# SiyuanHuang95/SUG

Hardware: AMD Instinct MI355X
Metric: point-clouds/sec (train step, N=1024) (higher is better)
Workload: dtype f32

## Files before the change

include/sug_amd.h:

```cpp
#ifndef SUG_AMD_H
#define SUG_AMD_H

#include <stdint.h>

#ifdef __cplusplus
extern "C" {
#endif

#define SUG_OK 0
#define SUG_ERR_ARG (-1)
#define SUG_ERR_LAUNCH (-2)
#define SUG_STATS_BLOCKS 1024

const char* sug_last_error(void);
#define SUG_ABI_VERSION 7
int sug_abi_version(void);

int sug_knn(const float* x, int64_t ldx, int B, int N, int C, int k,
            int32_t* idx, void* stream);

int sug_knn_reverse(const int32_t* idx, int B, int N, int k,
                    int32_t* rev_off, int32_t* rev_ent, void* stream);

int sug_fps(const float* xyz, const int32_t* start, int B, int N, int npoint,
// ... 8 lines not shown
                         int32_t* idx_out, float* dist_out, void* stream);

int sug_three_nn(const float* query, const float* cand, int B, int N, int S,
                 int32_t* idx3, float* dist3, void* stream);

int sug_three_nn_direct(const float* query, const float* cand, int B, int N, int S,
                        int32_t* idx3, float* dist3, void* stream);

int sug_ball_query_multi(const float* xyz, const float* query, int B, int N, int S, int R, const float* r2,
                         const int32_t* nsample, int32_t* const* out, void* stream);

int sug_fp_interp_fwd(const float* src, int64_t lds, const int32_t* idx3, const float* d3, int B, int N, int S, int D,
                      float* out, int64_t ldo, float* w3, void* stream);
int sug_fp_interp_bwd(const float* g, int64_t ldg, const int32_t* idx3, const float* w3, int B, int N, int S, int D,
                      int32_t* rev_off, int32_t* rev_ent, float* dsrc, int64_t ldd, void* stream);

int sug_copy_rows2d(const float* src, int64_t lds, float* dst, int64_t ldd, int64_t rows, int C, void* stream);

int sug_gather_rows(const float* feat, int64_t ldf, const int32_t* idx,
                    int B, int N, int S, int C, float* out, int64_t ldo, void* stream);
int sug_scatter_add_rows(const float* g, int64_t ldg, const int32_t* idx,
                         int B, int N, int S, int C, float* dfeat, int64_t ldf, void* stream);
int64_t sug_scatter_rows_workspace(int B, int N, int S);
int sug_scatter_rows_ordered_supported(int B, int N, int S);
int sug_scatter_rows_ordered(const float* g, int64_t ldg, const int32_t* idx, int B, int N, int S, int C,
                             float* dfeat, int64_t ldf, int32_t* ws, void* stream);

int sug_group_max(const float* feat, int64_t ldf, const int32_t* idx, int B, int N, int S,
                  int ns, int C, float* out, int32_t* arg, void* stream);
int sug_group_max_shared(const float* feat, int64_t ldf, int Bsrc, const int32_t* idx, int B, int N, int S,
                         int ns, int C, float* out, int32_t* arg, void* stream);
int sug_group_max_bwd(const float* g, const int32_t* arg, int B, int N, int S, int C,
                      float* dfeat, int64_t ldf, void* stream);

int sug_edgeconv_fwd(const float* pq, int64_t ldpq, const int32_t* idx, const float* gamma,
                     int B, int N, int k, int Co, float* z, uint8_t* arg, float* s1,
                     double* stats, float* ws, void* stream);

int sug_bn_finalize(const double* stats, const float* gamma, const float* beta, int C,
                    double count, float eps, float momentum, float* running_mean,
                    float* running_var, float* coef, void* stream);

int sug_edgeconv_fwd_bn(const float* pq, int64_t ldpq, const int32_t* idx, const float* gamma,
                        const float* beta, int B, int N, int k, int Co, float eps, float momentum,
                        float* running_mean, float* running_var, float* z, uint8_t* arg, float* s1,
                        float* coef, float* ws, void* stream);
int sug_col_stats_bn(const float* y, int64_t ldy, int64_t rows, int C, const float* gamma, const float* beta,
                     float eps, float momentum, float* running_mean, float* running_var, float* coef,
                     float* ws, void* stream);

int sug_col_stats_bn_grouped(const float* y, int64_t ldy, int64_t rows, int C, int groups, const float* gamma,
                             const float* beta, float eps, float momentum, float* running_mean, float* running_var,
                             float* coef, float* ws, void* stream);

int sug_bn_replay(const float* coef, int G, int C, float momentum, float* running_mean, float* running_var,
                  void* stream);
int sug_bn_replay_multi(int n, const void* const* coef, const int32_t* G, const int32_t* C, const float* momentum,
                        void* const* running_mean, void* const* running_var, void* stream);

int sug_affine_act(const float* z, int64_t ldz, const float* coef, int64_t rows, int C,
                   float slope, float* out, int64_t ldo, void* stream);

int sug_col_stats(const float* y, int64_t ldy, int64_t rows, int C, double* stats, float* ws,
                  void* stream);

int sug_edgeconv_bwd_reduce(const float* gout, int64_t ldg, const float* z, const float* coef,
                            int64_t rows, int Co, float slope, float* a, double* red, float* ws,
                            void* stream);
int sug_edgeconv_bwd_scatter(const float* a, const uint8_t* arg, const float* s1,
                             const float* pq, int64_t ldpq, const int32_t* rev_off,
                             const int32_t* rev_ent, const float* coef, const double* red,
                             int B, int N, int k, int Co, float* dpq, int64_t lddpq, void* stream);

int64_t sug_linear_dw_workspace(int64_t R, int M, int N);
int sug_linear_dw(const float* g, int64_t ldg, const float* x, int64_t ldx, int64_t R, int M, int N,
                  float* dw, float* ws, void* stream);
int sug_linear_dw_fold(const float* part, int nchunk, int64_t MN, float* dw, void* stream);
int sug_linear_dw_bias(const float* g, int64_t ldg, const float* x, int64_t ldx, int64_t R, int M, int N,
                       float* dw, float* db, float* ws, void* stream);

int64_t sug_colsum_workspace(int64_t rows, int C);
int sug_colsum(const void* x, int64_t ld, int64_t rows, int C, int dtype, float sign, float* out, float* ws, void* stream);

int sug_gate_fwd(const float* x, const float* z, int64_t n, float* out, void* stream);
int sug_gate_bwd(const float* g, const float* x, const float* z, int64_t n, float* dx, float* dz, void* stream);
int sug_gate_bn_fwd(const float* x, const float* z, int M, int C, const float* gamma, const float* beta,
                    float* running_mean, float* running_var, int training, float eps, float momentum, float* out,
                    float* stat, void* stream);
int sug_gate_bn_bwd(const float* g, const float* x, const float* z, int M, int C, const float* gamma, const float* stat,
                    int training, float* dx, float* dz, float* dgamma, float* dbeta, void* stream);

int sug_calayer_supported(int layers, int M, int C, int Hd);
int sug_calayer_fwd(int layers, const float* x, int64_t ldx, int M, int C, int Hd, const float* const* W0,
                    const float* const* b0, const float* const* W2, const float* const* b2, float* hp, float* h, float* z,
                    void* stream);
int sug_calayer_bwd(int layers, const float* x, int64_t ldx, int M, int C, int Hd, const float* const* W0,
                    const float* const* W2, const float* h, const float* dz, const float* dxg, float* const* dW0,
                    float* const* db0, float* const* dW2, float* const* db2, float* dhp, float* dh, float* dx, int64_t lddx,
                    void* stream);

int sug_head_linear_supported(int M, int K, int No, int pro, int epi);
int sug_head_linear_fwd(int heads, const float* const* in, int64_t ldin, const float* const* W, const float* const* bias,
                        float* const* z, const float* const* gamma, const float* const* beta, const float* const* u,
                        float* const* stats, float* const* act, int M, int K, int No, int pro, float slope, float eps,
                        float p_drop, void* stream);
int sug_head_ln_bwd(int heads, const float* const* gup, int64_t ldg, const float* const* z, const float* const* stats,
                    const float* const* gamma, const float* const* beta, const float* const* u,
                    const float* const* gextra, float* const* dz, float* const* dgamma, float* const* dbeta,
                    float* const* db, int M, int No, float slope, float p_drop, void* stream);
int sug_head_linear_bwd(int heads, int sum_da, const float* const* dz, int64_t ldg, const float* const* in, int64_t ldin,
                        const float* const* stats_in, const float* const* gamma_in, const float* const* beta_in,
                        const float* const* u_in, const float* const* W, float* const* dW, float* const* db,
                        float* const* da, int64_t ldda, int M, int K, int No, int pro, float slope, float p_drop_in,
                        void* stream);

int sug_ln_act_fwd(const float* x, const float* gamma, const float* beta, int rows, int C, float eps, float slope,
                   float* y, float* stat, void* stream);
int sug_ln_act_bwd(const float* g, const float* x, const float* gamma, const float* beta, const float* stat, int rows,
                   int C, float slope, float* dx, float* dgamma, float* dbeta, float* ws, void* stream);

int sug_adam_chunk(void);
int sug_adam_step(const int64_t* table, const int32_t* block_first, const int32_t* block_first_host, int T,
                  const void* const* grads_host, double lr, double beta1, double beta2, double eps,
                  double weight_decay, double bias_corr1, double bias_corr2, void* stream);
int sug_adam_step_capturable(const int64_t* table, const int32_t* block_first, const int32_t* block_first_host,
                             int T, const void* const* grads_host, double lr, double beta1, double beta2,
                             double eps, double weight_decay, int32_t* step_dev, float* scalars_dev,
                             const double* lr_dev, void* stream);

#define SUG_ADAM_CHAIN_SLOTS 2
#define SUG_ADAM_CHAIN_BUCKETS 8
int sug_adam_chain_chunk(void);
int sug_adam_chain_step(const int64_t* table, const int32_t* block_map, const int32_t* block_first_host, int T,
                        const void* const* grads_host, int nbuckets, const double* hyper_host, int32_t* steps_dev,
                        float* scalars_dev, const double* lr_dev, void* stream);

int sug_node_offset_fwd(const float* proj, const float* loc, const int32_t* fidx,
                        const int32_t* gidx, int B, int N, int S, int ns, float* off, float* nloc,
                        void* stream);
int sug_node_offset_bwd(const float* proj, const float* loc, const int32_t* fidx,
                        const int32_t* gidx, const float* goff, int B, int N, int S, int ns,
                        float* dproj, void* stream);
int sug_node_offset_fwd_shared(const float* proj, int Bsrc, const float* loc, const int32_t* fidx,
// ... 24 lines not shown
                        const float* gmean, int64_t ld_pool, const int32_t* arg, int B, int N, int C, float slope,
                        int train, double* red, float* ws, float* dy, int64_t lddy, void* stream);

int sug_edgeconv_layer_fwd(const float* pq, int64_t ldpq, const int32_t* idx, const float* gamma,
                           const float* beta, int B, int N, int k, int Co, int groups, int training,
                           float eps, float momentum, float slope, float* running_mean,
                           float* running_var, float* z, uint8_t* arg, float* s1, float* coef,
                           float* out, int64_t ldo, double* stats, float* ws, void* stream);
int sug_edgeconv_fused_supported(int N, int k, int Cin, int Co);
int sug_edgeconv_fused_layer_fwd(const float* x, int64_t ldx, int Cin, const float* wcat, const float* qbias,
                                 const int32_t* idx, const float* gamma, const float* beta, int B, int N, int k,
                                 int Co, int groups, int training, float eps, float momentum, float slope,
                                 float* running_mean, float* running_var, float* z, uint8_t* arg, float* s1,
                                 float* pq_out, int64_t ldpq, float* coef, float* out, int64_t ldo, float* ws,
                                 void* stream);
int sug_edgeconv_layer_bwd(const float* gout, int64_t ldg, const float* z, const uint8_t* arg,
                           const float* s1, const float* pq, int64_t ldpq, const int32_t* idx,
                           const float* coef, int B, int N, int k, int Co, int groups, int training,
                           float slope, float* a, double* red, int32_t* rev_off, int32_t* rev_ent,
                           float* dpq, int64_t lddpq, float* ws, float* dgb, void* stream);
int sug_sa_first_fwd(const float* P, int64_t ldp, const float* Q, const int32_t* idx, int B, int N, int S,
                     int ns, int C, int groups, const float* gamma, const float* beta, int training,
                     float eps, float momentum, float* running_mean, float* running_var, float* coef,
                     float* Z, float* ws, void* stream);
int sug_sa_first_bwd(const float* gz, const float* P, int64_t ldp, const float* Q, const int32_t* idx, int B,
                     int N, int S, int ns, int C, int groups, int training, const float* coef, double* red,
                     int32_t* rev_off, int32_t* rev_ent, float* segsum, float* dP, float* dQ, float* ws, float* dgb,
                     void* stream);
int sug_sa_first_geo_fwd(const float* Pf, int64_t ldp, const float* xyz, const float* cent, const float* Wx, int ldw,
                         const float* bias, const int32_t* idx, int B, int N, int S, int ns, int C, int groups,
                         const float* gamma, const float* beta, int training, float eps, float momentum,
                         float* running_mean, float* running_var, float* coef, float* Z, float* ws, void* stream);
int sug_sa_first_geo_bwd(const float* gz, const float* Pf, int64_t ldp, const float* xyz, const float* cent, const float* Wx,
                         int ldw, const float* bias, const int32_t* idx, int B, int N, int S, int ns, int C, int groups,
                         int training, const float* coef, double* red, int32_t* rev_off, int32_t* rev_ent, float* segsum,
                         float* dP, float* dQ, float* ws, float* dgb, void* stream);

int sug_bn_act_rows_fwd(const float* y, int64_t ldy, int64_t rows, int C, int groups, const float* gamma,
                        const float* beta, int training, float eps, float momentum, float slope,
                        float* running_mean, float* running_var, float* coef, float* out, int64_t ldo,
                        double* stats, float* ws, void* stream);
int sug_bn_act_rows_bwd(const float* gout, int64_t ldg, const float* y, int64_t ldy, const float* coef,
                        int64_t rows, int C, int groups, int training, float slope, float* a, double* red,
                        float* dy, float* ws, float* dgb, void* stream);
int sug_bn_act_pool_layer_fwd(const float* y, int64_t ldy, int B, int N, int C, int groups,
                              const float* gamma, const float* beta, int training, float eps, float momentum,
                              float slope, float* running_mean, float* running_var, float* coef,
                              float* out_max, float* out_mean, int64_t ld_pool, int32_t* arg, double* stats, float* ws_stats,
                              float* ws_pool, void* stream);
int sug_bn_act_pool_layer_bwd(const float* y, int64_t ldy, const float* coef, const float* gmax,
                              const float* gmean, int64_t ld_pool, const int32_t* arg, int B, int N, int C, int groups,
                              float slope, int training, double* red, float* ws, float* dy, int64_t lddy,
                              float* dgb, void* stream);

int sug_pointmlp_max_fwd(const float* x, int64_t ldx, int64_t rows, int K, const float* w, const float* bias,
                         const float* gamma, int Co, int seg, float* zext, int32_t* arg, float* ws, int* nblk,
                         void* stream);
int sug_rows_gemm(const float* x, int64_t ldx, int64_t rows, int K, const float* w, const float* bias, int Co,
                  float* y, int64_t ldy, void* stream);
int sug_pointmlp_max_layer_fwd(const float* x, int64_t ldx, int64_t rows, int K, const float* w, const float* bias,
                               const float* gamma, const float* beta, int Co, int seg, int groups, int training,
                               float eps, float momentum, float slope, float* running_mean, float* running_var,
                               float* zext, int32_t* arg, float* coef, float* out, int64_t ldo, float* ws,
                               void* stream);
int sug_pointmlp_max_layer_fwd_xf(const float* y, int64_t ldy, int64_t rows, int K, const float* xcoef, float xslope,
                                  float* zout, int64_t ldz, const float* w, const float* bias, const float* gamma,
                                  const float* beta, int Co, int seg, int groups, int training, float eps, float momentum,
                                  float slope, float* running_mean, float* running_var, float* zext, int32_t* arg,
                                  float* coef, float* out, int64_t ldo, float* ws, void* stream);
int sug_pointmlp_max_bwd_coef(const float* coef, const double* red, const float* bias, const float* w, int64_t rows,
                              int K, int Co, float* kb, float* k2, float* nkb, float* nwk, void* stream);
int sug_pointmlp_max_bwd_dwfix(float* dw, const float* dws, const float* kb, const float* k2, const float* w,
                               const float* xtx, const float* sx, int K, int Co, int with_stats, void* stream);
int64_t sug_pointmlp_max_bwd_workspace(int64_t rows, int K, int Co, int seg);
int sug_pointmlp_max_bwd_sparse(const float* a, const int32_t* arg, const float* x, int64_t ldx, const float* w,
                                int64_t rows, int K, int Co, int seg, float* dx, int64_t lddx, float* dw,
                                float* ws, void* stream);

int sug_ptran_pos1_fwd(const float* xyz, const int32_t* nbr, const float* w1, const float* b1, int B, int n, int k,
                       int d, int dtype, void* out, void* stream);
int sug_ptran_pos1_bwd(const void* g, const float* xyz, const int32_t* nbr, const float* w1, const float* b1, int B,
                       int n, int k, int d, int dtype, float* dw1, float* db1, float* ws, void* stream);
int sug_ptran_qk_fwd(const float* q, const float* kf, const void* delta, const int32_t* nbr, int B, int n, int k, int d,
                     int dtype, void* out, void* stream);
int sug_ptran_qk_bwd(const void* du, void* da, const int32_t* rev_off, const int32_t* rev_ent, int B, int n, int k, int d,
                     int dtype, float* dq, float* dk, float* db, float* ws, void* stream);
int sug_ptran_attn_fwd(const void* logits, const void* delta, const float* vf, const int32_t* nbr, int B, int n, int k,
                       int d, int dtype, float scale, float* mixed, float* mx, float* sm, void* stream);
int sug_ptran_attn_bwd(const float* g, const float* mixed, const void* logits, const void* delta, const float* vf,
                       const int32_t* nbr, const float* mx, const float* sm, const int32_t* rev_off, const int32_t* rev_ent,
                       int B, int n, int k, int d, int dtype, float scale, void* dlogits, void* da, float* dv, float* db,
                       float* ws, void* stream);
int sug_ptran_fused_supported(int B, int n, int k, int d);
int sug_ptran_fused_fwd(const float* xyz, const int32_t* nbr, const float* q, const float* kf, const float* vf,
                        const float* w1, const float* b1, const void* w2, const void* b2, const void* wg1, const void* bg1,
                        const void* wg2, const void* bg2, int B, int n, int k, int d, float scale, int save, void* T0,
                        void* delta, void* U, void* T1, void* Lg, float* mixed, float* mx, float* sm, void* stream);
int64_t sug_ptran_colsum_workspace(int64_t rows);
int sug_ptran_relu_bwd_db(void* G, const void* T1, int64_t rows, int d, int dtype, float* db, float* ws, void* stream);
int sug_grad_scale16(const float* g0, int64_t n0, const float* g1, int64_t n1, const float* g2, int64_t n2, int log2_target,
                     float* out, float* ws, void* stream);

int sug_fold_groups(const double* red, int groups, int n, float* out, void* stream);

int sug_mmd_rbf(const float* z, int64_t ldz, int m, int D, const float* w,
                const float* neg_gamma, int nsigma, double* sums, float* wt, void* stream);
// ... 23 lines not shown
int sug_soft_mmd_multi_fwd(int n, const void* const* feat_s, const int64_t* lds, const void* const* feat_t,
                           const int64_t* ldt, const int32_t* D, const float* label_scale, const int64_t* label_s,
                           const int64_t* label_t, int m, int num_class, const void* const* w, const float* neg_gamma,
                           int nsigma, void* const* z, void* const* wt, double* sums, float* values, void* stream);
int sug_soft_mmd_multi_bwd(int n, const void* const* z, const int32_t* D, const void* const* wt,
                           const void* const* gscale, int m, int num_class, void* const* dz, void* stream);

#define SUG_CLASS_MMD_MAX_ROWS 1024
#define SUG_CLASS_MMD_MAX_CLASSES 64
#define SUG_CLASS_MMD_MAX_D 1048576
int sug_mmd_select(const int64_t* label_s, const int64_t* label_t, int m, int num_class, int mode, int32_t* idx_s,
                   int32_t* idx_t, int32_t* pos_s, int32_t* pos_t, int32_t* count, void* stream);
int sug_class_mmd_fwd(const float* feat_s, int64_t lds, const float* feat_t, int64_t ldt, int m, int D,
                      const int32_t* idx_s, const int32_t* idx_t, const int32_t* count, const float* neg_gamma,
                      int nsigma, float* z, float* wt, double* sums, float* value, void* stream);
int sug_class_mmd_bwd(const float* z, const float* wt, int m, int D, const int32_t* count, const int32_t* pos_s,
                      const int32_t* pos_t, const float* gscale, float* dz, float* dfeat_s, int64_t ldds,
                      float* dfeat_t, int64_t lddt, void* stream);

#define SUG_MMD_EST_MAX_ROWS 1024
#define SUG_MMD_EST_MAX_D 1048576
#define SUG_MMD_EST_MAX_SIGMAS 8
#define SUG_MMD_POLY_MAX_DEGREE 8
#define SUG_MMD_RATIO_ROW_FIELDS 9
#define SUG_MMD_RATIO_STATS 16
int sug_mmd_ratio_fwd(const float* z, int64_t ldz, int m, int D, const float* neg_gamma, int nsigma, int biased, float* K,
                      float* G, double* rows, double* stats, float* out3, float* wt_m, float* wt_v, void* stream);
int sug_mmd_ratio_bwd(const float* z, int64_t ldz, int m, int D, const float* wt_m, const float* wt_v, const float* out3,
                      const float* g3, float* dz, int64_t lddz, void* stream);
int sug_mmd_adjacent_fwd(const float* x, int64_t ldx, const float* y, int64_t ldy, int m, int D, int mode, int degree,
                         double alpha, double c, double* part, float* coef, float* value, void* stream);
int sug_mmd_adjacent_bwd(const float* x, int64_t ldx, const float* y, int64_t ldy, int m, int D, int mode, const float* coef,
                         const float* gscale, float* dx, int64_t lddx, float* dy, int64_t lddy, void* stream);

#define SUG_CL_LOSS_MAX_ROWS 1024
#define SUG_CL_LOSS_MAX_D 1048576
#define SUG_CL_LOSS_MAX_TERMS 4
#define SUG_CL_LOSS_SUM_FIELDS 3
#define SUG_CL_LOSS_ROW_FIELDS 4
int sug_cl_loss_fwd(int n, const void* const* x, const int64_t* ldx, const void* const* y, const int64_t* ldy, const int32_t* D,
                    const double* margin, const int64_t* label_s, const int64_t* label_t, int m, const void* const* w,
                    double* sums, void* const* coef, float* values, void* stream);
int sug_cl_loss_bwd(int n, const void* const* x, const int64_t* ldx, const void* const* y, const int64_t* ldy, const int32_t* D,
                    int m, const void* const* coef, const void* const* gscale, void* const* dx, const int64_t* lddx,
                    void* const* dy, const int64_t* lddy, void* stream);

int sug_edge_weight_split(const float* in, int Co, int C, int backward, float* out, void* stream);
int sug_edge_weight_split_multi(const void* const* in_host, const int32_t* Co_host, const int32_t* C_host, int n,
                                int backward, void* const* out_host, void* stream);

int64_t sug_chamfer_workspace(int B, int N, int M);
int sug_chamfer(const float* a, const float* b, int B, int N, int M, float* out, float* ws, void* stream);
int sug_chamfer_weights(const float* a, const float* b, int B, int N, int M, int method, float* out, float* ws, void* stream);
#define SUG_CHAMFER_MAX_POINTS 5000
int sug_chamfer_nn(const float* a, const float* b, int B, int N, int M, float* dist1, float* dist2, int32_t* idx1, int32_t* idx2,
                   void* stream);
int sug_chamfer_nn_bwd(const float* g1, const float* g2, const float* a, const float* b, const int32_t* idx1, const int32_t* idx2,
                       int B, int N, int M, float* ga, float* gb, void* stream);

#define SUG_CE_PAIR_MAX_ROWS 512
#define SUG_CE_PAIR_MAX_CLASSES 32
int sug_ce_pair_fwd(const float* logits1, const float* logits2, int64_t ld, const int64_t* label, int M, int C, float w,
                    int64_t ignore_index, float* loss, float* lse, void* stream);
int sug_ce_pair_bwd(const float* logits1, const float* logits2, int64_t ld, const int64_t* label, int M, int Mtot, int C,
                    float w, int64_t ignore_index, const float* g, const float* lse, float* d1, float* d2, void* stream);
#define SUG_CE_MAX_ROWS 1024
#define SUG_CE_MAX_CLASSES 64
int sug_ce_fwd(const float* logits, int64_t ld, const int64_t* label, int M, int C, int64_t ignore_index, float label_smoothing,
               float* loss, float* lse, double* totals, void* stream);
int sug_ce_bwd(const float* logits, int64_t ld, const int64_t* label, int M, int C, int64_t ignore_index, float label_smoothing,
               const float* g, const float* lse, float* dlogits, void* stream);
#define SUG_MCD_MAX_ROWS 1024
int sug_mcd_loss_fwd(const float* ys1, const float* ys2, const float* yt1, const float* yt2, int64_t ld, const int64_t* label,
                     const int64_t* label_t, int Ms, int Mt, int C, float a_s, float a_t, float r_s, float* out4, float* lse,
                     double* totals, void* stream);
int sug_mcd_loss_bwd(const float* ys1, const float* ys2, const float* yt1, const float* yt2, int64_t ld, const int64_t* label,
                     const int64_t* label_t, int Ms, int Mt, int C, float a_s, float a_t, const float* g, const float* lse,
                     float* ds1, float* ds2, float* dt1, float* dt2, void* stream);
int sug_cls_loss_fwd(const float* ys1, const float* ys2, const float* yt1, const float* yt2, int64_t ld, const int64_t* label,
                     const int64_t* label_t, int Ms, int Mt, int C, const float* alpha, float gamma, int reduce_sum,
                     int64_t ignore_index, float a_s, float a_t, float a_d, float r_s, float* out4, float* save, double* totals,
                     void* stream);
int sug_cls_loss_bwd(const float* ys1, const float* ys2, const float* yt1, const float* yt2, int64_t ld, const int64_t* label,
                     const int64_t* label_t, int Ms, int Mt, int C, const float* alpha, float gamma, int reduce_sum,
                     int64_t ignore_index, float a_s, float a_t, float a_d, float r_s, const float* g, const float* save,
                     float* ds1, float* ds2, float* dt1, float* dt2, void* stream);
int sug_loss_combine_fwd(const float* loss_cls, const float* v_geo, const float* v_sem1, const float* v_sem2, float wg, float ws,
                         float* out3, void* stream);
int sug_loss_combine_bwd(const float* g, float wg, float ws, float* out4, void* stream);

#define SUG_EVAL_MAX_ROWS 4096
#define SUG_EVAL_MAX_CLASSES 64
#define SUG_EVAL_BATCH_COUNT 0
#define SUG_EVAL_DATA_TOTAL 1
#define SUG_EVAL_CORRECT_TOTAL 2
#define SUG_EVAL_ERROR 3
#define SUG_EVAL_LOSS_TOTAL 4
#define SUG_EVAL_CLASS_ACC 8
#define SUG_EVAL_CLASS_ROWS 136
#define SUG_EVAL_CLASS_CORRECT 200
#define SUG_EVAL_BATCH_ACC 264
#define SUG_EVAL_STATE_WORDS(cap) (SUG_EVAL_BATCH_ACC + (cap))
int sug_eval_accumulate(const float* logits1, const float* logits2, int64_t ld, const int64_t* label, int B, int C,
                        const float* loss_in, int ce_mode, int64_t ignore_index, float label_smoothing, float* out,
                        int64_t* pred, int cls_eval, void* state, int cap, void* stream);

// ... 91 lines not shown
```

sug_amd/csrc/bnpool.hip:

```cpp
#include "common.h"
#include <hip/hip_fp16.h>

namespace {

__global__ __launch_bounds__(256) void bn_bwd_apply_vec4_kernel(const float* __restrict__ a,
                                                                const float* __restrict__ y, int64_t ldy,
                                                                const float* __restrict__ coef,
                                                                const double* __restrict__ red,
                                                                int64_t rows, int C, float invM,
                                                                float* __restrict__ dy, int64_t lddy) {
  const int C4 = C >> 2;
  const int64_t total = rows * C4;
  for (int64_t e = (int64_t)blockIdx.x * 256 + threadIdx.x; e < total; e += (int64_t)gridDim.x * 256) {
    const int c = (int)(e % C4) * 4;
    const int64_t r = e / C4;
    const float4 av = *reinterpret_cast<const float4*>(a + r * C + c);
    const float4 yv = *reinterpret_cast<const float4*>(y + r * ldy + c);
    const float4 sc = *reinterpret_cast<const float4*>(coef + c);
    const float4 mean = *reinterpret_cast<const float4*>(coef + 2 * C + c);
    const float4 rstd = *reinterpret_cast<const float4*>(coef + 3 * C + c);
    float4 o;
    o.x = av.x - sc.x * invM * ((float)red[c + 0] + (yv.x - mean.x) * rstd.x * (float)red[C + c + 0]);
    o.y = av.y - sc.y * invM * ((float)red[c + 1] + (yv.y - mean.y) * rstd.y * (float)red[C + c + 1]);
    o.z = av.z - sc.z * invM * ((float)red[c + 2] + (yv.z - mean.z) * rstd.z * (float)red[C + c + 2]);
// ... 10 lines not shown
                                                                       int64_t rows_g, int C, float invM, float slope,
                                                                       float* __restrict__ dy, int64_t lddy) {
  const int C4 = C >> 2;
  const int64_t total = rows * C4;
  for (int64_t e = (int64_t)blockIdx.x * 256 + threadIdx.x; e < total; e += (int64_t)gridDim.x * 256) {
    const int c = (int)(e % C4) * 4;
    const int64_t r = e / C4;
    const int64_t g = r / rows_g;
    const float* cg = coef + g * 5 * C;
    const double* rg = red + g * 2 * C;
    float4 av = *reinterpret_cast<const float4*>(a + r * lda + c);
    const float4 yv = *reinterpret_cast<const float4*>(y + r * ldy + c);
    const float4 sc = *reinterpret_cast<const float4*>(cg + c);
    const float4 mean = *reinterpret_cast<const float4*>(cg + 2 * C + c);
    const float4 rstd = *reinterpret_cast<const float4*>(cg + 3 * C + c);
    if (FROM_G) {
      const float4 sh = *reinterpret_cast<const float4*>(cg + C + c);
      av.x = sc.x * (av.x * (fmaf(sc.x, yv.x, sh.x) > 0.f ? 1.f : slope));
      av.y = sc.y * (av.y * (fmaf(sc.y, yv.y, sh.y) > 0.f ? 1.f : slope));
      av.z = sc.z * (av.z * (fmaf(sc.z, yv.z, sh.z) > 0.f ? 1.f : slope));
      av.w = sc.w * (av.w * (fmaf(sc.w, yv.w, sh.w) > 0.f ? 1.f : slope));
    }
    float4 o;
    o.x = av.x - sc.x * invM * ((float)rg[c + 0] + (yv.x - mean.x) * rstd.x * (float)rg[C + c + 0]);
    o.y = av.y - sc.y * invM * ((float)rg[c + 1] + (yv.y - mean.y) * rstd.y * (float)rg[C + c + 1]);
    o.z = av.z - sc.z * invM * ((float)rg[c + 2] + (yv.z - mean.z) * rstd.z * (float)rg[C + c + 2]);
    o.w = av.w - sc.w * invM * ((float)rg[c + 3] + (yv.w - mean.w) * rstd.w * (float)rg[C + c + 3]);
    *reinterpret_cast<float4*>(dy + r * lddy + c) = o;
  }
}

__global__ __launch_bounds__(256) void bn_bwd_apply_kernel(const float* __restrict__ a,
                                                           const float* __restrict__ y, int64_t ldy,
                                                           const float* __restrict__ coef,
                                                           const double* __restrict__ red, int64_t rows,
                                                           int C, float invM, float* __restrict__ dy,
                                                           int64_t lddy) {
  const int64_t total = rows * C;
  for (int64_t e = (int64_t)blockIdx.x * 256 + threadIdx.x; e < total; e += (int64_t)gridDim.x * 256) {
    const int c = (int)(e % C);
    const int64_t r = e / C;
    const float f = coef[c] * invM;
    const float xhat = (y[r * ldy + c] - coef[2 * C + c]) * coef[3 * C + c];
    dy[r * lddy + c] = a[r * C + c] - f * ((float)red[c] + xhat * (float)red[C + c]);
  }
}

constexpr int NS = 4;

__device__ __forceinline__ float lrelu(float u, float slope) { return u > 0.f ? u : u * slope; }

template <int VEC>
__global__ __launch_bounds__(256) void bn_act_pool_part_kernel(const float* __restrict__ y, int64_t ldy,
                                                               const float* __restrict__ coef, int N,
                                                               int C, float slope,
                                                               float* __restrict__ pmax,
                                                               float* __restrict__ psum,
                                                               int32_t* __restrict__ parg) {
  constexpr int LX = 64 / VEC, LY = 256 / LX;
  __shared__ float s_m[LY][64];
  __shared__ float s_s[LY][64];
  __shared__ int s_a[LY][64];
  const int b = blockIdx.y, ch = blockIdx.z;
  const int lx = threadIdx.x % LX, ly = threadIdx.x / LX;
  const int c = blockIdx.x * 64 + lx * VEC;
  const int n0 = (int)((int64_t)N * ch / NS), n1 = (int)((int64_t)N * (ch + 1) / NS);
  float best[VEC], sum[VEC];
  int bi[VEC];
#pragma unroll
  for (int v = 0; v < VEC; ++v) { best[v] = -INFINITY; sum[v] = 0.f; bi[v] = n0; }
  if (c < C) {
    float sc[VEC], sh[VEC];
#pragma unroll
    for (int v = 0; v < VEC; ++v) { sc[v] = coef[c + v]; sh[v] = coef[C + c + v]; }
    const float* p = y + (int64_t)b * N * ldy + c;
#pragma unroll 4
    for (int n = n0 + ly; n < n1; n += LY) {
      float val[VEC];
      if constexpr (VEC == 4) {
        const float4 t = *reinterpret_cast<const float4*>(p + (int64_t)n * ldy);
        val[0] = t.x; val[1] = t.y; val[2] = t.z; val[3] = t.w;
      } else {
        val[0] = p[(int64_t)n * ldy];
      }
#pragma unroll
      for (int v = 0; v < VEC; ++v) {
        const float u = lrelu(fmaf(sc[v], val[v], sh[v]), slope);
        sum[v] += u;
        if (u > best[v]) { best[v] = u; bi[v] = n; }
      }
    }
  }
#pragma unroll
  for (int v = 0; v < VEC; ++v) {
    s_m[ly][lx * VEC + v] = best[v];
    s_s[ly][lx * VEC + v] = sum[v];
    s_a[ly][lx * VEC + v] = bi[v];
  }
  __syncthreads();
  if (threadIdx.x < 64) {
    const int cc = blockIdx.x * 64 + threadIdx.x;
    if (cc < C) {
      float m = s_m[0][threadIdx.x], sm = s_s[0][threadIdx.x];
      int a = s_a[0][threadIdx.x];
      for (int i = 1; i < LY; ++i) {
        sm += s_s[i][threadIdx.x];
        const float mi = s_m[i][threadIdx.x];
        const int ai = s_a[i][threadIdx.x];
        if (mi > m || (mi == m && ai < a)) { m = mi; a = ai; }
      }
      const int64_t o = ((int64_t)b * NS + ch) * C + cc;
      pmax[o] = m; psum[o] = sm; parg[o] = a;
    }
  }
}

__global__ __launch_bounds__(256) void pool_combine_kernel(const float* __restrict__ pmax,
                                                           const float* __restrict__ psum,
                                                           const int32_t* __restrict__ parg, int B, int N,
                                                           int C, float* __restrict__ omax,
                                                           float* __restrict__ omean, int64_t ldp,
                                                           int32_t* __restrict__ arg) {
  const int64_t e = (int64_t)blockIdx.x * 256 + threadIdx.x;
  if (e >= (int64_t)B * C) return;
  const int b = (int)(e / C), c = (int)(e % C);
  float m = -INFINITY, sm = 0.f;
  int a = 0;
  for (int ch = 0; ch < NS; ++ch) {
    const int64_t o = ((int64_t)b * NS + ch) * C + c;
    sm += psum[o];
    if (pmax[o] > m) { m = pmax[o]; a = parg[o]; }
  }
  omax[(int64_t)b * ldp + c] = m; omean[(int64_t)b * ldp + c] = sm / (float)N; arg[e] = a;
}

template <int VEC>
__global__ __launch_bounds__(256) void pool_bwd_reduce_kernel(const float* __restrict__ y, int64_t ldy,
                                                              const float* __restrict__ coef,
                                                              const float* __restrict__ gmax,
                                                              const float* __restrict__ gmean, int64_t ldp,
                                                              const int32_t* __restrict__ arg, int N,
                                                              int C, float slope, float* __restrict__ ws) {
  constexpr int LX = 64 / VEC, LY = 256 / LX;
  __shared__ float s_g[LY][64];
  __shared__ float s_x[LY][64];
  const int b = blockIdx.y, ch = blockIdx.z;
  const int lx = threadIdx.x % LX, ly = threadIdx.x / LX;
  const int c = blockIdx.x * 64 + lx * VEC;
  const int n0 = (int)((int64_t)N * ch / NS), n1 = (int)((int64_t)N * (ch + 1) / NS);
  float sg[VEC], sx[VEC];
#pragma unroll
  for (int v = 0; v < VEC; ++v) { sg[v] = 0.f; sx[v] = 0.f; }
  if (c < C) {
    float sc[VEC], sh[VEC], mean[VEC], rstd[VEC], gm[VEC], gx[VEC];
    int am[VEC];
#pragma unroll
    for (int v = 0; v < VEC; ++v) {
      sc[v] = coef[c + v]; sh[v] = coef[C + c + v]; mean[v] = coef[2 * C + c + v]; rstd[v] = coef[3 * C + c + v];
      gm[v] = gmean[(int64_t)b * ldp + c + v] / (float)N;
      gx[v] = gmax[(int64_t)b * ldp + c + v];
      am[v] = arg[(int64_t)b * C + c + v];
    }
    const float* p = y + (int64_t)b * N * ldy + c;
#pragma unroll 4
    for (int n = n0 + ly; n < n1; n += LY) {
      float val[VEC];
      if constexpr (VEC == 4) {
        const float4 t = *reinterpret_cast<const float4*>(p + (int64_t)n * ldy);
        val[0] = t.x; val[1] = t.y; val[2] = t.z; val[3] = t.w;
      } else {
        val[0] = p[(int64_t)n * ldy];
      }
#pragma unroll
      for (int v = 0; v < VEC; ++v) {
        const float u = fmaf(sc[v], val[v], sh[v]);
        const float g = (u > 0.f ? 1.f : slope) * (gm[v] + (n == am[v] ? gx[v] : 0.f));
        sg[v] += g;
        sx[v] = fmaf(g, (val[v] - mean[v]) * rstd[v], sx[v]);
      }
    }
  }
#pragma unroll
  for (int v = 0; v < VEC; ++v) {
    s_g[ly][lx * VEC + v] = sg[v];
    s_x[ly][lx * VEC + v] = sx[v];
  }
  __syncthreads();
  if (threadIdx.x < 64) {
    const int cc = blockIdx.x * 64 + threadIdx.x;
    if (cc < C) {
      float tg = 0.f, tx = 0.f;
      for (int i = 0; i < LY; ++i) { tg += s_g[i][threadIdx.x]; tx += s_x[i][threadIdx.x]; }
      float* w = ws + ((size_t)b * NS + ch) * 2 * C;
      w[cc] = tg;
      w[C + cc] = tx;
    }
  }
}

template <int VEC>
__global__ __launch_bounds__(256) void pool_bwd_apply_kernel(const float* __restrict__ y, int64_t ldy,
                                                             const float* __restrict__ coef,
                                                             const double* __restrict__ red,
                                                             const float* __restrict__ gmax,
                                                             const float* __restrict__ gmean, int64_t ldp,
                                                             const int32_t* __restrict__ arg, int B,
                                                             int N, int C, float slope, float invM,
                                                             float* __restrict__ dy, int64_t lddy) {
  const int CV = C / VEC;
  const int64_t total = (int64_t)B * N * CV;
  for (int64_t e = (int64_t)blockIdx.x * 256 + threadIdx.x; e < total; e += (int64_t)gridDim.x * 256) {
    const int c = (int)(e % CV) * VEC;
    const int64_t r = e / CV;
    const int b = (int)(r / N), n = (int)(r - (int64_t)b * N);
    float val[VEC], out[VEC];
    if constexpr (VEC == 4) {
      const float4 t = *reinterpret_cast<const float4*>(y + r * ldy + c);
      val[0] = t.x; val[1] = t.y; val[2] = t.z; val[3] = t.w;
    } else {
      val[0] = y[r * ldy + c];
    }
#pragma unroll
    for (int v = 0; v < VEC; ++v) {
      const float sc = coef[c + v];
      const float u = fmaf(sc, val[v], coef[C + c + v]);
      const float g = (u > 0.f ? 1.f : slope) * (gmean[(int64_t)b * ldp + c + v] / (float)N +
                                                 (n == arg[(int64_t)b * C + c + v] ? gmax[(int64_t)b * ldp + c + v] : 0.f));
      const float xhat = (val[v] - coef[2 * C + c + v]) * coef[3 * C + c + v];
      out[v] = sc * (g - invM * ((float)red[c + v] + xhat * (float)red[C + c + v]));
    }
    if constexpr (VEC == 4) {
      *reinterpret_cast<float4*>(dy + r * lddy + c) = make_float4(out[0], out[1], out[2], out[3]);
    } else {
      dy[r * lddy + c] = out[0];
    }
  }
}

__global__ __launch_bounds__(256) void pool_bwd_apply_rows_kernel(const float* __restrict__ y, int64_t ldy,
                                                                  const float* __restrict__ coef,
                                                                  const double* __restrict__ red,
                                                                  const float* __restrict__ gmax,
                                                                  const float* __restrict__ gmean, int64_t ldp,
                                                                  const int32_t* __restrict__ arg, int N, int C,
                                                                  int rows_per_block, float slope, float invM,
                                                                  float* __restrict__ dy, int64_t lddy) {
  const int CV = C >> 2;
  const int b = blockIdx.y;
  const int cg = threadIdx.x % CV, rl = threadIdx.x / CV, rstep = 256 / CV;
  const int c = cg * 4;
  float sc[4], sh[4], mu[4], rs[4], r0[4], r1[4], gme[4], gmx[4];
  int am[4];
#pragma unroll
  for (int v = 0; v < 4; ++v) {
    sc[v] = coef[c + v];
    sh[v] = coef[C + c + v];
    mu[v] = coef[2 * C + c + v];
    rs[v] = coef[3 * C + c + v];
    r0[v] = (float)red[c + v];
    r1[v] = (float)red[C + c + v];
    gme[v] = gmean[(int64_t)b * ldp + c + v] / (float)N;
    gmx[v] = gmax[(int64_t)b * ldp + c + v];
    am[v] = arg[(int64_t)b * C + c + v];
  }
  const int n0 = blockIdx.x * rows_per_block;
  const int n1 = n0 + rows_per_block < N ? n0 + rows_per_block : N;
  const float* yb = y + (int64_t)b * N * ldy + c;
  float* db = dy + (int64_t)b * N * lddy + c;
#pragma unroll 4
  for (int n = n0 + rl; n < n1; n += rstep) {
    const float4 t = *reinterpret_cast<const float4*>(yb + (int64_t)n * ldy);
    const float val[4] = {t.x, t.y, t.z, t.w};
    float out[4];
#pragma unroll
    for (int v = 0; v < 4; ++v) {
      const float u = fmaf(sc[v], val[v], sh[v]);
      const float g = (u > 0.f ? 1.f : slope) * (gme[v] + (n == am[v] ? gmx[v] : 0.f));
      const float xhat = (val[v] - mu[v]) * rs[v];
      out[v] = sc[v] * (g - invM * (r0[v] + xhat * r1[v]));
    }
    *reinterpret_cast<float4*>(db + (int64_t)n * lddy) = make_float4(out[0], out[1], out[2], out[3]);
  }
}

__global__ __launch_bounds__(256) void reduce_rows_kernel(const float* __restrict__ ws, int nrow, int W,
                                                          double* __restrict__ out) {
  __shared__ double s_p[16][17];
  const int cl = threadIdx.x & 15, p = threadIdx.x >> 4;
  const int c = blockIdx.x * 16 + cl;
  double acc = 0.0;
  if (c < W)
    for (int b = p; b < nrow; b += 16) acc += (double)ws[(size_t)b * W + c];
  s_p[p][cl] = acc;
  __syncthreads();
  if (p == 0 && c < W) {
    double t = 0.0;
#pragma unroll
    for (int i = 0; i < 16; ++i) t += s_p[i][cl];
    out[c] = t;
  }
}
// ... 104 lines not shown
    }
  }
  s1 = wave_sum_f(s1) / (float)C;
  s2 = wave_sum_f(s2) / (float)C;
#pragma unroll
  for (int u = 0; u < LN_MAXV; ++u) {
    const int c = lane + 64 * u;
    if (c < C) dx[(size_t)r * C + c] = rstd * (gh[u] - s1 - xh[u] * s2);
  }
}

__global__ __launch_bounds__(256) void ln_act_bwd_param_kernel(const float* __restrict__ ga, const float* __restrict__ x,
                                                               const float* __restrict__ stat, int rows, int C,
                                                               float* __restrict__ dgamma, float* __restrict__ dbeta) {
  const int c = blockIdx.x * 256 + threadIdx.x;
  if (c >= C) return;
  float dg = 0.f, db = 0.f;
  for (int r0 = 0; r0 < rows; r0 += 8) {
    float a[8], xv[8];
#pragma unroll
    for (int u = 0; u < 8; ++u) {
      const int r = r0 + u < rows ? r0 + u : rows - 1;
      a[u] = ga[(size_t)r * C + c];
      xv[u] = x[(size_t)r * C + c];
    }
#pragma unroll
    for (int u = 0; u < 8; ++u) {
      if (r0 + u >= rows) continue;
      const int r = r0 + u;
      dg = fmaf(a[u], (xv[u] - stat[2 * r]) * stat[2 * r + 1], dg);
      db += a[u];
    }
  }
  dgamma[c] = dg;
  dbeta[c] = db;
}

static bool vec4_ok(const float* y, int64_t ld, int C) {
  return (C % 4 == 0) && (ld % 4 == 0) && ((uintptr_t)y % 16 == 0);
}

extern "C" int sug_bn_act_pool_fwd(const float* y, int64_t ldy, const float* coef, int B, int N, int C,
                                   float slope, float* out_max, float* out_mean, int64_t ld_pool, int32_t* arg,
                                   float* ws, void* stream) {
  SUG_REQUIRE(y && coef && out_max && out_mean && arg && ws, "sug_bn_act_pool_fwd: null pointer");
  SUG_REQUIRE(B > 0 && N > 0 && C > 0 && ldy >= C && ld_pool >= C && B <= 65535, "sug_bn_act_pool_fwd: bad shape");
  hipStream_t st = (hipStream_t)stream;
  const size_t part = (size_t)B * NS * C;
  float* pmax = ws;
  float* psum = ws + part;
  int32_t* parg = reinterpret_cast<int32_t*>(ws + 2 * part);
  dim3 grid(sug_divup(C, 64), B, NS);
  if (vec4_ok(y, ldy, C))
    hipLaunchKernelGGL((bn_act_pool_part_kernel<4>), grid, dim3(256), 0, st, y, ldy, coef, N, C, slope, pmax, psum, parg);
  else
    hipLaunchKernelGGL((bn_act_pool_part_kernel<1>), grid, dim3(256), 0, st, y, ldy, coef, N, C, slope, pmax, psum, parg);
  SUG_LAUNCH_CHECK("sug_bn_act_pool_fwd");
  hipLaunchKernelGGL(pool_combine_kernel, dim3(sug_divup((int64_t)B * C, 256)), dim3(256), 0, st, pmax, psum, parg,
                     B, N, C, out_max, out_mean, ld_pool, arg);
  SUG_LAUNCH_CHECK("sug_bn_act_pool_fwd(combine)");
  return SUG_OK;
}

extern "C" int sug_bn_act_pool_bwd(const float* y, int64_t ldy, const float* coef, const float* gmax,
                                   const float* gmean, int64_t ld_pool, const int32_t* arg, int B, int N, int C,
                                   float slope, int train, double* red, float* ws, float* dy,
                                   int64_t lddy, void* stream) {
  SUG_REQUIRE(y && coef && gmax && gmean && arg && red && ws && dy, "sug_bn_act_pool_bwd: null pointer");
  SUG_REQUIRE(B > 0 && N > 0 && C > 0 && ldy >= C && lddy >= C && ld_pool >= C && B * NS <= SUG_STATS_BLOCKS,
              "sug_bn_act_pool_bwd: bad shape (B must be <= %d)", SUG_STATS_BLOCKS / NS);
  hipStream_t st = (hipStream_t)stream;
  const bool vec = vec4_ok(y, ldy, C) && vec4_ok(dy, lddy, C);
  dim3 grid(sug_divup(C, 64), B, NS);
  if (vec)
    hipLaunchKernelGGL((pool_bwd_reduce_kernel<4>), grid, dim3(256), 0, st, y, ldy, coef, gmax, gmean, ld_pool, arg, N, C, slope, ws);
  else
    hipLaunchKernelGGL((pool_bwd_reduce_kernel<1>), grid, dim3(256), 0, st, y, ldy, coef, gmax, gmean, ld_pool, arg, N, C, slope, ws);
  SUG_LAUNCH_CHECK("sug_bn_act_pool_bwd(reduce)");
  hipLaunchKernelGGL(reduce_rows_kernel, dim3(sug_divup(2 * C, 16)), dim3(256), 0, st, ws, B * NS, 2 * C, red);
  SUG_LAUNCH_CHECK("sug_bn_act_pool_bwd(combine)");
  const float invM = train ? (float)(1.0 / ((double)B * N)) : 0.f;
  if (vec && (C / 4) <= 256 && 256 % (C / 4) == 0 && B <= 65535) {
    const int rpb = 64 > 256 / (C / 4) ? 64 : 256 / (C / 4);
    hipLaunchKernelGGL(pool_bwd_apply_rows_kernel, dim3(sug_divup(N, rpb), B), dim3(256), 0, st, y, ldy, coef, red, gmax,
                       gmean, ld_pool, arg, N, C, rpb, slope, invM, dy, lddy);
  } else if (vec)
    hipLaunchKernelGGL((pool_bwd_apply_kernel<4>), dim3(ew_grid((int64_t)B * N * C / 4)), dim3(256), 0, st, y, ldy,
                       coef, red, gmax, gmean, ld_pool, arg, B, N, C, slope, invM, dy, lddy);
  else
    hipLaunchKernelGGL((pool_bwd_apply_kernel<1>), dim3(ew_grid((int64_t)B * N * C)), dim3(256), 0, st, y, ldy, coef,
                       red, gmax, gmean, ld_pool, arg, B, N, C, slope, invM, dy, lddy);
  SUG_LAUNCH_CHECK("sug_bn_act_pool_bwd(apply)");
  return SUG_OK;
}


namespace {
__global__ __launch_bounds__(256) void fold_groups_kernel(const double* __restrict__ red, int groups, int n,
                                                          float* __restrict__ out) {
  const int i = blockIdx.x * 256 + threadIdx.x;
  if (i >= n) return;
  double t = 0.0;
  for (int g = 0; g < groups; ++g) t += red[(int64_t)g * n + i];
  out[i] = (float)t;
}
}

extern "C" int sug_fold_groups(const double* red, int groups, int n, float* out, void* stream) {
  SUG_REQUIRE(red && out && groups >= 1 && n > 0, "sug_fold_groups: bad argument");
  hipLaunchKernelGGL(fold_groups_kernel, dim3(sug_divup(n, 256)), dim3(256), 0, (hipStream_t)stream, red, groups, n, out);
  SUG_LAUNCH_CHECK("sug_fold_groups");
  return SUG_OK;
}

extern "C" int sug_ln_act_fwd(const float* x, const float* gamma, const float* beta, int rows, int C, float eps, float slope,
                              float* y, float* stat, void* stream) {
  SUG_REQUIRE(x && gamma && beta && y && stat, "sug_ln_act_fwd: null pointer");
  SUG_REQUIRE(rows > 0 && C > 0 && C <= 64 * LN_MAXV, "sug_ln_act_fwd: rows=%d C=%d (C <= %d)", rows, C, 64 * LN_MAXV);
  hipLaunchKernelGGL(ln_act_fwd_kernel, dim3(sug_divup(rows, 4)), dim3(256), 0, (hipStream_t)stream, x, gamma, beta, rows, C, eps,
                     slope, y, stat);
  SUG_LAUNCH_CHECK("sug_ln_act_fwd");
  return SUG_OK;
}

extern "C" int sug_ln_act_bwd(const float* g, const float* x, const float* gamma, const float* beta, const float* stat, int rows,
                              int C, float slope, float* dx, float* dgamma, float* dbeta, float* ws, void* stream) {
  SUG_REQUIRE(g && x && gamma && beta && stat && dx && dgamma && dbeta && ws, "sug_ln_act_bwd: null pointer");
  SUG_REQUIRE(rows > 0 && C > 0 && C <= 64 * LN_MAXV, "sug_ln_act_bwd: rows=%d C=%d (C <= %d)", rows, C, 64 * LN_MAXV);
  hipStream_t st = (hipStream_t)stream;
  hipLaunchKernelGGL(ln_act_bwd_dx_kernel, dim3(sug_divup(rows, 4)), dim3(256), 0, st, g, x, gamma, beta, stat, rows, C, slope, dx,
                     ws);
  SUG_LAUNCH_CHECK("sug_ln_act_bwd");
  hipLaunchKernelGGL(ln_act_bwd_param_kernel, dim3(sug_divup(C, 256)), dim3(256), 0, st, ws, x, stat, rows, C, dgamma, dbeta);
  SUG_LAUNCH_CHECK("sug_ln_act_bwd(param)");
  return SUG_OK;
}

namespace {

__global__ __launch_bounds__(256) void gate_fwd_kernel(const float* __restrict__ x, const float* __restrict__ z, int64_t n,
                                                       float* __restrict__ out) {
  const int64_t i = (int64_t)blockIdx.x * 256 + threadIdx.x;
  if (i >= n) return;
  const float s = 1.0f / (1.0f + expf(-z[i]));
  out[i] = __fadd_rn(__fmul_rn(x[i], s), x[i]);
}

__global__ __launch_bounds__(256) void gate_bwd_kernel(const float* __restrict__ g, const float* __restrict__ x,
                                                       const float* __restrict__ z, int64_t n, float* __restrict__ dx,
                                                       float* __restrict__ dz) {
  const int64_t i = (int64_t)blockIdx.x * 256 + threadIdx.x;
  if (i >= n) return;
  const float s = 1.0f / (1.0f + expf(-z[i]));
  const float gi = g[i];
  dx[i] = __fadd_rn(__fmul_rn(gi, s), gi);
  dz[i] = __fmul_rn(__fmul_rn(gi, x[i]), __fmul_rn(__fsub_rn(1.0f, s), s));
}

}

extern "C" int sug_gate_fwd(const float* x, const float* z, int64_t n, float* out, void* stream) {
  SUG_REQUIRE(x && z && out, "sug_gate_fwd: null pointer");
  SUG_REQUIRE(n > 0, "sug_gate_fwd: empty input");
  hipLaunchKernelGGL(gate_fwd_kernel, dim3((unsigned)sug_divup(n, 256)), dim3(256), 0, (hipStream_t)stream, x, z, n, out);
  SUG_LAUNCH_CHECK("sug_gate_fwd");
  return SUG_OK;
}

extern "C" int sug_gate_bwd(const float* g, const float* x, const float* z, int64_t n, float* dx, float* dz, void* stream) {
  SUG_REQUIRE(g && x && z && dx && dz, "sug_gate_bwd: null pointer");
  SUG_REQUIRE(n > 0, "sug_gate_bwd: empty input");
  hipLaunchKernelGGL(gate_bwd_kernel, dim3((unsigned)sug_divup(n, 256)), dim3(256), 0, (hipStream_t)stream, g, x, z, n, dx, dz);
  SUG_LAUNCH_CHECK("sug_gate_bwd");
  return SUG_OK;
}

namespace {

__device__ __forceinline__ float gate_val(float x, float z) {
  const float s = 1.0f / (1.0f + expf(-z));
  return __fadd_rn(__fmul_rn(x, s), x);
}

template <int MR>
__global__ __launch_bounds__(64) void gate_bn_fwd_kernel(const float* __restrict__ x, const float* __restrict__ z, int M, int C,
                                                         const float* __restrict__ gamma, const float* __restrict__ beta,
                                                         float* __restrict__ rmean, float* __restrict__ rvar, int training,
                                                         float eps, float momentum, float* __restrict__ out,
                                                         float* __restrict__ stat) {
  const int c = blockIdx.x * 64 + threadIdx.x;
  if (c >= C) return;
  float gv[MR > 0 ? MR : 1];
  if constexpr (MR > 0) {
    float xv[MR], zv[MR];
#pragma unroll
    for (int i = 0; i < MR; ++i) {
      const int r = i < M ? i : M - 1;
      xv[i] = x[(int64_t)r * C + c];
      zv[i] = z[(int64_t)r * C + c];
    }
#pragma unroll
    for (int i = 0; i < MR; ++i) gv[i] = gate_val(xv[i], zv[i]);
  }
  auto g_at = [&](int i) { if constexpr (MR > 0) return gv[i]; else return gate_val(x[(int64_t)i * C + c], z[(int64_t)i * C + c]); };
  float mean, invstd;
  if (training) {
    float s = 0.f;
    if constexpr (MR > 0) {
#pragma unroll
      for (int i = 0; i < MR; ++i) s += i < M ? gv[i] : 0.f;
    } else {
#pragma unroll 8
      for (int i = 0; i < M; ++i) s += g_at(i);
    }
    mean = s / (float)M;
    float q = 0.f;
    if constexpr (MR > 0) {
#pragma unroll
      for (int i = 0; i < MR; ++i) { const float d = gv[i] - mean; q = i < M ? fmaf(d, d, q) : q; }
    } else {
#pragma unroll 8
      for (int i = 0; i < M; ++i) { const float d = g_at(i) - mean; q = fmaf(d, d, q); }
    }
    const float var = q / (float)M;
    invstd = 1.0f / sqrtf(var + eps);
    if (rmean) {
      rmean[c] = (1.0f - momentum) * rmean[c] + momentum * mean;
      rvar[c] = (1.0f - momentum) * rvar[c] + momentum * (M > 1 ? q / (float)(M - 1) : var);
    }
  } else {
    mean = rmean[c];
    invstd = 1.0f / sqrtf(rvar[c] + eps);
  }
  stat[c] = mean;
  stat[C + c] = invstd;
  const float sc = gamma[c] * invstd, sh = beta[c] - mean * sc;
  if constexpr (MR > 0) {
#pragma unroll
    for (int i = 0; i < MR; ++i)
      if (i < M) out[(int64_t)i * C + c] = fmaf(gv[i], sc, sh);
  } else {
#pragma unroll 8
    for (int i = 0; i < M; ++i) out[(int64_t)i * C + c] = fmaf(g_at(i), sc, sh);
  }
}

template <int MR>
__global__ __launch_bounds__(64) void gate_bn_bwd_kernel(const float* __restrict__ g, const float* __restrict__ x,
                                                         const float* __restrict__ z, int M, int C,
                                                         const float* __restrict__ gamma, const float* __restrict__ stat,
                                                         int training, float* __restrict__ dx, float* __restrict__ dz,
                                                         float* __restrict__ dgamma, float* __restrict__ dbeta) {
  const int c = blockIdx.x * 64 + threadIdx.x;
  if (c >= C) return;
  const float mean = stat[c], invstd = stat[C + c];
  float sb = 0.f, sg = 0.f;
  float xr[MR > 0 ? MR : 1], sr[MR > 0 ? MR : 1], hr[MR > 0 ? MR : 1], gr[MR > 0 ? MR : 1];
  if constexpr (MR > 0) {
    float zr[MR];
#pragma unroll
    for (int i = 0; i < MR; ++i) {
      const int r = i < M ? i : M - 1;
      xr[i] = x[(int64_t)r * C + c];
      zr[i] = z[(int64_t)r * C + c];
      gr[i] = i < M ? g[(int64_t)r * C + c] : 0.f;
    }
#pragma unroll
    for (int i = 0; i < MR; ++i) {
      sr[i] = 1.0f / (1.0f + expf(-zr[i]));
      hr[i] = (__fadd_rn(__fmul_rn(xr[i], sr[i]), xr[i]) - mean) * invstd;
      sb += gr[i];
      sg = fmaf(gr[i], hr[i], sg);
    }
  } else {
#pragma unroll 8
    for (int i = 0; i < M; ++i) {
      const float gi = g[(int64_t)i * C + c];
      const float xh = (gate_val(x[(int64_t)i * C + c], z[(int64_t)i * C + c]) - mean) * invstd;
      sb += gi;
      sg = fmaf(gi, xh, sg);
    }
  }
  dgamma[c] = sg;
  dbeta[c] = sb;
  const float k = gamma[c] * invstd;
  const float mb = training ? sb / (float)M : 0.f, mg = training ? sg / (float)M : 0.f;
  if constexpr (MR > 0) {
#pragma unroll
    for (int i = 0; i < MR; ++i) {
      if (i < M) {
        const float dg = k * (gr[i] - mb - hr[i] * mg);
        dx[(int64_t)i * C + c] = __fadd_rn(__fmul_rn(dg, sr[i]), dg);
        dz[(int64_t)i * C + c] = __fmul_rn(__fmul_rn(dg, xr[i]), __fmul_rn(__fsub_rn(1.0f, sr[i]), sr[i]));
      }
    }
  } else {
#pragma unroll 8
    for (int i = 0; i < M; ++i) {
      const float xv = x[(int64_t)i * C + c], zv = z[(int64_t)i * C + c];
      const float s = 1.0f / (1.0f + expf(-zv));
      const float gv = __fadd_rn(__fmul_rn(xv, s), xv);
      const float xh = (gv - mean) * invstd;
      const float dg = k * (g[(int64_t)i * C + c] - mb - xh * mg);
      dx[(int64_t)i * C + c] = __fadd_rn(__fmul_rn(dg, s), dg);
      dz[(int64_t)i * C + c] = __fmul_rn(__fmul_rn(dg, xv), __fmul_rn(__fsub_rn(1.0f, s), s));
    }
  }
}

}

extern "C" int sug_gate_bn_fwd(const float* x, const float* z, int M, int C, const float* gamma, const float* beta,
                               float* running_mean, float* running_var, int training, float eps, float momentum, float* out,
                               float* stat, void* stream) {
  SUG_REQUIRE(x && z && gamma && beta && out && stat, "sug_gate_bn_fwd: null pointer");
  SUG_REQUIRE(M >= 1 && M <= 1024 && C >= 1, "sug_gate_bn_fwd: bad shape M=%d C=%d", M, C);
  SUG_REQUIRE(training || (running_mean && running_var), "sug_gate_bn_fwd: eval mode needs the running buffers");
  SUG_REQUIRE(!running_mean == !running_var, "sug_gate_bn_fwd: running_mean and running_var come together");
  if (M <= 32)
    hipLaunchKernelGGL(gate_bn_fwd_kernel<32>, dim3((unsigned)sug_divup(C, 64)), dim3(64), 0, (hipStream_t)stream, x, z, M, C, gamma,
                       beta, running_mean, running_var, training, eps, momentum, out, stat);
  else
    hipLaunchKernelGGL(gate_bn_fwd_kernel<0>, dim3((unsigned)sug_divup(C, 64)), dim3(64), 0, (hipStream_t)stream, x, z, M, C, gamma,
                       beta, running_mean, running_var, training, eps, momentum, out, stat);
  SUG_LAUNCH_CHECK("sug_gate_bn_fwd");
  return SUG_OK;
}

extern "C" int sug_gate_bn_bwd(const float* g, const float* x, const float* z, int M, int C, const float* gamma,
                               const float* stat, int training, float* dx, float* dz, float* dgamma, float* dbeta,
                               void* stream) {
  SUG_REQUIRE(g && x && z && gamma && stat && dx && dz && dgamma && dbeta, "sug_gate_bn_bwd: null pointer");
  SUG_REQUIRE(M >= 1 && M <= 1024 && C >= 1, "sug_gate_bn_bwd: bad shape M=%d C=%d", M, C);
  if (M <= 32)
    hipLaunchKernelGGL(gate_bn_bwd_kernel<32>, dim3((unsigned)sug_divup(C, 64)), dim3(64), 0, (hipStream_t)stream, g, x, z, M, C,
                       gamma, stat, training, dx, dz, dgamma, dbeta);
  else
    hipLaunchKernelGGL(gate_bn_bwd_kernel<0>, dim3((unsigned)sug_divup(C, 64)), dim3(64), 0, (hipStream_t)stream, g, x, z, M, C,
                       gamma, stat, training, dx, dz, dgamma, dbeta);
  SUG_LAUNCH_CHECK("sug_gate_bn_bwd");
  return SUG_OK;
}

namespace {

template <typename T>
__global__ __launch_bounds__(256) void colsum_part_kernel(const T* __restrict__ x, int64_t ld, int64_t R, int C,
                                                          float* __restrict__ part) {
  __shared__ float s_p[8][33];
  const int cx = threadIdx.x & 31, ry = threadIdx.x >> 5;
  const int c = blockIdx.x * 32 + cx;
  float acc = 0.f;
  if (c < C)
    for (int64_t r = (int64_t)blockIdx.y * 8 + ry; r < R; r += (int64_t)gridDim.y * 8) acc += (float)x[r * ld + c];
  s_p[ry][cx] = acc;
  __syncthreads();
  if (ry == 0 && c < C) {
    float t = s_p[0][cx];
#pragma unroll
    for (int i = 1; i < 8; ++i) t += s_p[i][cx];
    part[(int64_t)blockIdx.y * C + c] = t;
  }
}

__global__ __launch_bounds__(256) void colsum_fold_kernel(const float* __restrict__ part, int nblk, int C, float sign,
                                                          float* __restrict__ out) {
  const int c = blockIdx.x * 256 + threadIdx.x;
  if (c >= C) return;
  double t = 0.0;
  for (int b = 0; b < nblk; ++b) t += (double)part[(int64_t)b * C + c];
  out[c] = sign * (float)t;
}

}

extern "C" int64_t sug_colsum_workspace(int64_t rows, int C) {
  int64_t nblk = (rows + 63) / 64;
  if (nblk > 128) nblk = 128;
  if (nblk < 1) nblk = 1;
  return nblk * (int64_t)C;
}

extern "C" int sug_colsum(const void* x, int64_t ld, int64_t rows, int C, int dtype, float sign, float* out, float* ws,
                          void* stream) {
  SUG_REQUIRE(x && out && ws, "sug_colsum: null pointer");
  SUG_REQUIRE(rows > 0 && C > 0 && ld >= C && (dtype == 0 || dtype == 1), "sug_colsum: bad shape / dtype (0 fp32, 1 fp16)");
  const int nblk = (int)(sug_colsum_workspace(rows, C) / C);
  hipStream_t st = (hipStream_t)stream;
  const dim3 grid(sug_divup(C, 32), nblk);
  if (dtype == 0) hipLaunchKernelGGL(colsum_part_kernel<float>, grid, dim3(256), 0, st, (const float*)x, ld, rows, C, ws);
  else hipLaunchKernelGGL(colsum_part_kernel<__half>, grid, dim3(256), 0, st, (const __half*)x, ld, rows, C, ws);
  SUG_LAUNCH_CHECK("sug_colsum");
  hipLaunchKernelGGL(colsum_fold_kernel, dim3(sug_divup(C, 256)), dim3(256), 0, st, ws, nblk, C, sign, out);
  SUG_LAUNCH_CHECK("sug_colsum(fold)");
  return SUG_OK;
}
// ... 1 lines not shown
```

sug_amd/csrc/edgeconv.hip:

```cpp
#include "common.h"

namespace {

__device__ __forceinline__ float4 ld4(const float* p) { return *reinterpret_cast<const float4*>(p); }
__device__ __forceinline__ void st4(float* p, float4 v) { *reinterpret_cast<float4*>(p) = v; }

template <int NCH>
__global__ __launch_bounds__(256) void edgeconv_fwd_kernel(
    const float* __restrict__ pq, int64_t ldpq, const int32_t* __restrict__ idx,
    const float* __restrict__ gamma, int64_t BN, int N, int k, int Co, int LPP, int bpc,
    float* __restrict__ z, uint8_t* __restrict__ arg, float* __restrict__ s1,
    float* __restrict__ ws) {
  extern __shared__ __attribute__((aligned(16))) float s_red[];
  const int nchunk = Co >> 2;
  const int ppb = 256 / LPP;
  const int slot = threadIdx.x / LPP, ch0 = threadIdx.x % LPP;
  float4 a1[NCH], a2[NCH], gs[NCH];
#pragma unroll
  for (int u = 0; u < NCH; ++u) {
    a1[u] = make_float4(0, 0, 0, 0);
    a2[u] = make_float4(0, 0, 0, 0);
    const int ch = ch0 + u * LPP;
    gs[u] = ch < nchunk ? ld4(gamma + ch * 4) : make_float4(1, 1, 1, 1);
  }
// ... 312 lines not shown
  const int col = (cl < 8) ? ch : C + ch;
  const int W = 2 * C;
  const bool fin = threadIdx.x < 8 && ch < C;
  float rm = (fin && rmean) ? rmean[ch] : 0.f, rv = (fin && rvar) ? rvar[ch] : 0.f;
  for (int g0 = 0; g0 < groups; g0 += GMAX) {
    const int ng = groups - g0 < GMAX ? groups - g0 : GMAX;
    double acc[GMAX] = {0.0, 0.0, 0.0, 0.0};
    if (ch < C) {
#pragma unroll 4
      for (int b = p; b < nblk; b += RL) {
#pragma unroll
        for (int g = 0; g < GMAX; ++g)
          if (g < ng) acc[g] += (double)ws[((size_t)(g0 + g) * nblk + b) * W + col];
      }
    }
    __syncthreads();
#pragma unroll
    for (int g = 0; g < GMAX; ++g) s_p[g][p][cl] = acc[g];
    __syncthreads();
    if (p < ng) {
      double t = 0.0;
#pragma unroll
      for (int i = 0; i < RL; ++i) t += s_p[p][i][cl];
      s_tot[p][cl] = t;
    }
    __syncthreads();
    if (fin) {
      const int c = ch;
      for (int g = 0; g < ng; ++g) {
        float* cg = coef + (size_t)(g0 + g) * 5 * C;
        const double m1 = s_tot[g][threadIdx.x] / count;
        double var = s_tot[g][8 + threadIdx.x] / count - m1 * m1;
        if (var < 0) var = 0;
        const double mean = (pivot ? (double)pivot[(size_t)(g0 + g) * C + c] : 0.0) + m1;
        const float rstd = (float)(1.0 / sqrt(var + (double)eps));
        const float scale = gamma[c] * rstd;
        cg[c] = scale;
        cg[C + c] = beta[c] - (float)mean * scale;
        cg[2 * C + c] = (float)mean;
        cg[3 * C + c] = rstd;
        const double unb = count > 1.0 ? var * count / (count - 1.0) : var;
        cg[4 * C + c] = (float)unb;
        rm = (1.f - momentum) * rm + momentum * (float)mean;
        rv = (1.f - momentum) * rv + momentum * (float)unb;
      }
    }
  }
  if (fin) {
    if (rmean) rmean[ch] = rm;
    if (rvar) rvar[ch] = rv;
  }
}

__global__ __launch_bounds__(256) void bn_replay_kernel(const float* __restrict__ coef, int G, int C,
                                                        float momentum, float* __restrict__ rmean,
                                                        float* __restrict__ rvar) {
  const int c = blockIdx.x * 256 + threadIdx.x;
  if (c >= C) return;
  float m = rmean[c], v = rvar[c];
  for (int g = 0; g < G; ++g) {
    const float* cg = coef + (size_t)g * 5 * C;
    m = (1.f - momentum) * m + momentum * cg[2 * C + c];
    v = (1.f - momentum) * v + momentum * cg[4 * C + c];
  }
  rmean[c] = m;
  rvar[c] = v;
}

#define SUG_REPLAY_MULTI 16
struct ReplayMulti {
  const float* coef[SUG_REPLAY_MULTI];
  float* rmean[SUG_REPLAY_MULTI];
  float* rvar[SUG_REPLAY_MULTI];
  int G[SUG_REPLAY_MULTI], C[SUG_REPLAY_MULTI];
  float momentum[SUG_REPLAY_MULTI];
};
__global__ __launch_bounds__(256) void bn_replay_multi_kernel(ReplayMulti a) {
  const int l = blockIdx.y, C = a.C[l], G = a.G[l];
  const int c = blockIdx.x * 256 + threadIdx.x;
  if (c >= C) return;
  const float momentum = a.momentum[l];
  const float* coef = a.coef[l];
  float m = a.rmean[l][c], v = a.rvar[l][c];
  for (int g = 0; g < G; ++g) {
    const float* cg = coef + (size_t)g * 5 * C;
    m = (1.f - momentum) * m + momentum * cg[2 * C + c];
    v = (1.f - momentum) * v + momentum * cg[4 * C + c];
  }
  a.rmean[l][c] = m;
  a.rvar[l][c] = v;
}

__global__ __launch_bounds__(256) void affine_act_kernel(const float* __restrict__ z, int64_t ldz,
                                                         const float* __restrict__ coef, int64_t rows,
                                                         int C, float slope, float* __restrict__ out,
                                                         int64_t ldo) {
  const int64_t total = rows * C;
  for (int64_t e = (int64_t)blockIdx.x * 256 + threadIdx.x; e < total; e += (int64_t)gridDim.x * 256) {
    const int c = (int)(e % C);
    const int64_t r = e / C;
    const float u = fmaf(coef[c], z[r * ldz + c], coef[C + c]);
    out[r * ldo + c] = u > 0.f ? u : u * slope;
  }
}

__global__ __launch_bounds__(256) void affine_act_vec4_kernel(const float* __restrict__ z, int64_t ldz,
// ... 53 lines not shown
template <int MODE>
__global__ __launch_bounds__(256) void col_reduce_kernel(const float* __restrict__ y, int64_t ldy,
                                                         const float* __restrict__ z,
                                                         const float* __restrict__ coef, int64_t rows,
                                                         int C, float slope, float* __restrict__ a,
                                                         float* __restrict__ ws, int CW,
                                                         int rows_per_block, int pivoted) {
  extern __shared__ float s_red[];
  const int RY = 256 / CW;
  const int cx = threadIdx.x % CW, ry = threadIdx.x / CW;
  const int64_t r0 = (int64_t)blockIdx.x * rows_per_block;
  int64_t r1 = r0 + rows_per_block;
  if (r1 > rows) r1 = rows;
  for (int c = cx; c < C; c += CW) {
    float s = 0.f, q = 0.f;
    float scale = 0.f, shift = 0.f, mean = 0.f, rstd = 0.f;
    const float pv = (MODE == 0 && pivoted) ? y[c] : 0.f;
    if (MODE == 0 && pivoted && blockIdx.x == 0 && ry == 0) ws[SUG_PIVOT_OFFSET(C) + c] = pv;
    if (MODE == 1) {
      scale = coef[c]; shift = coef[C + c]; mean = coef[2 * C + c]; rstd = coef[3 * C + c];
    }
    for (int64_t r = r0 + ry; r < r1; r += RY) {
      if (MODE == 0) {
        const float v = y[r * ldy + c] - pv;
        s += v;
        q = fmaf(v, v, q);
      } else {
        const float zv = z[r * C + c];
        const float u = fmaf(scale, zv, shift);
        const float g = y[r * ldy + c] * (u > 0.f ? 1.f : slope);
        a[r * C + c] = scale * g;
        s += g;
        q = fmaf(g, (zv - mean) * rstd, q);
      }
    }
    s_red[(size_t)ry * 2 * C + c] = s;
    s_red[(size_t)ry * 2 * C + C + c] = q;
  }
  __syncthreads();
  for (int i = threadIdx.x; i < 2 * C; i += 256) {
    float acc = 0.f;
    for (int r = 0; r < RY; ++r) acc += s_red[(size_t)r * 2 * C + i];
    ws[(size_t)blockIdx.x * 2 * C + i] = acc;
  }
}

template <int MODE>
__global__ __launch_bounds__(256) void col_reduce_vec4_kernel(const float* __restrict__ y, int64_t ldy,
                                                              const float* __restrict__ z,
                                                              const float* __restrict__ coef,
                                                              int64_t rows, int C, float slope,
                                                              float* __restrict__ a,
                                                              float* __restrict__ ws, int LX,
                                                              int rows_per_block, int pivoted) {
  extern __shared__ __attribute__((aligned(16))) float s_red[];
  float* const ws_pivot = ws + SUG_PIVOT_OFFSET(C) + (size_t)blockIdx.y * C;
  const int64_t g0 = (int64_t)blockIdx.y * rows;
  y += g0 * ldy;
  if (MODE >= 1) {
    z += g0 * C;
    if (MODE == 1) a += g0 * C;
    coef += (int64_t)blockIdx.y * 5 * C;
  }
  ws += (size_t)blockIdx.y * gridDim.x * 2 * C;
  const int LY = 256 / LX;
  const int lx = threadIdx.x % LX, ly = threadIdx.x / LX;
  const int C4 = C >> 2;
  const int64_t r0 = (int64_t)blockIdx.x * rows_per_block;
  int64_t r1 = r0 + rows_per_block;
  if (r1 > rows) r1 = rows;
  for (int c4 = lx; c4 < C4; c4 += LX) {
    const int c = c4 * 4;
    float4 s = make_float4(0, 0, 0, 0), q = make_float4(0, 0, 0, 0);
    float4 sc = s, sh = s, mean = s, rstd = s;
    float4 pv = s;
    if (MODE == 0 && pivoted) {
      pv = *reinterpret_cast<const float4*>(y + c);
      if (blockIdx.x == 0 && ly == 0) *reinterpret_cast<float4*>(ws_pivot + c) = pv;
    }
    if (MODE >= 1) {
      sc = *reinterpret_cast<const float4*>(coef + c);
      sh = *reinterpret_cast<const float4*>(coef + C + c);
      mean = *reinterpret_cast<const float4*>(coef + 2 * C + c);
      rstd = *reinterpret_cast<const float4*>(coef + 3 * C + c);
    }
#pragma unroll 4
    for (int64_t r = r0 + ly; r < r1; r += LY) {
      float4 v = *reinterpret_cast<const float4*>(y + r * ldy + c);
      if (MODE == 0) {
        v.x -= pv.x; v.y -= pv.y; v.z -= pv.z; v.w -= pv.w;
        s.x += v.x; s.y += v.y; s.z += v.z; s.w += v.w;
        q.x = fmaf(v.x, v.x, q.x); q.y = fmaf(v.y, v.y, q.y); q.z = fmaf(v.z, v.z, q.z); q.w = fmaf(v.w, v.w, q.w);
      } else {
        const float4 zv = *reinterpret_cast<const float4*>(z + r * C + c);
        float4 g;
        g.x = v.x * (fmaf(sc.x, zv.x, sh.x) > 0.f ? 1.f : slope);
        g.y = v.y * (fmaf(sc.y, zv.y, sh.y) > 0.f ? 1.f : slope);
        g.z = v.z * (fmaf(sc.z, zv.z, sh.z) > 0.f ? 1.f : slope);
        g.w = v.w * (fmaf(sc.w, zv.w, sh.w) > 0.f ? 1.f : slope);
        if (MODE == 1)
          *reinterpret_cast<float4*>(a + r * C + c) = make_float4(sc.x * g.x, sc.y * g.y, sc.z * g.z, sc.w * g.w);
        s.x += g.x; s.y += g.y; s.z += g.z; s.w += g.w;
        q.x = fmaf(g.x, (zv.x - mean.x) * rstd.x, q.x); q.y = fmaf(g.y, (zv.y - mean.y) * rstd.y, q.y);
        q.z = fmaf(g.z, (zv.z - mean.z) * rstd.z, q.z); q.w = fmaf(g.w, (zv.w - mean.w) * rstd.w, q.w);
      }
    }
    *reinterpret_cast<float4*>(s_red + (size_t)ly * 2 * C + c) = s;
    *reinterpret_cast<float4*>(s_red + (size_t)ly * 2 * C + C + c) = q;
  }
  __syncthreads();
  for (int i = threadIdx.x; i < 2 * C; i += 256) {
    float acc = 0.f;
    for (int r = 0; r < LY; ++r) acc += s_red[(size_t)r * 2 * C + i];
    ws[(size_t)blockIdx.x * 2 * C + i] = acc;
  }
}

// ... 332 lines not shown
  }
  for (int g = 0; g < groups; ++g) {
    const int64_t r0 = (int64_t)g * rows;
    float* cg = coef + (int64_t)g * 5 * Co;
    if (int rc = sug_edgeconv_fwd_bn(pq + r0 * ldpq, ldpq, idx + r0 * k, gamma, beta, Bg, N, k, Co, eps, momentum, running_mean,
                                     running_var, z + r0 * Co, arg + r0 * Co, s1 ? s1 + r0 * Co : nullptr, cg, ws, stream))
      return rc;
    if (int rc = sug_affine_act(z + r0 * Co, Co, cg, rows, Co, slope, out + r0 * ldo, ldo, stream)) return rc;
  }
  return SUG_OK;
}

extern "C" int sug_bn_finalize(const double* stats, const float* gamma, const float* beta, int C,
                               double count, float eps, float momentum, float* running_mean,
                               float* running_var, float* coef, void* stream) {
  SUG_REQUIRE(stats && gamma && beta && coef, "sug_bn_finalize: null pointer");
  SUG_REQUIRE(C > 0 && count > 0, "sug_bn_finalize: bad shape");
  hipLaunchKernelGGL(bn_finalize_kernel, dim3(sug_divup(C, 256)), dim3(256), 0, (hipStream_t)stream,
                     stats, gamma, beta, C, count, eps, momentum, running_mean, running_var, coef);
  SUG_LAUNCH_CHECK("sug_bn_finalize");
  return SUG_OK;
}

extern "C" int sug_bn_replay(const float* coef, int G, int C, float momentum, float* running_mean,
                             float* running_var, void* stream) {
  SUG_REQUIRE(coef && running_mean && running_var, "sug_bn_replay: null pointer");
  SUG_REQUIRE(G > 0 && C > 0, "sug_bn_replay: bad shape");
  hipLaunchKernelGGL(bn_replay_kernel, dim3(sug_divup(C, 256)), dim3(256), 0, (hipStream_t)stream, coef, G, C,
                     momentum, running_mean, running_var);
  SUG_LAUNCH_CHECK("sug_bn_replay");
  return SUG_OK;
}

extern "C" int sug_affine_act(const float* z, int64_t ldz, const float* coef, int64_t rows, int C,
                              float slope, float* out, int64_t ldo, void* stream) {
  SUG_REQUIRE(z && coef && out, "sug_affine_act: null pointer");
  SUG_REQUIRE(rows > 0 && C > 0 && ldz >= C && ldo >= C, "sug_affine_act: bad shape");
  hipStream_t st = (hipStream_t)stream;
  const bool vec = (C % 4 == 0) && (ldz % 4 == 0) && (ldo % 4 == 0) && ((uintptr_t)z % 16 == 0) &&
                   ((uintptr_t)out % 16 == 0) && ((uintptr_t)coef % 16 == 0);
  const int64_t total = vec ? rows * (C / 4) : rows * C;
  int64_t g = (total + 255) / 256;
  if (g > 4096) g = 4096;
  if (vec)
    hipLaunchKernelGGL(affine_act_vec4_kernel, dim3((int)g), dim3(256), 0, st, z, ldz, coef, rows, C, slope, out, ldo);
  else
    hipLaunchKernelGGL(affine_act_kernel, dim3((int)g), dim3(256), 0, st, z, ldz, coef, rows, C, slope, out, ldo);
  SUG_LAUNCH_CHECK("sug_affine_act");
  return SUG_OK;
}

template <int MODE>
static int launch_col_reduce(const float* y, int64_t ldy, const float* z, const float* coef, int64_t rows,
                             int C, float slope, float* a, float* ws, hipStream_t st, int groups = 1, int pivoted = 0);

static int col_rows_per_block(int64_t rows, int cw) {
  int64_t rpb = 64 * (256 / cw) > 256 ? 64 * (256 / cw) : 256;
  while ((rows + rpb - 1) / rpb > SUG_STATS_ROWS) rpb *= 2;
  return (int)rpb;
}

template <int MODE>
static int launch_col_reduce(const float* y, int64_t ldy, const float* z, const float* coef, int64_t rows,
                             int C, float slope, float* a, float* ws, hipStream_t st, int groups, int pivoted) {
  const bool vec = (C % 4 == 0) && (ldy % 4 == 0) && ((uintptr_t)y % 16 == 0) &&
                   (MODE == 0 || (((uintptr_t)z % 16 == 0) && (MODE == 2 || (uintptr_t)a % 16 == 0) && ((uintptr_t)coef % 16 == 0)));
  if (vec) {
    int lx = 1;
    while (lx < (C >> 2) && lx < 256) lx <<= 1;
    const int ly = 256 / lx;
    int64_t rpb = (rows * groups + SUG_STATS_ROWS - 1) / SUG_STATS_ROWS;
    if (rpb < 4 * ly) rpb = 4 * ly;
    rpb = (rpb + ly - 1) / ly * ly;
    const int grid = sug_divup(rows, rpb);
    if ((int64_t)grid * groups > SUG_STATS_ROWS || groups > 16) return -1;
    hipLaunchKernelGGL((col_reduce_vec4_kernel<MODE>), dim3(grid, groups), dim3(256), (size_t)ly * 2 * C * sizeof(float),
                       st, y, ldy, z, coef, rows, C, slope, a, ws, lx, (int)rpb, pivoted);
    return grid;
  }
  if (groups > 1 || MODE == 2) return -1;
  const int cw = col_width(C);
  const int rpb = col_rows_per_block(rows, cw);
  const int grid = sug_divup(rows, rpb);
  hipLaunchKernelGGL((col_reduce_kernel<MODE>), dim3(grid), dim3(256), (size_t)(256 / cw) * 2 * C * sizeof(float),
                     st, y, ldy, z, coef, rows, C, slope, a, ws, cw, rpb, pivoted);
  return grid;
}

extern "C" int sug_col_stats(const float* y, int64_t ldy, int64_t rows, int C, double* stats,
                             float* ws, void* stream) {
  SUG_REQUIRE(y && stats && ws, "sug_col_stats: null pointer");
  SUG_REQUIRE(rows > 0 && C > 0 && C <= 4096 && ldy >= C, "sug_col_stats: bad shape");
  hipStream_t st = (hipStream_t)stream;
  const int grid = launch_col_reduce<0>(y, ldy, nullptr, nullptr, rows, C, 0.f, nullptr, ws, st);
  SUG_LAUNCH_CHECK("sug_col_stats");
  hipLaunchKernelGGL(reduce_partials_kernel, dim3(sug_divup(2 * C, 16)), dim3(256), 0, st, ws, grid, 2 * C, stats);
  SUG_LAUNCH_CHECK("sug_col_stats(reduce)");
  return SUG_OK;
}

extern "C" int sug_col_stats_bn(const float* y, int64_t ldy, int64_t rows, int C, const float* gamma,
                                const float* beta, float eps, float momentum, float* running_mean,
                                float* running_var, float* coef, float* ws, void* stream) {
  SUG_REQUIRE(y && gamma && beta && coef && ws, "sug_col_stats_bn: null pointer");
  SUG_REQUIRE(rows > 0 && C > 0 && C <= 4096 && ldy >= C, "sug_col_stats_bn: bad shape");
  hipStream_t st = (hipStream_t)stream;
  const int grid = launch_col_reduce<0>(y, ldy, nullptr, nullptr, rows, C, 0.f, nullptr, ws, st, 1, 1);
  SUG_LAUNCH_CHECK("sug_col_stats_bn");
  hipLaunchKernelGGL(stats_finalize_kernel, dim3(sug_divup(C, 8)), dim3(256), 0, st, ws, grid, C, gamma, beta,
                     (double)rows, eps, momentum, running_mean, running_var, coef, ws + SUG_PIVOT_OFFSET(C));
  SUG_LAUNCH_CHECK("sug_col_stats_bn(finalize)");
  return SUG_OK;
}

int sug_col_stats_bn_groups(const float* y, int64_t ldy, int64_t rows, int C, int groups, const float* gamma,
                            const float* beta, float eps, float momentum, float* running_mean, float* running_var,
                            float* coef, float* ws, hipStream_t st) {
  const int grid = launch_col_reduce<0>(y, ldy, nullptr, nullptr, rows, C, 0.f, nullptr, ws, st, groups, 1);
  if (grid < 0) return 1;
  SUG_LAUNCH_CHECK("sug_bn_act_rows_fwd(stats)");
  hipLaunchKernelGGL(stats_finalize_groups_kernel, dim3(sug_divup(C, 8)), dim3(1024), 0, st, ws, grid, C, groups, gamma, beta,
                     (double)rows, eps, momentum, running_mean, running_var, coef, ws + SUG_PIVOT_OFFSET(C));
  SUG_LAUNCH_CHECK("sug_bn_act_rows_fwd(finalize)");
  return SUG_OK;
}
int sug_affine_act_groups(const float* z, int64_t ldz, const float* coef, int64_t rows, int groups, int C, float slope,
                          float* out, int64_t ldo, hipStream_t st) {
  const bool vec = (C % 4 == 0) && (ldz % 4 == 0) && (ldo % 4 == 0) && ((uintptr_t)z % 16 == 0) &&
                   ((uintptr_t)out % 16 == 0) && ((uintptr_t)coef % 16 == 0);
  if (!vec) return 1;
  const int64_t total = rows * groups * (C / 4);
  int64_t g = (total + 1023) / 1024;
  if (g > 8192) g = 8192;
  if (g < 1) g = 1;
  hipLaunchKernelGGL(affine_act_vec4_groups_kernel, dim3((int)g), dim3(256), 0, st, z, ldz, coef, rows * groups, rows, C,
                     slope, out, ldo);
  SUG_LAUNCH_CHECK("sug_bn_act_rows_fwd(act)");
  return SUG_OK;
}
int sug_bwd_reduce_groups(const float* gout, int64_t ldg, const float* z, const float* coef, int64_t rows, int Co,
                          int groups, float slope, float* a, double* red, float* ws, hipStream_t st, float* dgb) {
  const int grid = a ? launch_col_reduce<1>(gout, ldg, z, coef, rows, Co, slope, a, ws, st, groups)
                     : launch_col_reduce<2>(gout, ldg, z, coef, rows, Co, slope, nullptr, ws, st, groups);
  if (grid < 0) return 1;
  SUG_LAUNCH_CHECK("sug_edgeconv_bwd_reduce");
  if (dgb)
    hipLaunchKernelGGL(reduce_partials_fold_kernel, dim3(sug_divup(2 * Co, 16)), dim3(256), 0, st, ws, grid, 2 * Co, groups, red, dgb);
  else
    hipLaunchKernelGGL(reduce_partials_kernel, dim3(sug_divup(2 * Co, 16), groups), dim3(256), 0, st, ws, grid, 2 * Co, red);
  SUG_LAUNCH_CHECK("sug_edgeconv_bwd_reduce(reduce)");
  return SUG_OK;
}

extern "C" int sug_edgeconv_bwd_reduce(const float* gout, int64_t ldg, const float* z, const float* coef,
                                       int64_t rows, int Co, float slope, float* a, double* red,
                                       float* ws, void* stream) {
  SUG_REQUIRE(gout && z && coef && a && red && ws, "sug_edgeconv_bwd_reduce: null pointer");
  SUG_REQUIRE(rows > 0 && Co > 0 && Co <= 4096 && ldg >= Co, "sug_edgeconv_bwd_reduce: bad shape");
  hipStream_t st = (hipStream_t)stream;
  const int grid = launch_col_reduce<1>(gout, ldg, z, coef, rows, Co, slope, a, ws, st);
  SUG_LAUNCH_CHECK("sug_edgeconv_bwd_reduce");
  hipLaunchKernelGGL(reduce_partials_kernel, dim3(sug_divup(2 * Co, 16)), dim3(256), 0, st, ws, grid, 2 * Co, red);
  SUG_LAUNCH_CHECK("sug_edgeconv_bwd_reduce(reduce)");
  return SUG_OK;
}

static int edgeconv_bwd_scatter_groups(const float* a, const uint8_t* arg, const float* s1, const float* pq,
                                       int64_t ldpq, const int32_t* rev_off, const int32_t* rev_ent, const float* coef,
                                       const double* red, int B, int N, int k, int Co, int groups, int64_t coef_stride,
                                       int64_t red_stride, float* dpq, int64_t lddpq, void* stream);

extern "C" int sug_edgeconv_bwd_scatter(const float* a, const uint8_t* arg, const float* s1,
                                        const float* pq, int64_t ldpq, const int32_t* rev_off,
                                        const int32_t* rev_ent, const float* coef, const double* red,
                                        int B, int N, int k, int Co, float* dpq, int64_t lddpq,
                                        void* stream) {
// ... 94 lines not shown
```

sug_amd/csrc/layers.cpp:

```cpp
#include <stdint.h>
#include "../../include/sug_amd.h"

void sug_set_error(const char* fmt, ...);
struct ihipStream_t;
int sug_col_stats_bn_groups(const float* y, int64_t ldy, int64_t rows, int C, int groups, const float* gamma,
                            const float* beta, float eps, float momentum, float* running_mean, float* running_var,
                            float* coef, float* ws, ihipStream_t* st);
int sug_affine_act_groups(const float* z, int64_t ldz, const float* coef, int64_t rows, int groups, int C, float slope,
                          float* out, int64_t ldo, ihipStream_t* st);
int sug_bwd_reduce_groups(const float* gout, int64_t ldg, const float* z, const float* coef, int64_t rows, int Co,
                          int groups, float slope, float* a, double* red, float* ws, ihipStream_t* st, float* dgb);
int sug_bn_bwd_apply_groups(const float* a, int64_t lda, int from_g, float slope, const float* y, int64_t ldy,
                            const float* coef, const double* red, int64_t rows_g, int groups, int C, float* dy,
                            int64_t lddy, ihipStream_t* st);
int sug_edgeconv_fwd_bn_act_groups(const float* pq, int64_t ldpq, const int32_t* idx, const float* gamma,
                                   const float* beta, int B, int N, int k, int Co, int groups, float eps, float momentum,
                                   float slope, float* running_mean, float* running_var, float* z, uint8_t* arg,
                                   float* s1, float* coef, float* out, int64_t ldo, float* ws, void* stream);
int sug_edgeconv_bwd_scatter_groups(const float* a, const uint8_t* arg, const float* s1, const float* pq, int64_t ldpq,
                                    const int32_t* rev_off, const int32_t* rev_ent, const float* coef, const double* red,
                                    int B, int N, int k, int Co, int groups, int64_t coef_stride, int64_t red_stride,
                                    float* dpq, int64_t lddpq, void* stream);
#define LAYER_REQUIRE(cond, ...) do { if (!(cond)) { sug_set_error(__VA_ARGS__); return SUG_ERR_ARG; } } while (0)
#define LAYER_TRY(call) do { const int rc_ = (call); if (rc_ != SUG_OK) return rc_; } while (0)

extern "C" int sug_edgeconv_layer_fwd(const float* pq, int64_t ldpq, const int32_t* idx, const float* gamma,
                                      const float* beta, int B, int N, int k, int Co, int groups, int training,
                                      float eps, float momentum, float slope, float* running_mean,
                                      float* running_var, float* z, uint8_t* arg, float* s1, float* coef,
                                      float* out, int64_t ldo, double* stats, float* ws, void* stream) {
  LAYER_REQUIRE(groups >= 1 && B > 0 && B % groups == 0, "sug_edgeconv_layer_fwd: B=%d does not split into %d groups", B, groups);
  LAYER_REQUIRE(coef && out && z && arg && stats, "sug_edgeconv_layer_fwd: null pointer");
  const int Bg = B / groups;
  const int64_t rows = (int64_t)Bg * N;
  if (training)
    return sug_edgeconv_fwd_bn_act_groups(pq, ldpq, idx, gamma, beta, B, N, k, Co, groups, eps, momentum, slope, running_mean,
                                          running_var, z, arg, s1, coef, out, ldo, ws, stream);
  for (int g = 0; g < groups; ++g) {
    const int64_t r0 = (int64_t)g * rows;
    float* cg = coef + (int64_t)g * 5 * Co;
    LAYER_TRY(sug_edgeconv_fwd(pq + r0 * ldpq, ldpq, idx + r0 * k, gamma, Bg, N, k, Co, z + r0 * Co, arg + r0 * Co,
                               s1 ? s1 + r0 * Co : nullptr, stats, ws, stream));
    LAYER_TRY(sug_affine_act(z + r0 * Co, Co, cg, rows, Co, slope, out + r0 * ldo, ldo, stream));
  }
  return SUG_OK;
}

extern "C" int sug_edgeconv_layer_bwd(const float* gout, int64_t ldg, const float* z, const uint8_t* arg,
                                      const float* s1, const float* pq, int64_t ldpq, const int32_t* idx,
                                      const float* coef, int B, int N, int k, int Co, int groups, int training,
                                      float slope, float* a, double* red, int32_t* rev_off, int32_t* rev_ent,
                                      float* dpq, int64_t lddpq, float* ws, float* dgb, void* stream) {
  LAYER_REQUIRE(groups >= 1 && B > 0 && B % groups == 0, "sug_edgeconv_layer_bwd: B=%d does not split into %d groups", B, groups);
  LAYER_REQUIRE(red && a && rev_off && rev_ent, "sug_edgeconv_layer_bwd: null pointer");
  const int Bg = B / groups;
  const int64_t rows = (int64_t)Bg * N;
  LAYER_TRY(sug_knn_reverse(idx, B, N, k, rev_off, rev_ent, stream));
  int grouped = 1;
  if (groups > 1) {
    grouped = sug_bwd_reduce_groups(gout, ldg, z, coef, rows, Co, groups, slope, a, red, ws, (ihipStream_t*)stream, dgb);
    if (grouped < 0) return grouped;
  }
  for (int g = 0; grouped != 0 && g < groups; ++g) {
    const int64_t r0 = (int64_t)g * rows;
    const float* cg = coef + (int64_t)g * 5 * Co;
    double* rg = red + (int64_t)g * 2 * Co;
    LAYER_TRY(sug_edgeconv_bwd_reduce(gout + r0 * ldg, ldg, z + r0 * Co, cg, rows, Co, slope, a + r0 * Co, rg, ws, stream));
// ... 82 lines not shown
  bool applied = false;
  if (reduced && training) {
    const int rc = sug_bn_bwd_apply_groups(a, C, 0, slope, y, C, coef, red, rg, groups, C, dy, C, st);
    if (rc < 0) return rc;
    applied = rc == 0;
  }
  for (int g = 0; g < groups; ++g) {
    const float* cg = coef + (int64_t)g * 5 * C;
    double* rd = red + (int64_t)g * 2 * C;
    if (!reduced)
      LAYER_TRY(sug_edgeconv_bwd_reduce(gout + g * rg * ldg, ldg, y + g * rg * C, cg, rg, C, slope, a + g * rg * C, rd, ws,
                                        stream));
    if (training && !applied)
      LAYER_TRY(sug_bn_bwd_apply(a + g * rg * C, y + g * rg * C, C, cg, rd, rg, C, dy + g * rg * C, C, stream));
  }
  if (dgb && !reduced) LAYER_TRY(sug_fold_groups(red, groups, 2 * C, dgb, stream));
  return SUG_OK;
}

extern "C" int sug_bn_act_pool_layer_fwd(const float* y, int64_t ldy, int B, int N, int C, int groups,
                                         const float* gamma, const float* beta, int training, float eps,
                                         float momentum, float slope, float* running_mean, float* running_var,
                                         float* coef, float* out_max, float* out_mean, int64_t ld_pool, int32_t* arg, double* stats,
                                         float* ws_stats, float* ws_pool, void* stream) {
  LAYER_REQUIRE(groups >= 1 && B > 0 && B % groups == 0, "sug_bn_act_pool_layer_fwd: B=%d does not split into %d groups", B, groups);
  const int Bg = B / groups;
  const int64_t rg = (int64_t)Bg * N;
  for (int g = 0; g < groups; ++g) {
    float* cg = coef + (int64_t)g * 5 * C;
    const float* yg = y + g * rg * ldy;
    if (training)
      LAYER_TRY(sug_col_stats_bn(yg, ldy, rg, C, gamma, beta, eps, momentum, running_mean, running_var, cg, ws_stats,
                                 stream));
    LAYER_TRY(sug_bn_act_pool_fwd(yg, ldy, cg, Bg, N, C, slope, out_max + (int64_t)g * Bg * ld_pool, out_mean + (int64_t)g * Bg * ld_pool,
                                  ld_pool, arg + (int64_t)g * Bg * C, ws_pool, stream));
  }
  return SUG_OK;
}

extern "C" int sug_bn_act_pool_layer_bwd(const float* y, int64_t ldy, const float* coef, const float* gmax,
                                         const float* gmean, int64_t ld_pool, const int32_t* arg, int B, int N, int C, int groups,
                                         float slope, int training, double* red, float* ws, float* dy, int64_t lddy,
                                         float* dgb, void* stream) {
  LAYER_REQUIRE(groups >= 1 && B > 0 && B % groups == 0, "sug_bn_act_pool_layer_bwd: B=%d does not split into %d groups", B, groups);
  const int Bg = B / groups;
  const int64_t rg = (int64_t)Bg * N;
  for (int g = 0; g < groups; ++g)
    LAYER_TRY(sug_bn_act_pool_bwd(y + g * rg * ldy, ldy, coef + (int64_t)g * 5 * C, gmax + (int64_t)g * Bg * ld_pool,
                                  gmean + (int64_t)g * Bg * ld_pool, ld_pool, arg + (int64_t)g * Bg * C, Bg, N, C, slope, training,
                                  red + (int64_t)g * 2 * C, ws, dy + g * rg * lddy, lddy, stream));
  if (dgb) LAYER_TRY(sug_fold_groups(red, groups, 2 * C, dgb, stream));
  return SUG_OK;
}
```

sug_amd/csrc/mmd.hip:

```cpp
#include "common.h"

namespace {

constexpr int TI = 16;
constexpr int DK = 64;

__device__ __forceinline__ int global_row(int li, int m, int row0, int mloc) {
  return li < mloc ? row0 + li : m + row0 + (li - mloc);
}

__device__ __forceinline__ void pair_epilogue(int li, int i, int j, int m, float g, float ni, float nj,
                                              const float* __restrict__ w, const float* __restrict__ neg_gamma,
                                              int ns, float* __restrict__ wt, float& kxx, float& kyy, float& kxy) {
  const int M2 = 2 * m;
  {
    const float e = __fadd_rn(__fsub_rn(ni, __fmul_rn(2.0f, g)), nj);
    float K = 0.f, Kp = 0.f;
    for (int s = 0; s < ns; ++s) {
      const float ng = neg_gamma[s];
      const float t = expf(__fmul_rn(ng, e));
      K += t;
      Kp = fmaf(ng, t, Kp);
    }
    const float inv_m2 = 1.0f / ((float)m * (float)m);
// ... 125 lines not shown
  mmd_rbf_body(blockIdx.x, blockIdx.y, z, ldz, m, D, w, neg_gamma, ns, row0, mloc, sums, wt);
}
__global__ __launch_bounds__(256) void mmd_rbf_small_kernel(const float* __restrict__ z, int64_t ldz, int m, int D,
                                                            const float* __restrict__ w, const float* __restrict__ neg_gamma,
                                                            int ns, int row0, int mloc, double* __restrict__ sums,
                                                            float* __restrict__ wt) {
  mmd_rbf_small_body(blockIdx.x, blockIdx.y, z, ldz, m, D, w, neg_gamma, ns, row0, mloc, sums, wt);
}

#define SUG_MMD_MULTI 4
struct MmdTerm {
  const float* fs; const float* ft; int64_t lds, ldt;
  float* z; int D;
  float scale;
  const float* w; float* wt;
  const float* gscale; float* dz;
  int small;
};
struct MmdMulti {
  MmdTerm t[SUG_MMD_MULTI];
};

__global__ __launch_bounds__(256) void mmd_assemble_multi_kernel(MmdMulti a, int n, const int64_t* __restrict__ ls,
                                                                 const int64_t* __restrict__ lt, int m, int ncls,
                                                                 double* __restrict__ sums) {
  if (blockIdx.x == 0 && blockIdx.y == 0 && (int)threadIdx.x < 3 * n) sums[threadIdx.x] = 0.0;
  const MmdTerm& t = a.t[blockIdx.y];
  const int row = blockIdx.x, D = t.D;
  const float* src = row < m ? t.fs + (int64_t)row * t.lds : t.ft + (int64_t)(row - m) * t.ldt;
  const int64_t lab = row < m ? ls[row] : lt[row - m];
  float* dst = t.z + (int64_t)row * (D + ncls);
  for (int c = threadIdx.x; c < D; c += 256) dst[c] = src[c];
  for (int c = threadIdx.x; c < ncls; c += 256) dst[D + c] = (c == lab) ? t.scale : 0.f;
}

__global__ __launch_bounds__(256) void mmd_rbf_multi_kernel(MmdMulti a, int m, int ncls, const float* __restrict__ neg_gamma, int ns,
                                                            double* __restrict__ sums) {
  const MmdTerm& t = a.t[blockIdx.z];
  const int Dz = t.D + ncls;
  if (t.small) {
    mmd_rbf_small_body(blockIdx.x, blockIdx.y, t.z, Dz, m, Dz, t.w, neg_gamma, ns, 0, m, sums + 3 * blockIdx.z, t.wt);
  } else {
    const int nb = (2 * m + TI - 1) / TI;
    if ((int)blockIdx.x >= nb || (int)blockIdx.y >= nb) return;
    mmd_rbf_body(blockIdx.x, blockIdx.y, t.z, Dz, m, Dz, t.w, neg_gamma, ns, 0, m, sums + 3 * blockIdx.z, t.wt);
  }
}

__global__ void mmd_value_multi_kernel(const double* __restrict__ sums, int n, double mm, float* __restrict__ out) {
  const int i = threadIdx.x;
  if (i < n) out[i] = (float)((sums[3 * i] + sums[3 * i + 1] - 2.0 * sums[3 * i + 2]) / mm);
}

__global__ __launch_bounds__(256) void chamfer_dir_kernel(const float* __restrict__ a,
                                                          const float* __restrict__ bpts, int N, int M,
                                                          float* __restrict__ part) {
  extern __shared__ __attribute__((aligned(16))) float s_p[];
  const int b = blockIdx.y;
  const float* bb = bpts + (int64_t)b * M * 3;
  for (int e = threadIdx.x; e < M * 3; e += 256) s_p[(e / 3) * 4 + e % 3] = bb[e];
  __syncthreads();
  const int t = blockIdx.x * 256 + threadIdx.x;
  const int i = t >> 2, cl = t & 3;
  float best = INFINITY;
  if (i < N) {
    const float* p = a + ((int64_t)b * N + i) * 3;
    const float x = p[0], y = p[1], zc = p[2];
    float b0 = INFINITY, b1 = INFINITY;
    int j = cl;
    for (; j + 4 < M; j += 8) {
      const float4 c0 = *reinterpret_cast<const float4*>(s_p + 4 * j), c1 = *reinterpret_cast<const float4*>(s_p + 4 * j + 16);
      const float d0 = sq3(x - c0.x, y - c0.y, zc - c0.z), d1 = sq3(x - c1.x, y - c1.y, zc - c1.z);
      b0 = d0 < b0 ? d0 : b0;
      b1 = d1 < b1 ? d1 : b1;
    }
    for (; j < M; j += 4) {
      const float4 c = *reinterpret_cast<const float4*>(s_p + 4 * j);
      const float d = sq3(x - c.x, y - c.y, zc - c.z);
      b0 = d < b0 ? d : b0;
    }
    best = b1 < b0 ? b1 : b0;
  }
  {
    float o = __shfl_xor(best, 1);
    best = o < best ? o : best;
    o = __shfl_xor(best, 2);
    best = o < best ? o : best;
  }
  best = (cl == 0 && i < N) ? best : 0.f;
  __shared__ float s_w[256 / WAVE];
  const float s = wave_sum_f(best);
  if ((threadIdx.x & (WAVE - 1)) == 0) s_w[threadIdx.x / WAVE] = s;
  __syncthreads();
  if (threadIdx.x == 0) part[(int64_t)b * gridDim.x + blockIdx.x] = ((s_w[0] + s_w[1]) + s_w[2]) + s_w[3];
}

__global__ __launch_bounds__(256) void chamfer_fold_kernel(const float* __restrict__ pn, int nbn, const float* __restrict__ pm,
                                                           int nbm, int B, float inv_n, float inv_m, float* __restrict__ out) {
  const int b = blockIdx.x * 256 + threadIdx.x;
  if (b >= B) return;
  float sn = 0.f, sm = 0.f;
  for (int i = 0; i < nbn; ++i) sn += pn[(int64_t)b * nbn + i];
  for (int i = 0; i < nbm; ++i) sm += pm[(int64_t)b * nbm + i];
  out[b] = sn * inv_n + sm * inv_m;
}

__global__ __launch_bounds__(256) void chamfer_fold_weights_kernel(const float* __restrict__ pn, int nbn,
                                                                   const float* __restrict__ pm, int nbm, int B, float inv_n,
                                                                   float inv_m, int method, float* __restrict__ out) {
  __shared__ double s_red[4][2];
  const int lane = threadIdx.x & 63, wv = threadIdx.x >> 6;
  double dsum = 0.0, wsum = 0.0;
  for (int b = threadIdx.x; b < B; b += 256) {
    float sn = 0.f, sm = 0.f;
    for (int i = 0; i < nbn; ++i) sn += pn[(int64_t)b * nbn + i];
    for (int i = 0; i < nbm; ++i) sm += pm[(int64_t)b * nbm + i];
    const float dist = sn * inv_n + sm * inv_m;
    out[b] = dist;
    dsum += (double)dist;
    wsum += method == 1 ? (double)(1.f / (dist + 1e-8f)) : (method == 2 ? (double)expf(-dist) : 0.0);
  }
  dsum = wave_sum_d(dsum);
  wsum = wave_sum_d(wsum);
  if (lane == 0) { s_red[wv][0] = dsum; s_red[wv][1] = wsum; }
  __syncthreads();
  const double td = ((s_red[0][0] + s_red[1][0]) + s_red[2][0]) + s_red[3][0];
  const double tw = ((s_red[0][1] + s_red[1][1]) + s_red[2][1]) + s_red[3][1];
  const float mean = (float)(td / (double)B);
  const float scale = (float)(int)(1.f / mean);
  for (int b = threadIdx.x; b < B; b += 256) {
    const float dist = out[b];
    out[b] = method == 1 ? (1.f / (dist + 1e-8f)) / (float)tw : (method == 2 ? expf(-dist) / (float)tw : dist * scale);
  }
}


constexpr int JT = 128;
__device__ __forceinline__ void mmd_bwd_body(const int bx, const int by, const float* __restrict__ z, int64_t ldz,
                                             const float* __restrict__ wt, int m, int D, int row0, int mloc,
                                             const float* __restrict__ gscale, float gmul,
                                             float* __restrict__ dz, int64_t lddz) {
  __shared__ float s_z[JT * 64];
  __shared__ __attribute__((aligned(16))) float s_w[JT * 32];
  const int M2 = 2 * m, ML = 2 * mloc;
  const int c = threadIdx.x & 63, rg = threadIdx.x >> 6;
  const int d = bx * 64 + c;
  const int li0 = by * 32;
// ... 223 lines not shown
  } else {
    hipLaunchKernelGGL(mmd_rbf_kernel, dim3(sug_divup(2 * m, TI), sug_divup(2 * mloc, TI)), dim3(256), 0,
                       (hipStream_t)stream, z, ldz, m, D, w, neg_gamma, nsigma, row0, mloc, sums, wt);
  }
  SUG_LAUNCH_CHECK("sug_mmd_rbf");
  return SUG_OK;
}

extern "C" int sug_mmd_rbf(const float* z, int64_t ldz, int m, int D, const float* w,
                           const float* neg_gamma, int nsigma, double* sums, float* wt, void* stream) {
  return sug_mmd_rbf_rows(z, ldz, m, D, w, neg_gamma, nsigma, 0, m, sums, wt, stream);
}

namespace {
__global__ void mmd_value_kernel(const double* __restrict__ sums, double mm, float* __restrict__ out) {
  if (threadIdx.x == 0) out[0] = (float)((sums[0] + sums[1] - 2.0 * sums[2]) / mm);
}
__global__ void mmd_zero_sums_kernel(double* __restrict__ sums) {
  if (threadIdx.x < 3) sums[threadIdx.x] = 0.0;
}
}

extern "C" int sug_mmd_rbf_value(const float* z, int64_t ldz, int m, int D, const float* w, const float* neg_gamma,
                                 int nsigma, double* sums, float* wt, float* value, void* stream) {
  SUG_REQUIRE(sums && value, "sug_mmd_rbf_value: null pointer");
  hipStream_t st = (hipStream_t)stream;
  hipLaunchKernelGGL(mmd_zero_sums_kernel, dim3(1), dim3(64), 0, st, sums);
  const int rc = sug_mmd_rbf_rows(z, ldz, m, D, w, neg_gamma, nsigma, 0, m, sums, wt, stream);
  if (rc != SUG_OK) return rc;
  hipLaunchKernelGGL(mmd_value_kernel, dim3(1), dim3(64), 0, st, sums, (double)m * (double)m, value);
  SUG_LAUNCH_CHECK("sug_mmd_rbf_value");
  return SUG_OK;
}

extern "C" int64_t sug_chamfer_workspace(int B, int N, int M) {
  return (int64_t)B * (sug_divup(4 * (int64_t)N, 256) + sug_divup(4 * (int64_t)M, 256));
}

extern "C" int sug_chamfer(const float* a, const float* b, int B, int N, int M, float* out, float* ws,
                           void* stream) {
  SUG_REQUIRE(a && b && out && ws, "sug_chamfer: null pointer");
  SUG_REQUIRE(B > 0 && N > 0 && M > 0 && N <= 5000 && M <= 5000 && B <= 65535, "sug_chamfer: bad shape");
  hipStream_t st = (hipStream_t)stream;
  const int nbn = sug_divup(4 * N, 256), nbm = sug_divup(4 * M, 256);
  float* pm = ws + (int64_t)B * nbn;
  hipLaunchKernelGGL(chamfer_dir_kernel, dim3(nbn, B), dim3(256), (size_t)M * 4 * sizeof(float), st, a, b, N, M, ws);
  hipLaunchKernelGGL(chamfer_dir_kernel, dim3(nbm, B), dim3(256), (size_t)N * 4 * sizeof(float), st, b, a, M, N, pm);
  hipLaunchKernelGGL(chamfer_fold_kernel, dim3(sug_divup(B, 256)), dim3(256), 0, st, ws, nbn, pm, nbm, B, 1.0f / (float)N,
                     1.0f / (float)M, out);
  SUG_LAUNCH_CHECK("sug_chamfer");
  return SUG_OK;
}

extern "C" int sug_mmd_rbf_rows_bwd(const float* z, int64_t ldz, const float* wt, int m, int D, int row0, int mloc,
                                    const float* gscale, float gmul, float* dz, int64_t lddz, void* stream) {
  SUG_REQUIRE(z && wt && gscale && dz, "sug_mmd_rbf_bwd: null pointer");
  SUG_REQUIRE(m > 0 && D > 0 && ldz >= D && lddz >= D, "sug_mmd_rbf_bwd: bad shape");
  SUG_REQUIRE(row0 >= 0 && mloc > 0 && row0 + mloc <= m, "sug_mmd_rbf_bwd: row block outside 0..%d", m);
  hipLaunchKernelGGL(mmd_bwd_kernel, dim3(sug_divup(D, 64), sug_divup(2 * mloc, 32)), dim3(256), 0, (hipStream_t)stream, z,
                     ldz, wt, m, D, row0, mloc, gscale, gmul, dz, lddz);
  SUG_LAUNCH_CHECK("sug_mmd_rbf_bwd");
  return SUG_OK;
}

extern "C" int sug_mmd_rbf_bwd(const float* z, int64_t ldz, const float* wt, int m, int D, const float* gscale,
                               float* dz, int64_t lddz, void* stream) {
  return sug_mmd_rbf_rows_bwd(z, ldz, wt, m, D, 0, m, gscale, 1.0f, dz, lddz, stream);
}

extern "C" int sug_sda_prob_weights(const float* pred_s, int64_t lds, const float* pred_t, int64_t ldt,
                                    const int64_t* label_s, const int64_t* label_t, int m, int num_class,
                                    float label_weight, int method, float* weights, void* stream) {
  SUG_REQUIRE(pred_s && pred_t && label_s && label_t && weights, "sug_sda_prob_weights: null pointer");
  SUG_REQUIRE(m > 0 && num_class >= 2 && num_class <= SUG_SDA_MAX_CLASSES && lds >= num_class && ldt >= num_class,
              "sug_sda_prob_weights: bad shape (2..%d classes, rows at least that long; got %d classes, m=%d)",
              SUG_SDA_MAX_CLASSES, num_class, m);
  SUG_REQUIRE(method >= 0 && method <= 3, "sug_sda_prob_weights: unknown weighting method");
  if (num_class == 10)
    hipLaunchKernelGGL(sda_prob_weights_kernel, dim3(1), dim3(256), 0, (hipStream_t)stream, pred_s, lds, pred_t, ldt,
                       label_s, label_t, m, label_weight, method, weights);
  else
    hipLaunchKernelGGL(sda_prob_weights_rt_kernel, dim3(1), dim3(256), 0, (hipStream_t)stream, pred_s, lds, pred_t, ldt,
                       label_s, label_t, m, num_class, label_weight, method, weights);
  SUG_LAUNCH_CHECK("sug_sda_prob_weights");
  return SUG_OK;
}

namespace {

__global__ __launch_bounds__(256) void mmd_assemble_kernel(const float* __restrict__ fs, int64_t lds,
                                                           const float* __restrict__ ft, int64_t ldt,
                                                           const int64_t* __restrict__ ls, const int64_t* __restrict__ lt,
                                                           int m, int D, int ncls, float scale, float* __restrict__ z) {
  const int row = blockIdx.x;
  const float* src = row < m ? fs + (int64_t)row * lds : ft + (int64_t)(row - m) * ldt;
  const int64_t lab = row < m ? ls[row] : lt[row - m];
  float* dst = z + (int64_t)row * (D + ncls);
  for (int c = threadIdx.x; c < D; c += 256) dst[c] = src[c];
  for (int c = threadIdx.x; c < ncls; c += 256) dst[D + c] = (c == lab) ? scale : 0.f;
}

__global__ __launch_bounds__(256) void split_weight_kernel(const float* __restrict__ in, int Co, int C, int backward,
                                                           float* __restrict__ out) {
  const int e = blockIdx.x * 256 + threadIdx.x;
  if (e >= 2 * Co * C) return;
  if (!backward) {
// ... 142 lines not shown
  if (na == 0) return SUG_OK;
  for (int i = na; i < SUG_MMD_MULTI; ++i) a.t[i] = a.t[0];
  hipLaunchKernelGGL(mmd_bwd_multi_kernel, dim3(sug_divup(dmax, 64), sug_divup(2 * m, 32), na), dim3(256), 0,
                     (hipStream_t)stream, a, m, num_class);
  SUG_LAUNCH_CHECK("sug_soft_mmd_multi_bwd");
  return SUG_OK;
}

extern "C" int sug_sda_prob_weights_multi(int n, const void* const* pred_s, const int64_t* lds, const void* const* pred_t,
                                          const int64_t* ldt, const int64_t* label_s, const int64_t* label_t, int m,
                                          int num_class, float label_weight, int method, void* const* weights, void* stream) {
  SUG_REQUIRE(pred_s && lds && pred_t && ldt && label_s && label_t && weights, "sug_sda_prob_weights_multi: null pointer");
  SUG_REQUIRE(n >= 1 && n <= SUG_MMD_MULTI, "sug_sda_prob_weights_multi: %d heads (1..%d)", n, SUG_MMD_MULTI);
  SUG_REQUIRE(m > 0 && num_class >= 2 && num_class <= SUG_SDA_MAX_CLASSES,
              "sug_sda_prob_weights_multi: bad shape (2..%d classes; got %d classes, m=%d)", SUG_SDA_MAX_CLASSES, num_class, m);
  SUG_REQUIRE(method >= 0 && method <= 3, "sug_sda_prob_weights_multi: unknown weighting method");
  SdaMulti a;
  for (int i = 0; i < SUG_MMD_MULTI; ++i) {
    const int k = i < n ? i : 0;
    SUG_REQUIRE(pred_s[k] && pred_t[k] && weights[k] && lds[k] >= num_class && ldt[k] >= num_class,
                "sug_sda_prob_weights_multi: bad operand %d (rows of at least %d logits)", k, num_class);
    a.ps[i] = (const float*)pred_s[k];
    a.pt[i] = (const float*)pred_t[k];
    a.lds[i] = lds[k];
    a.ldt[i] = ldt[k];
    a.out[i] = (float*)weights[k];
  }
  if (num_class == 10)
    hipLaunchKernelGGL(sda_prob_weights_multi_kernel, dim3(n), dim3(256), 0, (hipStream_t)stream, a, label_s, label_t, m,
                       label_weight, method);
  else
    hipLaunchKernelGGL(sda_prob_weights_multi_rt_kernel, dim3(n), dim3(256), 0, (hipStream_t)stream, a, label_s, label_t, m,
                       num_class, label_weight, method);
  SUG_LAUNCH_CHECK("sug_sda_prob_weights_multi");
  return SUG_OK;
}

extern "C" int sug_chamfer_weights(const float* a, const float* b, int B, int N, int M, int method, float* out, float* ws,
                                   void* stream) {
  SUG_REQUIRE(a && b && out && ws, "sug_chamfer_weights: null pointer");
  SUG_REQUIRE(B > 0 && N > 0 && M > 0 && N <= 5000 && M <= 5000 && B <= 65535, "sug_chamfer_weights: bad shape");
  SUG_REQUIRE(method >= 1 && method <= 3, "sug_chamfer_weights: weighting method %d (1 naive_inverse, 2 exp_inverse, 3 mean2one)", method);
  hipStream_t st = (hipStream_t)stream;
  const int nbn = sug_divup(4 * N, 256), nbm = sug_divup(4 * M, 256);
  float* pm = ws + (int64_t)B * nbn;
  hipLaunchKernelGGL(chamfer_dir_kernel, dim3(nbn, B), dim3(256), (size_t)M * 4 * sizeof(float), st, a, b, N, M, ws);
  hipLaunchKernelGGL(chamfer_dir_kernel, dim3(nbm, B), dim3(256), (size_t)N * 4 * sizeof(float), st, b, a, M, N, pm);
  hipLaunchKernelGGL(chamfer_fold_weights_kernel, dim3(1), dim3(256), 0, st, ws, nbn, pm, nbm, B, 1.0f / (float)N,
                     1.0f / (float)M, method, out);
  SUG_LAUNCH_CHECK("sug_chamfer_weights");
  return SUG_OK;
}

namespace {

constexpr int SEL_MAX_M = SUG_CLASS_MMD_MAX_ROWS, SEL_MAX_CLASSES = SUG_CLASS_MMD_MAX_CLASSES, SEL_MAX_D = SUG_CLASS_MMD_MAX_D;

__global__ __launch_bounds__(256) void mmd_select_kernel(const int64_t* __restrict__ ls, const int64_t* __restrict__ lt, int m,
                                                         int num_class, int mode, int* __restrict__ idx_s,
                                                         int* __restrict__ idx_t, int* __restrict__ pos_s,
                                                         int* __restrict__ pos_t, int* __restrict__ count) {
  __shared__ short s_ks[SEL_MAX_M], s_kt[SEL_MAX_M];
  __shared__ int s_k[SEL_MAX_CLASSES], s_off[SEL_MAX_CLASSES + 1];
  const int nc = mode == 0 ? 1 : num_class;
  for (int i = threadIdx.x; i < m; i += 256) {
    const int64_t a = ls[i], b = lt[i];
    if (mode == 0) {
      s_ks[i] = s_kt[i] = (a == b) ? 0 : -1;
    } else {
      s_ks[i] = (a >= 0 && a < num_class) ? (short)a : (short)-1;
      s_kt[i] = (b >= 0 && b < num_class) ? (short)b : (short)-1;
    }
  }
  __syncthreads();
  if ((int)threadIdx.x < nc) {
    const int c = threadIdx.x;
    int a = 0, b = 0;
    for (int j = 0; j < m; ++j) {
      a += s_ks[j] == c;
      b += s_kt[j] == c;
    }
    s_k[c] = a < b ? a : b;
  }
  __syncthreads();
  if (threadIdx.x == 0) {
    int o = 0;
    for (int c = 0; c < nc; ++c) {
      s_off[c] = o;
      o += s_k[c];
    }
    s_off[nc] = o;
    count[0] = o;
  }
  __syncthreads();
  const int n = s_off[nc];
  for (int i = threadIdx.x; i < m; i += 256) {
    if (i >= n) idx_s[i] = idx_t[i] = -1;
  }
  for (int i = threadIdx.x; i < m; i += 256) {
    const int cs = s_ks[i], ct = s_kt[i];
    int rs = 0, rt = 0;
    for (int j = 0; j < i; ++j) {
      rs += s_ks[j] == cs;
      rt += s_kt[j] == ct;
    }
    const int ps = (cs >= 0 && rs < s_k[cs]) ? s_off[cs] + rs : -1;
// ... 121 lines not shown
```

sug_amd/ops.py:

```python
import contextlib
import ctypes
import math
import os as _os

import torch

from ._lib import lib, check, STATS_BLOCKS, CONSTANTS as _H

class StepContext:
    __slots__ = ('bn_groups', 'start_queue', 'start_provider', 'geometry_plan', 'profile', 'profile_only', 'parallel_branches',
                 'fused_heads', 'w16_cache', 'bn_record', 'pending_counts')

    def __init__(self):
        self.bn_groups = 1
        self.start_queue = self.start_provider = self.geometry_plan = None
        self.profile = self.profile_only = None
        self.parallel_branches = False
        self.fused_heads = False
        self.w16_cache = self.bn_record = self.pending_counts = None

    @contextlib.contextmanager
    def scoped(self, **fields):
        old = {k: getattr(self, k) for k in fields}
        for k, v in fields.items():
# ... 1100 lines not shown
def record_bn_stats():
    with CTX.scoped(bn_record=[]):
        yield CTX.bn_record


def _record_bn(bn, coef):
    if CTX.bn_record is not None and bn.training and bn.track_running_stats:
        CTX.bn_record.append((bn, coef))


def replay_bn_stats(rec):
    rec = list(rec)
    i = 0
    while i < len(rec):
        run, seen = [], set()
        while i < len(rec) and len(run) < 16 and id(rec[i][0]) not in seen:
            seen.add(id(rec[i][0]))
            run.append(rec[i])
            i += 1
        if len(run) == 1:
            bn_replay(*run[0])
            continue
        c3s = []
        for _, coef in run:
            c3 = coef if coef.dim() == 3 else coef.unsqueeze(0)
            c3s.append(c3 if c3.is_contiguous() else c3.contiguous())
        n = len(run)
        I32, F32 = ctypes.c_int32 * n, ctypes.c_float * n
        check(lib().sug_bn_replay_multi(n, _ptrs(c3s), I32(*[c.shape[0] for c in c3s]), I32(*[c.shape[2] for c in c3s]),
                                        F32(*[float(bn.momentum) for bn, _ in run]), _ptrs([bn.running_mean for bn, _ in run]),
                                        _ptrs([bn.running_var for bn, _ in run]), _st()), 'sug_bn_replay_multi')
        for (bn, _), c3 in zip(run, c3s):
            _count_bn_call(bn, c3.shape[0])


def bn_replay(bn, coef):
    c3 = coef if coef.dim() == 3 else coef.unsqueeze(0)
    c3 = c3 if c3.is_contiguous() else c3.contiguous()
    G, _, C = c3.shape
    check(lib().sug_bn_replay(_p(c3), G, C, float(bn.momentum), _p(bn.running_mean), _p(bn.running_var), _st()),
          'sug_bn_replay')
    _count_bn_call(bn, G)


def bn_act_rows(y, bn, slope, pre=None):
    if pre is not None:
        return _BNActRows.apply(y, bn.weight, bn.bias, _bn_state(bn), slope, pre)[0]
    _count_bn_call(bn)
    out, coef = _BNActRows.apply(y, bn.weight, bn.bias, _bn_state(bn), slope)
    _record_bn(bn, coef)
    return out


class _BNActPool(torch.autograd.Function):

    @staticmethod
    def forward(ctx, y, gamma, beta, st, slope):
        _need_gpu(y, gamma)
        y, B, N, C, ld = _rows3(y)
        G = st.G
        _check_groups('bn_act_pool', B, 'clouds', G)
        dev = y.device
        g, b, coef = _bn_params(gamma, beta, st, C)
        pooled = torch.empty(B, 2 * C, dtype=torch.float32, device=dev)
        omax, omean = pooled[:, :C], pooled[:, C:]
        arg = torch.empty(B, C, dtype=torch.int32, device=dev)
        stats = torch.empty(2 * C, dtype=torch.float64, device=dev)
        wss = _stats_ws(C, dev)
        wsp = torch.empty(12 * (B // G) * C, dtype=torch.float32, device=dev)
        check(lib().sug_bn_act_pool_layer_fwd(_p(y), ld, B, N, C, G, _p(g), _p(b), st.train, st.eps, st.momentum,
                                              float(slope), _p(st.mean), _p(st.var), _p(coef), _p(omax),
                                              _p(omean), 2 * C, _p(arg), _p(stats), _p(wss), _p(wsp), _st()),
              'sug_bn_act_pool_layer_fwd')
        ctx.save_for_backward(y, coef, arg)
        ctx.meta = (B, N, C, ld, float(slope), st.train, G)
        return pooled

    @staticmethod
    def backward(ctx, g):
        y, coef, arg = ctx.saved_tensors
        B, N, C, ld, slope, train, G = ctx.meta
        dev = y.device
        if g.stride(1) != 1 or g.stride(0) < 2 * C:
            g = g.contiguous()
        gmax, gmean, ldp = g[:, :C], g[:, C:], g.stride(0)
        red = torch.empty(G, 2 * C, dtype=torch.float64, device=dev)
        ws = _stats_ws(C, dev)
        dy = torch.empty(B, N, C, dtype=torch.float32, device=dev)
        rf = torch.empty(2 * C, dtype=torch.float32, device=dev)
        check(lib().sug_bn_act_pool_layer_bwd(_p(y), ld, _p(coef), _p(gmax), _p(gmean), ldp, _p(arg), B, N, C, G, slope,
                                              train, _p(red), _p(ws), _p(dy), C, _p(rf), _st()),
              'sug_bn_act_pool_layer_bwd')
        return (dy,) + _dgamma_dbeta(rf) + (None, None)


def bn_update_stats(y, bn):
    if not bn.training:
        return
    _need_gpu(y)
    C = y.shape[-1]
    y2 = y.detach().reshape(-1, C)
    if y2.stride(1) != 1:
        y2 = y2.contiguous()
    rows, G = y2.shape[0], CTX.bn_groups
    _check_groups('bn_update_stats', rows, 'rows', G)
    rg = rows // G
    g, b = bn.weight.detach().contiguous(), bn.bias.detach().contiguous()
    coef = torch.empty(5, C, dtype=torch.float32, device=y.device)
    ws = _stats_ws(C, y.device)
    for i in range(G):
        yi = y2[i * rg:(i + 1) * rg]
        check(lib().sug_col_stats_bn(_p(yi), yi.stride(0), rg, C, _p(g), _p(b), bn.eps, bn.momentum,
                                     _p(bn.running_mean), _p(bn.running_var), _p(coef), _p(ws), _st()),
              'sug_col_stats_bn')
    _count_bn_call(bn)


def bn_act_pool_cat(y, bn, slope):
    _count_bn_call(bn)
    return _BNActPool.apply(y, bn.weight, bn.bias, _bn_state(bn), slope)


def bn_act_pool(y, bn, slope):
    C = y.shape[-1]
    pooled = bn_act_pool_cat(y, bn, slope)
    return pooled[:, :C], pooled[:, C:]


def _edgeconv_out(out_holder, B, N, Co, dev):
    if out_holder is None:
        return torch.empty(B, N, Co, dtype=torch.float32, device=dev)
    out = out_holder[0]
    if tuple(out.shape) != (B, N, Co) or out.stride(2) != 1 or out.stride(0) != N * out.stride(1) \
            or out.dtype != torch.float32 or out.requires_grad:
        raise RuntimeError('edgeconv: bad destination slice')
    return out


def _edgeconv_backward(gout, z, arg, s1, pq, ldpq, idx, coef, B, N, k, Co, G, slope, train):
    dev = gout.device
    gout, _, _, _, ldg = _rows3(gout)
    a = torch.empty(B, N, Co, dtype=torch.float32, device=dev)
    red = (torch.empty if train else torch.zeros)(G + 1, 2 * Co, dtype=torch.float64, device=dev)
    ws = _stats_ws(Co, dev)
    off = torch.empty(B, N + 1, dtype=torch.int32, device=dev)
    ent = torch.empty(B, N * k, dtype=torch.int32, device=dev)
    dpq = torch.empty(B, N, 2 * Co, dtype=torch.float32, device=dev)
    rf = torch.empty(2 * Co, dtype=torch.float32, device=dev)
    check(_timed('edgeconv_layer_bwd_Co%d' % Co, {'B': B, 'N': N, 'k': k, 'Co': Co},
                 lambda: lib().sug_edgeconv_layer_bwd(_p(gout), ldg, _p(z), _p(arg), _p(s1), _p(pq), ldpq, _p(idx),
                                                      _p(coef), B, N, k, Co, G, train, slope, _p(a),
                                                      _p(red), _p(off), _p(ent), _p(dpq), 2 * Co, _p(ws), _p(rf), _st())),
          'sug_edgeconv_layer_bwd')
    return (dpq,) + _dgamma_dbeta(rf)


class _EdgeConv(torch.autograd.Function):

    @staticmethod
    def forward(ctx, pq, idx, gamma, beta, st, slope, out_holder, grad_on=True):
# ... 514 lines not shown
        return mixed

    @staticmethod
    def backward(ctx, g):
        xyz, nbr, vf, w1c, b1c, w2l, wg1l, wg2l, T0, delta, U, T1, Lg, mx, sm, mixed = ctx.saved_tensors
        B, n, k, d, code, scale = ctx.meta
        dev, lo = g.device, T0.dtype
        L_ = lib()
        g = g.contiguous().float()
        if code == 1:
            s, inv = _grad_scale16(g)
            g = g * s
        off, ent = knn_reverse(nbr)
        dL, da = torch.empty_like(Lg), torch.empty_like(Lg)
        dv = torch.empty(B, n, d, dtype=torch.float32, device=dev)
        f32 = torch.float32
        R = B * n * k
        cws = torch.empty(L_.sug_ptran_colsum_workspace(R), dtype=f32, device=dev)
        dbg2, dbg1, db2 = (torch.empty(d, dtype=f32, device=dev) for _ in range(3))
        shp = {'B': B, 'N': n, 'k': k, 'd': d, 'e': 4 if code == 0 else 2}
        check(_timed('ptran_attn_bwd_n%d' % n, shp, lambda: L_.sug_ptran_attn_bwd(_p(g), _p(mixed), _p(Lg), _p(delta), _p(vf), _p(nbr), _p(mx),
                                                                          _p(sm), _p(off), _p(ent), B, n, k, d, code, scale, _p(dL),
                                                                          _p(da), _p(dv), _p(dbg2), _p(cws), _st())),
              'sug_ptran_attn_bwd')

        dwg2 = _dweight(dL, T1)
        dT1 = dL @ wg2l
        check(L_.sug_ptran_relu_bwd_db(_p(dT1), _p(T1), R, d, code, _p(dbg1), _p(cws), _st()), 'sug_ptran_relu_bwd_db')
        dwg1 = _dweight(dT1, U)
        dU = dT1 @ wg1l
        dq, dk = torch.empty_like(dv), torch.empty_like(dv)
        check(_timed('ptran_qk_bwd_n%d' % n, shp, lambda: L_.sug_ptran_qk_bwd(_p(dU), _p(da), _p(off), _p(ent), B, n, k, d, code, _p(dq), _p(dk),
                                                                      _p(db2), _p(cws), _st())), 'sug_ptran_qk_bwd')
        ddelta = da
        dw2 = _dweight(ddelta, T0)
        dT0 = ddelta @ w2l
        dw1 = torch.empty(d, 3, dtype=f32, device=dev)
        db1 = torch.empty(d, dtype=f32, device=dev)
        ws = torch.empty(1024 * 4 * d, dtype=f32, device=dev)
        check(L_.sug_ptran_pos1_bwd(_p(dT0), _p(xyz), _p(nbr), _p(w1c), _p(b1c), B, n, k, d, code, _p(dw1), _p(db1), _p(ws),
                                    _st()), 'sug_ptran_pos1_bwd')
        if code == 1:
            torch._foreach_mul_([dq, dk, dv, dw1, db1, dw2, db2, dwg1, dbg1, dwg2, dbg2], inv)
        return None, None, dq, dk, dv, dw1, db1, dw2, db2, dwg1, dbg1, dwg2, dbg2, None


def ptran_attention(xyz, nbr, q, kf, vf, fc_delta, fc_gamma, dtype=None):
    return _PTranAttention.apply(xyz, nbr, q, kf, vf, fc_delta[0].weight, fc_delta[0].bias, fc_delta[2].weight,
                                 fc_delta[2].bias, fc_gamma[0].weight, fc_gamma[0].bias, fc_gamma[2].weight,
                                 fc_gamma[2].bias, dtype)


CALAYER_FUSED = _os.environ.get('SUG_CALAYER_FUSED', '1') != '0'


def calayer_supported(layers, x):
    if not (CALAYER_FUSED and x.is_cuda and x.dtype == torch.float32 and x.dim() == 2 and CTX.bn_groups == 1):
        return False
    if x.shape[0] % len(layers):
        return False
    M, C = x.shape[0] // len(layers), x.shape[1]
    for m in layers:
        c0, c2, bn = m.conv_du[0], m.conv_du[2], m.bn
        if c0.weight.shape[1] != C or c2.weight.shape[0] != C or c0.bias is None or c2.bias is None or not bn.affine \
                or not (bn.training or bn.track_running_stats) or bn.momentum is None or not bn.track_running_stats:
            return False
        if any(mm.training != layers[0].training for mm in (m, bn)):
            return False
    return bool(lib().sug_calayer_supported(len(layers), M, C, layers[0].conv_du[0].weight.shape[0]))


class _CALayers(torch.autograd.Function):

    @staticmethod
    def forward(ctx, x, nl, training, eps, momentum, *params):
        _need_gpu(x)
        x = x if (x.stride(1) == 1 and x.stride(0) % 4 == 0 and x.data_ptr() % 16 == 0) else x.contiguous()
        M, C = x.shape[0] // nl, x.shape[1]
        P = [params[8 * a:8 * a + 8] for a in range(nl)]
        W0 = [p[0].detach().reshape(p[0].shape[0], -1).contiguous() for p in P]
        W2 = [p[2].detach().reshape(p[2].shape[0], -1).contiguous() for p in P]
        b0, b2 = [p[1].detach().contiguous() for p in P], [p[3].detach().contiguous() for p in P]
        gam, bet = [p[4].detach().contiguous() for p in P], [p[5].detach().contiguous() for p in P]
        Hd = W0[0].shape[0]
        dev = x.device
        L = lib()
        hp = torch.empty(nl, C // 512, M, Hd, dtype=torch.float32, device=dev)
        h = torch.empty(nl, M, Hd, dtype=torch.float32, device=dev)
        z = torch.empty(nl * M, C, dtype=torch.float32, device=dev)
        check(L.sug_calayer_fwd(nl, _p(x), x.stride(0), M, C, Hd, _ptrs(W0), _ptrs(b0), _ptrs(W2), _ptrs(b2), _p(hp), _p(h), _p(z),
                                _st()), 'sug_calayer_fwd')
        out = torch.empty(nl * M, C, dtype=torch.float32, device=dev)
        stat = torch.empty(nl, 2, C, dtype=torch.float32, device=dev)
        xc = x if x.stride(0) == C else x.contiguous()
        for a in range(nl):
            check(L.sug_gate_bn_fwd(_p(xc[a * M:]), _p(z[a * M:]), M, C, _p(gam[a]), _p(bet[a]), _p(P[a][6]), _p(P[a][7]),
                                    1 if training else 0, float(eps), float(momentum), _p(out[a * M:]), _p(stat[a]), _st()),
                  'sug_gate_bn_fwd')
        ctx.save_for_backward(xc, h, z, stat, *W0, *W2, *gam)
        ctx.meta = (nl, M, C, Hd, bool(training))
        return out

    @staticmethod
    def backward(ctx, g):
        nl, M, C, Hd, training = ctx.meta
        sv = ctx.saved_tensors
        x, h, z, stat = sv[:4]
        W0, W2, gam = sv[4:4 + nl], sv[4 + nl:4 + 2 * nl], sv[4 + 2 * nl:4 + 3 * nl]
        dev = x.device
        L = lib()
        g = g.contiguous()
        dxg, dz = torch.empty_like(x), torch.empty_like(x)
        dgb = torch.empty(nl, 2, C, dtype=torch.float32, device=dev)
        for a in range(nl):
            check(L.sug_gate_bn_bwd(_p(g[a * M:]), _p(x[a * M:]), _p(z[a * M:]), M, C, _p(gam[a]), _p(stat[a]), 1 if training else 0,
                                    _p(dxg[a * M:]), _p(dz[a * M:]), _p(dgb[a, 0]), _p(dgb[a, 1]), _st()), 'sug_gate_bn_bwd')
        f32 = torch.float32
        dW0 = [torch.empty(Hd, C, dtype=f32, device=dev) for _ in range(nl)]
        dW2 = [torch.empty(C, Hd, dtype=f32, device=dev) for _ in range(nl)]
        db0 = [torch.empty(Hd, dtype=f32, device=dev) for _ in range(nl)]
        db2 = [torch.empty(C, dtype=f32, device=dev) for _ in range(nl)]
        dhp = torch.empty(nl, C // 32, M, Hd, dtype=f32, device=dev)
        dh = torch.empty(nl, M, Hd, dtype=f32, device=dev)
        dx = torch.empty(nl * M, C, dtype=f32, device=dev)
        check(L.sug_calayer_bwd(nl, _p(x), x.stride(0), M, C, Hd, _ptrs(W0), _ptrs(W2), _p(h), _p(dz), _p(dxg), _ptrs(dW0), _ptrs(db0),
                                _ptrs(dW2), _ptrs(db2), _p(dhp), _p(dh), _p(dx), C, _st()), 'sug_calayer_bwd')
        grads = []
        for a in range(nl):
            grads += [dW0[a].view(Hd, C, 1, 1), db0[a], dW2[a].view(C, Hd, 1, 1), db2[a], dgb[a, 0], dgb[a, 1], None, None]
        return (dx, None, None, None, None) + tuple(grads)


def calayers(layers, x):
    params = []
    for m in layers:
        _count_bn_call(m.bn)
        c0, c2 = m.conv_du[0], m.conv_du[2]
        params += [c0.weight, c0.bias, c2.weight, c2.bias, m.bn.weight, m.bn.bias, m.bn.running_mean, m.bn.running_var]
    bn = layers[0].bn
    return _CALayers.apply(x, len(layers), bn.training, bn.eps, bn.momentum, *params)


_rows_cache = [None, None, None]


def clear_rows_cache():
    _rows_cache[0] = _rows_cache[1] = _rows_cache[2] = None


def cloud_rows(x):
    import weakref
    ref, ver, rows = _rows_cache
    if ref is not None and ref() is x and ver == x._version and not x.requires_grad:
        return rows
    rows = x.squeeze(-1).transpose(1, 2).contiguous()
    if not x.requires_grad and not torch.is_inference_mode_enabled():
        _rows_cache[0], _rows_cache[1], _rows_cache[2] = weakref.ref(x), x._version, rows
    return rows


class _CEPair(torch.autograd.Function):

    @staticmethod
    def forward(ctx, y1, y2, label, w, ignore_index=-100):
        _need_gpu(y1, y2, label)
        M, C = label.shape[0], y1.shape[1]
        a = y1 if y1.stride(1) == 1 else y1.contiguous()
# ... 1122 lines not shown
SDA_MAX_CLASSES = _H['SUG_SDA_MAX_CLASSES']


def _sda_num_class(*preds):
    C = int(preds[0].shape[-1])
    if any(int(p.shape[-1]) != C for p in preds):
        raise RuntimeError('sda_prob_weights: logits of one width (got %s)' % sorted({int(p.shape[-1]) for p in preds}))
    return C


def sda_prob_weights(pred_s, pred_t, label_s, label_t, label_weight, method):
    _need_gpu(pred_s, pred_t, label_s, label_t)
    if method not in _SDA_METHODS:
        raise RuntimeError('Not supported weighting method %s' % method)
    C = _sda_num_class(pred_s, pred_t)
    ps = pred_s.detach().reshape(-1, C).float()
    pt = pred_t.detach().reshape(-1, C).float()
    ps = ps if ps.stride(1) == 1 else ps.contiguous()
    pt = pt if pt.stride(1) == 1 else pt.contiguous()
    ls, lt = label_s.reshape(-1).long().contiguous(), label_t.reshape(-1).long().contiguous()
    m = ps.shape[0]
    out = torch.empty(m, dtype=torch.float32, device=ps.device)
    check(lib().sug_sda_prob_weights(_p(ps), ps.stride(0), _p(pt), pt.stride(0), _p(ls), _p(lt), m, C,
                                     float(label_weight), _SDA_METHODS[method], _p(out), _st()),
          'sug_sda_prob_weights')
    return out


def sda_prob_weights_multi(preds, label_s, label_t, label_weight, method):
    preds = list(preds)
    if len(preds) == 1:
        return [sda_prob_weights(preds[0][0], preds[0][1], label_s, label_t, label_weight, method)]
    if len(preds) > 4:
        return sda_prob_weights_multi(preds[:4], label_s, label_t, label_weight, method) + \
            sda_prob_weights_multi(preds[4:], label_s, label_t, label_weight, method)
    if method not in _SDA_METHODS:
        raise RuntimeError('Not supported weighting method %s' % method)
    C = _sda_num_class(*[t for pr in preds for t in pr])
    rows = lambda p: (lambda q: q if q.stride(1) == 1 else q.contiguous())(p.detach().reshape(-1, C).float())
    ps, pt = [rows(a) for a, _ in preds], [rows(b) for _, b in preds]
    _need_gpu(label_s, label_t, *(ps + pt))
    ls, lt = label_s.reshape(-1).long().contiguous(), label_t.reshape(-1).long().contiguous()
    m, n = ps[0].shape[0], len(preds)
    if any(t.shape[0] != m for t in ps + pt):
        raise RuntimeError('sda_prob_weights_multi: one batch size for all heads')
    outs = [torch.empty(m, dtype=torch.float32, device=ps[0].device) for _ in range(n)]
    I64 = ctypes.c_int64 * n
    check(lib().sug_sda_prob_weights_multi(n, _ptrs(ps), I64(*[t.stride(0) for t in ps]), _ptrs(pt), I64(*[t.stride(0) for t in pt]),
                                           _p(ls), _p(lt), m, C, float(label_weight), _SDA_METHODS[method], _ptrs(outs), _st()),
          'sug_sda_prob_weights_multi')
    return outs


def chamfer(a, b):
    _need_gpu(a, b)
    a, b = a.detach().contiguous(), b.detach().contiguous()
    B, N, _ = a.shape
    M = b.shape[1]
    out = torch.empty(B, dtype=torch.float32, device=a.device)
    ws = torch.empty(lib().sug_chamfer_workspace(B, N, M), dtype=torch.float32, device=a.device)
    check(lib().sug_chamfer(_p(a), _p(b), B, N, M, _p(out), _p(ws), _st()), 'sug_chamfer')
    return out


def chamfer_weights(a, b, method):
    _need_gpu(a, b)
    if method not in ('naive_inverse', 'exp_inverse', 'mean2one'):
        raise RuntimeError('Not supported weighting method %s' % method)
    a, b = a.detach().contiguous(), b.detach().contiguous()
    B, N, _ = a.shape
    M = b.shape[1]
    out = torch.empty(B, dtype=torch.float32, device=a.device)
    ws = torch.empty(lib().sug_chamfer_workspace(B, N, M), dtype=torch.float32, device=a.device)
    check(lib().sug_chamfer_weights(_p(a), _p(b), B, N, M, _SDA_METHODS[method], _p(out), _p(ws), _st()), 'sug_chamfer_weights')
    return out


CHAMFER_MAX_POINTS = _H['SUG_CHAMFER_MAX_POINTS']


class _ChamferNN(torch.autograd.Function):
    @staticmethod
    def forward(ctx, a, b):
        a, b = a.contiguous(), b.contiguous()
        B, N, _ = a.shape
        M = b.shape[1]
        dist1 = torch.empty(B, N, dtype=torch.float32, device=a.device)
        dist2 = torch.empty(B, M, dtype=torch.float32, device=a.device)
        idx1 = torch.empty(B, N, dtype=torch.int32, device=a.device)
        idx2 = torch.empty(B, M, dtype=torch.int32, device=a.device)
        check(lib().sug_chamfer_nn(_p(a), _p(b), B, N, M, _p(dist1), _p(dist2), _p(idx1), _p(idx2), _st()), 'sug_chamfer_nn')
        ctx.save_for_backward(a, b, idx1, idx2)
        ctx.mark_non_differentiable(idx1, idx2)
        return dist1, dist2, idx1, idx2

    @staticmethod
    @torch.autograd.function.once_differentiable
    def backward(ctx, g1, g2, _gi1, _gi2):
        a, b, idx1, idx2 = ctx.saved_tensors
        B, N, _ = a.shape
        M = b.shape[1]
        ga = torch.empty_like(a) if ctx.needs_input_grad[0] else None
        gb = torch.empty_like(b) if ctx.needs_input_grad[1] else None
        check(lib().sug_chamfer_nn_bwd(_p(g1.contiguous()), _p(g2.contiguous()), _p(a), _p(b), _p(idx1), _p(idx2), B, N, M,
                                       _p(ga), _p(gb), _st()), 'sug_chamfer_nn_bwd')
        return ga, gb


def chamfer_nn(a, b):
    _need_gpu(a, b)
    if a.dtype != torch.float32 or b.dtype != torch.float32:
        raise RuntimeError('chamfer_nn: fp32 clouds only (got %s, %s)' % (a.dtype, b.dtype))
    if a.dim() != 3 or b.dim() != 3 or a.shape[2] != 3 or b.shape[2] != 3:
        raise RuntimeError('chamfer_nn: clouds are rows [B,N,3] and [B,M,3] (got %s, %s)' % (tuple(a.shape), tuple(b.shape)))
    if a.shape[0] != b.shape[0]:
        raise RuntimeError('chamfer_nn: %d clouds against %d: the clouds are paired' % (a.shape[0], b.shape[0]))
    return _ChamferNN.apply(a, b)


KPCONV_MAX_CLOUD = _H['SUG_KPCONV_MAX_CLOUD']


def kp_grid_subsample(pts, off, B, cap, dl):
    _need_gpu(pts, off)
    pts = pts.detach().contiguous()
    pad = torch.empty(B, cap, 3, dtype=torch.float32, device=pts.device)
    cnt = torch.empty(B, dtype=torch.int32, device=pts.device)
# ... 438 lines not shown
```

Before: 13860.

## Batch grouped BN-pool, gate-BN layers, group stats and chamfer directions into single launches

Adds grouped variants of the BN+activation+pool forward and backward that handle all BN groups in one launch by offsetting coef/red per batch group. Also adds a multi-layer gate-BN forward/backward, an exact grouped column-stats BN update, and merged chamfer kernels that compute both directions in one launch. All are enabled by default through environment flags. The aim is to cut per-group and per-layer kernel launches and Python loop overhead, at the cost of larger workspaces and new code paths.

```diff
diff --git a/include/sug_amd.h b/include/sug_amd.h
--- a/include/sug_amd.h
+++ b/include/sug_amd.h
@@ -84,6 +84,9 @@
 int sug_col_stats_bn_grouped(const float* y, int64_t ldy, int64_t rows, int C, int groups, const float* gamma,
                              const float* beta, float eps, float momentum, float* running_mean, float* running_var,
                              float* coef, float* ws, void* stream);
+int sug_col_stats_bn_groups_exact(const float* y, int64_t ldy, int64_t rows, int C, int groups, const float* gamma,
+                                  const float* beta, float eps, float momentum, float* running_mean, float* running_var,
+                                  float* coef, float* ws, void* stream);
 
 int sug_bn_replay(const float* coef, int G, int C, float momentum, float* running_mean, float* running_var,
                   void* stream);
@@ -121,6 +124,12 @@
                     float* stat, void* stream);
 int sug_gate_bn_bwd(const float* g, const float* x, const float* z, int M, int C, const float* gamma, const float* stat,
                     int training, float* dx, float* dz, float* dgamma, float* dbeta, void* stream);
+int sug_gate_bn_fwd_multi(int layers, const float* x, const float* z, int M, int C, const void* const* gamma,
+                          const void* const* beta, void* const* running_mean, void* const* running_var, int training,
+                          float eps, float momentum, float* out, float* stat, void* stream);
+int sug_gate_bn_bwd_multi(int layers, const float* g, const float* x, const float* z, int M, int C,
+                          const void* const* gamma, const float* stat, int training, float* dx, float* dz, float* dgb,
+                          void* stream);
 
 int sug_calayer_supported(int layers, int M, int C, int Hd);
 int sug_calayer_fwd(int layers, const float* x, int64_t ldx, int M, int C, int Hd, const float* const* W0,
@@ -251,6 +260,15 @@
                               const float* gmean, int64_t ld_pool, const int32_t* arg, int B, int N, int C, int groups,
                               float slope, int training, double* red, float* ws, float* dy, int64_t lddy,
                               float* dgb, void* stream);
+int sug_bn_act_pool_groups_fwd(const float* y, int64_t ldy, int B, int N, int C, int groups,
+                               const float* gamma, const float* beta, int training, float eps, float momentum,
+                               float slope, float* running_mean, float* running_var, float* coef,
+                               float* out_max, float* out_mean, int64_t ld_pool, int32_t* arg, double* stats, float* ws_stats,
+                               float* ws_pool, void* stream);
+int sug_bn_act_pool_groups_bwd(const float* y, int64_t ldy, const float* coef, const float* gmax,
+                               const float* gmean, int64_t ld_pool, const int32_t* arg, int B, int N, int C, int groups,
+                               float slope, int training, double* red, float* ws, float* dy, int64_t lddy,
+                               float* dgb, void* stream);
 
 int sug_pointmlp_max_fwd(const float* x, int64_t ldx, int64_t rows, int K, const float* w, const float* bias,
                          const float* gamma, int Co, int seg, float* zext, int32_t* arg, float* ws, int* nblk,
@@ -380,6 +398,9 @@
 int64_t sug_chamfer_workspace(int B, int N, int M);
 int sug_chamfer(const float* a, const float* b, int B, int N, int M, float* out, float* ws, void* stream);
 int sug_chamfer_weights(const float* a, const float* b, int B, int N, int M, int method, float* out, float* ws, void* stream);
+int sug_chamfer_merged(const float* a, const float* b, int B, int N, int M, float* out, float* ws, void* stream);
+int sug_chamfer_weights_merged(const float* a, const float* b, int B, int N, int M, int method, float* out, float* ws,
+                               void* stream);
 #define SUG_CHAMFER_MAX_POINTS 5000
 int sug_chamfer_nn(const float* a, const float* b, int B, int N, int M, float* dist1, float* dist2, int32_t* idx1, int32_t* idx2,
                    void* stream);
diff --git a/sug_amd/csrc/bnpool.hip b/sug_amd/csrc/bnpool.hip
--- a/sug_amd/csrc/bnpool.hip
+++ b/sug_amd/csrc/bnpool.hip
@@ -86,7 +86,7 @@
 
 template <int VEC>
 __global__ __launch_bounds__(256) void bn_act_pool_part_kernel(const float* __restrict__ y, int64_t ldy,
-                                                               const float* __restrict__ coef, int N,
+                                                               const float* __restrict__ coef, int Bg, int N,
                                                                int C, float slope,
                                                                float* __restrict__ pmax,
                                                                float* __restrict__ psum,
@@ -96,6 +96,7 @@
   __shared__ float s_s[LY][64];
   __shared__ int s_a[LY][64];
   const int b = blockIdx.y, ch = blockIdx.z;
+  coef += (int64_t)(b / Bg) * 5 * C;
   const int lx = threadIdx.x % LX, ly = threadIdx.x / LX;
   const int c = blockIdx.x * 64 + lx * VEC;
   const int n0 = (int)((int64_t)N * ch / NS), n1 = (int)((int64_t)N * (ch + 1) / NS);
@@ -173,12 +174,13 @@
                                                               const float* __restrict__ coef,
                                                               const float* __restrict__ gmax,
                                                               const float* __restrict__ gmean, int64_t ldp,
-                                                              const int32_t* __restrict__ arg, int N,
+                                                              const int32_t* __restrict__ arg, int Bg, int N,
                                                               int C, float slope, float* __restrict__ ws) {
   constexpr int LX = 64 / VEC, LY = 256 / LX;
   __shared__ float s_g[LY][64];
   __shared__ float s_x[LY][64];
   const int b = blockIdx.y, ch = blockIdx.z;
+  coef += (int64_t)(b / Bg) * 5 * C;
   const int lx = threadIdx.x % LX, ly = threadIdx.x / LX;
   const int c = blockIdx.x * 64 + lx * VEC;
   const int n0 = (int)((int64_t)N * ch / NS), n1 = (int)((int64_t)N * (ch + 1) / NS);
@@ -276,11 +278,13 @@
                                                                   const double* __restrict__ red,
                                                                   const float* __restrict__ gmax,
                                                                   const float* __restrict__ gmean, int64_t ldp,
-                                                                  const int32_t* __restrict__ arg, int N, int C,
+                                                                  const int32_t* __restrict__ arg, int Bg, int N, int C,
                                                                   int rows_per_block, float slope, float invM,
-                                                                  float* __restrict__ dy, int64_t lddy) {
+                                                                  float* __restrict__ dy, int64_t lddy, int last_first) {
   const int CV = C >> 2;
-  const int b = blockIdx.y;
+  const int b = last_first ? gridDim.y - 1 - blockIdx.y : blockIdx.y;
+  coef += (int64_t)(b / Bg) * 5 * C;
+  red += (int64_t)(b / Bg) * 2 * C;
   const int cg = threadIdx.x % CV, rl = threadIdx.x / CV, rstep = 256 / CV;
   const int c = cg * 4;
   float sc[4], sh[4], mu[4], rs[4], r0[4], r1[4], gme[4], gmx[4];
@@ -491,9 +495,9 @@
   int32_t* parg = reinterpret_cast<int32_t*>(ws + 2 * part);
   dim3 grid(sug_divup(C, 64), B, NS);
   if (vec4_ok(y, ldy, C))
-    hipLaunchKernelGGL((bn_act_pool_part_kernel<4>), grid, dim3(256), 0, st, y, ldy, coef, N, C, slope, pmax, psum, parg);
+    hipLaunchKernelGGL((bn_act_pool_part_kernel<4>), grid, dim3(256), 0, st, y, ldy, coef, B, N, C, slope, pmax, psum, parg);
   else
-    hipLaunchKernelGGL((bn_act_pool_part_kernel<1>), grid, dim3(256), 0, st, y, ldy, coef, N, C, slope, pmax, psum, parg);
+    hipLaunchKernelGGL((bn_act_pool_part_kernel<1>), grid, dim3(256), 0, st, y, ldy, coef, B, N, C, slope, pmax, psum, parg);
   SUG_LAUNCH_CHECK("sug_bn_act_pool_fwd");
   hipLaunchKernelGGL(pool_combine_kernel, dim3(sug_divup((int64_t)B * C, 256)), dim3(256), 0, st, pmax, psum, parg,
                      B, N, C, out_max, out_mean, ld_pool, arg);
@@ -512,9 +516,9 @@
   const bool vec = vec4_ok(y, ldy, C) && vec4_ok(dy, lddy, C);
   dim3 grid(sug_divup(C, 64), B, NS);
   if (vec)
-    hipLaunchKernelGGL((pool_bwd_reduce_kernel<4>), grid, dim3(256), 0, st, y, ldy, coef, gmax, gmean, ld_pool, arg, N, C, slope, ws);
+    hipLaunchKernelGGL((pool_bwd_reduce_kernel<4>), grid, dim3(256), 0, st, y, ldy, coef, gmax, gmean, ld_pool, arg, B, N, C, slope, ws);
   else
-    hipLaunchKernelGGL((pool_bwd_reduce_kernel<1>), grid, dim3(256), 0, st, y, ldy, coef, gmax, gmean, ld_pool, arg, N, C, slope, ws);
+    hipLaunchKernelGGL((pool_bwd_reduce_kernel<1>), grid, dim3(256), 0, st, y, ldy, coef, gmax, gmean, ld_pool, arg, B, N, C, slope, ws);
   SUG_LAUNCH_CHECK("sug_bn_act_pool_bwd(reduce)");
   hipLaunchKernelGGL(reduce_rows_kernel, dim3(sug_divup(2 * C, 16)), dim3(256), 0, st, ws, B * NS, 2 * C, red);
   SUG_LAUNCH_CHECK("sug_bn_act_pool_bwd(combine)");
@@ -522,7 +526,7 @@
   if (vec && (C / 4) <= 256 && 256 % (C / 4) == 0 && B <= 65535) {
     const int rpb = 64 > 256 / (C / 4) ? 64 : 256 / (C / 4);
     hipLaunchKernelGGL(pool_bwd_apply_rows_kernel, dim3(sug_divup(N, rpb), B), dim3(256), 0, st, y, ldy, coef, red, gmax,
-                       gmean, ld_pool, arg, N, C, rpb, slope, invM, dy, lddy);
+                       gmean, ld_pool, arg, B, N, C, rpb, slope, invM, dy, lddy, 0);
   } else if (vec)
     hipLaunchKernelGGL((pool_bwd_apply_kernel<4>), dim3(ew_grid((int64_t)B * N * C / 4)), dim3(256), 0, st, y, ldy,
                        coef, red, gmax, gmean, ld_pool, arg, B, N, C, slope, invM, dy, lddy);
@@ -533,6 +537,70 @@
   return SUG_OK;
 }
 
+namespace {
+__global__ __launch_bounds__(256) void reduce_rows_groups_kernel(const float* __restrict__ ws, int nrow, int W, int groups,
+                                                                 double* __restrict__ out, float* __restrict__ dgb) {
+  __shared__ double s_p[16][17];
+  const int cl = threadIdx.x & 15, p = threadIdx.x >> 4;
+  const int c = blockIdx.x * 16 + cl;
+  const int gfirst = blockIdx.y, glast = (blockIdx.y == 0 && dgb) ? groups : gfirst + 1;
+  double fold = 0.0;
+  for (int g = gfirst; g < glast; ++g) {
+    const float* wg = ws + (size_t)g * nrow * W;
+    double acc = 0.0;
+    if (c < W)
+      for (int b = p; b < nrow; b += 16) acc += (double)wg[(size_t)b * W + c];
+    __syncthreads();
+    s_p[p][cl] = acc;
+    __syncthreads();
+    if (p == 0 && c < W) {
+      double t = 0.0;
+#pragma unroll
+      for (int i = 0; i < 16; ++i) t += s_p[i][cl];
+      if (g == gfirst) out[(size_t)g * W + c] = t;
+      fold += t;
+    }
+  }
+  if (blockIdx.y == 0 && dgb && p == 0 && c < W) dgb[c] = (float)fold;
+}
+}
+
+int sug_bn_act_pool_fwd_groups(const float* y, int64_t ldy, const float* coef, int B, int groups, int N, int C, float slope,
+                               float* out_max, float* out_mean, int64_t ld_pool, int32_t* arg, float* ws, hipStream_t st) {
+  if (!vec4_ok(y, ldy, C) || B > 65535) return 1;
+  const size_t part = (size_t)B * NS * C;
+  float* pmax = ws;
+  float* psum = ws + part;
+  int32_t* parg = reinterpret_cast<int32_t*>(ws + 2 * part);
+  hipLaunchKernelGGL((bn_act_pool_part_kernel<4>), dim3(sug_divup(C, 64), B, NS), dim3(256), 0, st, y, ldy, coef, B / groups, N, C,
+                     slope, pmax, psum, parg);
+  SUG_LAUNCH_CHECK("sug_bn_act_pool_groups_fwd");
+  hipLaunchKernelGGL(pool_combine_kernel, dim3(sug_divup((int64_t)B * C, 256)), dim3(256), 0, st, pmax, psum, parg,
+                     B, N, C, out_max, out_mean, ld_pool, arg);
+  SUG_LAUNCH_CHECK("sug_bn_act_pool_groups_fwd(combine)");
+  return SUG_OK;
+}
+
+int sug_bn_act_pool_bwd_groups(const float* y, int64_t ldy, const float* coef, const float* gmax, const float* gmean,
+                               int64_t ld_pool, const int32_t* arg, int B, int groups, int N, int C, float slope, double* red,
+                               float* ws, float* dy, int64_t lddy, float* dgb, hipStream_t st) {
+  if (!(vec4_ok(y, ldy, C) && vec4_ok(dy, lddy, C) && (C / 4) <= 256 && 256 % (C / 4) == 0 && B <= 65535 &&
+        B * NS <= SUG_STATS_BLOCKS))
+    return 1;
+  const int Bg = B / groups;
+  hipLaunchKernelGGL((pool_bwd_reduce_kernel<4>), dim3(sug_divup(C, 64), B, NS), dim3(256), 0, st, y, ldy, coef, gmax, gmean,
+                     ld_pool, arg, Bg, N, C, slope, ws);
+  SUG_LAUNCH_CHECK("sug_bn_act_pool_groups_bwd(reduce)");
+  hipLaunchKernelGGL(reduce_rows_groups_kernel, dim3(sug_divup(2 * C, 16), groups), dim3(256), 0, st, ws, Bg * NS, 2 * C, groups,
+                     red, dgb);
+  SUG_LAUNCH_CHECK("sug_bn_act_pool_groups_bwd(combine)");
+  const float invM = (float)(1.0 / ((double)Bg * N));
+  const int rpb = 64 > 256 / (C / 4) ? 64 : 256 / (C / 4);
+  hipLaunchKernelGGL(pool_bwd_apply_rows_kernel, dim3(sug_divup(N, rpb), B), dim3(256), 0, st, y, ldy, coef, red, gmax, gmean,
+                     ld_pool, arg, Bg, N, C, rpb, slope, invM, dy, lddy, 1);
+  SUG_LAUNCH_CHECK("sug_bn_act_pool_groups_bwd(apply)");
+  return SUG_OK;
+}
 
 namespace {
 __global__ __launch_bounds__(256) void fold_groups_kernel(const double* __restrict__ red, int groups, int n,
@@ -622,6 +690,67 @@
 }
 
 template <int MR>
+__device__ __forceinline__ void gate_bn_fwd_body(const int c, const float* __restrict__ x, const float* __restrict__ z, int M, int C,
+                                                 const float* __restrict__ gamma, const float* __restrict__ beta,
+                                                 float* __restrict__ rmean, float* __restrict__ rvar, int training,
+                                                 float eps, float momentum, float* __restrict__ out,
+                                                 float* __restrict__ stat) {
+  float gv[MR > 0 ? MR : 1];
+  if constexpr (MR > 0) {
+    float xv[MR], zv[MR];
+#pragma unroll
+    for (int i = 0; i < MR; ++i) {
+      const int r = i < M ? i : M - 1;
+      xv[i] = x[(int64_t)r * C + c];
+      zv[i] = z[(int64_t)r * C + c];
+    }
+#pragma unroll
+    for (int i = 0; i < MR; ++i) gv[i] = gate_val(xv[i], zv[i]);
+  }
+  auto g_at = [&](int i) { if constexpr (MR > 0) return gv[i]; else return gate_val(x[(int64_t)i * C + c], z[(int64_t)i * C + c]); };
+  float mean, invstd;
+  if (training) {
+    float s = 0.f;
+    if constexpr (MR > 0) {
+#pragma unroll
+      for (int i = 0; i < MR; ++i) s += i < M ? gv[i] : 0.f;
+    } else {
+#pragma unroll 8
+      for (int i = 0; i < M; ++i) s += g_at(i);
+    }
+    mean = s / (float)M;
+    float q = 0.f;
+    if constexpr (MR > 0) {
+#pragma unroll
+      for (int i = 0; i < MR; ++i) { const float d = gv[i] - mean; q = i < M ? fmaf(d, d, q) : q; }
+    } else {
+#pragma unroll 8
+      for (int i = 0; i < M; ++i) { const float d = g_at(i) - mean; q = fmaf(d, d, q); }
+    }
+    const float var = q / (float)M;
+    invstd = 1.0f / sqrtf(var + eps);
+    if (rmean) {
+      rmean[c] = (1.0f - momentum) * rmean[c] + momentum * mean;
+      rvar[c] = (1.0f - momentum) * rvar[c] + momentum * (M > 1 ? q / (float)(M - 1) : var);
+    }
+  } else {
+    mean = rmean[c];
+    invstd = 1.0f / sqrtf(rvar[c] + eps);
+  }
+  stat[c] = mean;
+  stat[C + c] = invstd;
+  const float sc = gamma[c] * invstd, sh = beta[c] - mean * sc;
+  if constexpr (MR > 0) {
+#pragma unroll
+    for (int i = 0; i < MR; ++i)
+      if (i < M) out[(int64_t)i * C + c] = fmaf(gv[i], sc, sh);
+  } else {
+#pragma unroll 8
+    for (int i = 0; i < M; ++i) out[(int64_t)i * C + c] = fmaf(g_at(i), sc, sh);
+  }
+}
+
+template <int MR>
 __global__ __launch_bounds__(64) void gate_bn_fwd_kernel(const float* __restrict__ x, const float* __restrict__ z, int M, int C,
                                                          const float* __restrict__ gamma, const float* __restrict__ beta,
                                                          float* __restrict__ rmean, float* __restrict__ rvar, int training,
@@ -629,69 +758,34 @@
                                                          float* __restrict__ stat) {
   const int c = blockIdx.x * 64 + threadIdx.x;
   if (c >= C) return;
-  float gv[MR > 0 ? MR : 1];
-  if constexpr (MR > 0) {
-    float xv[MR], zv[MR];
-#pragma unroll
-    for (int i = 0; i < MR; ++i) {
-      const int r = i < M ? i : M - 1;
-      xv[i] = x[(int64_t)r * C + c];
-      zv[i] = z[(int64_t)r * C + c];
-    }
-#pragma unroll
-    for (int i = 0; i < MR; ++i) gv[i] = gate_val(xv[i], zv[i]);
-  }
-  auto g_at = [&](int i) { if constexpr (MR > 0) return gv[i]; else return gate_val(x[(int64_t)i * C + c], z[(int64_t)i * C + c]); };
-  float mean, invstd;
-  if (training) {
-    float s = 0.f;
-    if constexpr (MR > 0) {
-#pragma unroll
-      for (int i = 0; i < MR; ++i) s += i < M ? gv[i] : 0.f;
-    } else {
-#pragma unroll 8
-      for (int i = 0; i < M; ++i) s += g_at(i);
-    }
-    mean = s / (float)M;
-    float q = 0.f;
-    if constexpr (MR > 0) {
-#pragma unroll
-      for (int i = 0; i < MR; ++i) { const float d = gv[i] - mean; q = i < M ? fmaf(d, d, q) : q; }
-    } else {
-#pragma unroll 8
-      for (int i = 0; i < M; ++i) { const float d = g_at(i) - mean; q = fmaf(d, d, q); }
-    }
-    const float var = q / (float)M;
-    invstd = 1.0f / sqrtf(var + eps);
-    if (rmean) {
-      rmean[c] = (1.0f - momentum) * rmean[c] + momentum * mean;
-      rvar[c] = (1.0f - momentum) * rvar[c] + momentum * (M > 1 ? q / (float)(M - 1) : var);
-    }
-  } else {
-    mean = rmean[c];
-    invstd = 1.0f / sqrtf(rvar[c] + eps);
-  }
-  stat[c] = mean;
-  stat[C + c] = invstd;
-  const float sc = gamma[c] * invstd, sh = beta[c] - mean * sc;
-  if constexpr (MR > 0) {
-#pragma unroll
-    for (int i = 0; i < MR; ++i)
-      if (i < M) out[(int64_t)i * C + c] = fmaf(gv[i], sc, sh);
-  } else {
-#pragma unroll 8
-    for (int i = 0; i < M; ++i) out[(int64_t)i * C + c] = fmaf(g_at(i), sc, sh);
-  }
-}
+  gate_bn_fwd_body<MR>(c, x, z, M, C, gamma, beta, rmean, rvar, training, eps, momentum, out, stat);
+}
+
+#define SUG_GATE_BN_MULTI 4
+struct GateBNMulti {
+  const float* gamma[SUG_GATE_BN_MULTI];
+  const float* beta[SUG_GATE_BN_MULTI];
+  float* rmean[SUG_GATE_BN_MULTI];
+  float* rvar[SUG_GATE_BN_MULTI];
+};
 
 template <int MR>
-__global__ __launch_bounds__(64) void gate_bn_bwd_kernel(const float* __restrict__ g, const float* __restrict__ x,
-                                                         const float* __restrict__ z, int M, int C,
-                                                         const float* __restrict__ gamma, const float* __restrict__ stat,
-                                                         int training, float* __restrict__ dx, float* __restrict__ dz,
-                                                         float* __restrict__ dgamma, float* __restrict__ dbeta) {
-  const int c = blockIdx.x * 64 + threadIdx.x;
+__global__ __launch_bounds__(64) void gate_bn_fwd_multi_kernel(const float* __restrict__ x, const float* __restrict__ z, int M, int C,
+                                                               GateBNMulti t, int training, float eps, float momentum,
+                                                               float* __restrict__ out, float* __restrict__ stat) {
+  const int c = blockIdx.x * 64 + threadIdx.x, l = blockIdx.y;
   if (c >= C) return;
+  const int64_t o = (int64_t)l * M * C;
+  gate_bn_fwd_body<MR>(c, x + o, z + o, M, C, t.gamma[l], t.beta[l], t.rmean[l], t.rvar[l], training, eps, momentum, out + o,
+                       stat + (int64_t)l * 2 * C);
+}
+
+template <int MR>
+__device__ __forceinline__ void gate_bn_bwd_body(const int c, const float* __restrict__ g, const float* __restrict__ x,
+                                                 const float* __restrict__ z, int M, int C,
+                                                 const float* __restrict__ gamma, const float* __restrict__ stat,
+                                                 int training, float* __restrict__ dx, float* __restrict__ dz,
+                                                 float* __restrict__ dgamma, float* __restrict__ dbeta) {
   const float mean = stat[c], invstd = stat[C + c];
   float sb = 0.f, sg = 0.f;
   float xr[MR > 0 ? MR : 1], sr[MR > 0 ? MR : 1], hr[MR > 0 ? MR : 1], gr[MR > 0 ? MR : 1];
@@ -745,6 +839,30 @@
       dz[(int64_t)i * C + c] = __fmul_rn(__fmul_rn(dg, xv), __fmul_rn(__fsub_rn(1.0f, s), s));
     }
   }
+}
+
+template <int MR>
+__global__ __launch_bounds__(64) void gate_bn_bwd_kernel(const float* __restrict__ g, const float* __restrict__ x,
+                                                         const float* __restrict__ z, int M, int C,
+                                                         const float* __restrict__ gamma, const float* __restrict__ stat,
+                                                         int training, float* __restrict__ dx, float* __restrict__ dz,
+                                                         float* __restrict__ dgamma, float* __restrict__ dbeta) {
+  const int c = blockIdx.x * 64 + threadIdx.x;
+  if (c >= C) return;
+  gate_bn_bwd_body<MR>(c, g, x, z, M, C, gamma, stat, training, dx, dz, dgamma, dbeta);
+}
+
+template <int MR>
+__global__ __launch_bounds__(64) void gate_bn_bwd_multi_kernel(const float* __restrict__ g, const float* __restrict__ x,
+                                                               const float* __restrict__ z, int M, int C, GateBNMulti t,
+                                                               const float* __restrict__ stat, int training,
+                                                               float* __restrict__ dx, float* __restrict__ dz,
+                                                               float* __restrict__ dgb) {
+  const int c = blockIdx.x * 64 + threadIdx.x, l = blockIdx.y;
+  if (c >= C) return;
+  const int64_t o = (int64_t)l * M * C;
+  gate_bn_bwd_body<MR>(c, g + o, x + o, z + o, M, C, t.gamma[l], stat + (int64_t)l * 2 * C, training, dx + o, dz + o,
+                       dgb + (int64_t)l * 2 * C, dgb + (int64_t)l * 2 * C + C);
 }
 
 }
@@ -781,6 +899,62 @@
   return SUG_OK;
 }
 
+extern "C" int sug_gate_bn_fwd_multi(int layers, const float* x, const float* z, int M, int C, const void* const* gamma,
+                                     const void* const* beta, void* const* running_mean, void* const* running_var, int training,
+                                     float eps, float momentum, float* out, float* stat, void* stream) {
+  SUG_REQUIRE(x && z && gamma && beta && out && stat, "sug_gate_bn_fwd_multi: null pointer");
+  SUG_REQUIRE(layers >= 1 && layers <= SUG_GATE_BN_MULTI, "sug_gate_bn_fwd_multi: %d layers (1..%d)", layers, SUG_GATE_BN_MULTI);
+  SUG_REQUIRE(M >= 1 && M <= 1024 && C >= 1, "sug_gate_bn_fwd_multi: bad shape M=%d C=%d", M, C);
+  GateBNMulti t;
+  for (int i = 0; i < SUG_GATE_BN_MULTI; ++i) {
+    const int k = i < layers ? i : 0;
+    float* rm = running_mean ? (float*)running_mean[k] : nullptr;
+    float* rv = running_var ? (float*)running_var[k] : nullptr;
+    SUG_REQUIRE(gamma[k] && beta[k], "sug_gate_bn_fwd_multi: null parameter of layer %d", k);
+    SUG_REQUIRE(training || (rm && rv), "sug_gate_bn_fwd_multi: eval mode needs the running buffers");
+    SUG_REQUIRE(!rm == !rv, "sug_gate_bn_fwd_multi: running_mean and running_var come together");
+    t.gamma[i] = (const float*)gamma[k];
+    t.beta[i] = (const float*)beta[k];
+    t.rmean[i] = rm;
+    t.rvar[i] = rv;
+  }
+  const dim3 grid((unsigned)sug_divup(C, 64), layers);
+  if (M <= 32)
+    hipLaunchKernelGGL(gate_bn_fwd_multi_kernel<32>, grid, dim3(64), 0, (hipStream_t)stream, x, z, M, C, t, training, eps, momentum,
+                       out, stat);
+  else
+    hipLaunchKernelGGL(gate_bn_fwd_multi_kernel<0>, grid, dim3(64), 0, (hipStream_t)stream, x, z, M, C, t, training, eps, momentum,
+                       out, stat);
+  SUG_LAUNCH_CHECK("sug_gate_bn_fwd_multi");
+  return SUG_OK;
+}
+
+extern "C" int sug_gate_bn_bwd_multi(int layers, const float* g, const float* x, const float* z, int M, int C,
+                                     const void* const* gamma, const float* stat, int training, float* dx, float* dz, float* dgb,
+                                     void* stream) {
+  SUG_REQUIRE(g && x && z && gamma && stat && dx && dz && dgb, "sug_gate_bn_bwd_multi: null pointer");
+  SUG_REQUIRE(layers >= 1 && layers <= SUG_GATE_BN_MULTI, "sug_gate_bn_bwd_multi: %d layers (1..%d)", layers, SUG_GATE_BN_MULTI);
+  SUG_REQUIRE(M >= 1 && M <= 1024 && C >= 1, "sug_gate_bn_bwd_multi: bad shape M=%d C=%d", M, C);
+  GateBNMulti t;
+  for (int i = 0; i < SUG_GATE_BN_MULTI; ++i) {
+    const int k = i < layers ? i : 0;
+    SUG_REQUIRE(gamma[k], "sug_gate_bn_bwd_multi: null parameter of layer %d", k);
+    t.gamma[i] = (const float*)gamma[k];
+    t.beta[i] = nullptr;
+    t.rmean[i] = nullptr;
+    t.rvar[i] = nullptr;
+  }
+  const dim3 grid((unsigned)sug_divup(C, 64), layers);
+  if (M <= 32)
+    hipLaunchKernelGGL(gate_bn_bwd_multi_kernel<32>, grid, dim3(64), 0, (hipStream_t)stream, g, x, z, M, C, t, stat, training, dx,
+                       dz, dgb);
+  else
+    hipLaunchKernelGGL(gate_bn_bwd_multi_kernel<0>, grid, dim3(64), 0, (hipStream_t)stream, g, x, z, M, C, t, stat, training, dx,
+                       dz, dgb);
+  SUG_LAUNCH_CHECK("sug_gate_bn_bwd_multi");
+  return SUG_OK;
+}
+
 namespace {
 
 template <typename T>
diff --git a/sug_amd/csrc/edgeconv.hip b/sug_amd/csrc/edgeconv.hip
--- a/sug_amd/csrc/edgeconv.hip
+++ b/sug_amd/csrc/edgeconv.hip
@@ -388,6 +388,76 @@
   }
 }
 
+#define SUG_FIN_GT 4
+__global__ __launch_bounds__(256 * SUG_FIN_GT) void stats_finalize_own_ws_kernel(const float* __restrict__ ws, int nblk, int C,
+                                                                                 int groups, const float* __restrict__ gamma,
+                                                                                 const float* __restrict__ beta, double count,
+                                                                                 float eps, float momentum,
+                                                                                 float* __restrict__ rmean, float* __restrict__ rvar,
+                                                                                 float* __restrict__ coef) {
+  constexpr int UN = 32;
+  __shared__ double s_p[SUG_FIN_GT][16][17];
+  __shared__ double s_tot[SUG_FIN_GT][16];
+  const int GT = blockDim.x >> 8, gl = threadIdx.x >> 8, t = threadIdx.x & 255;
+  const int cl = t & 15, p = t >> 4;
+  const int ch = blockIdx.x * 8 + (cl & 7);
+  const int col = (cl < 8) ? ch : C + ch;
+  const int W = 2 * C;
+  const size_t gstride = (size_t)SUG_STATS_BLOCKS * W;
+  const bool fin = threadIdx.x < 8 && ch < C;
+  float rm = (fin && rmean) ? rmean[ch] : 0.f, rv = (fin && rvar) ? rvar[ch] : 0.f;
+  for (int g0 = 0; g0 < groups; g0 += GT) {
+    const int ng = groups - g0 < GT ? groups - g0 : GT;
+    double acc = 0.0;
+    if (ch < C && gl < ng) {
+      const float* wg = ws + (size_t)(g0 + gl) * gstride + col;
+      for (int b = p; b < nblk; b += 16 * UN) {
+        float v[UN];
+#pragma unroll
+        for (int u = 0; u < UN; ++u) v[u] = wg[(size_t)(b + 16 * u < nblk ? b + 16 * u : b) * W];
+#pragma unroll
+        for (int u = 0; u < UN; ++u)
+          if (b + 16 * u < nblk) acc += (double)v[u];
+      }
+    }
+    __syncthreads();
+    s_p[gl][p][cl] = acc;
+    __syncthreads();
+    if (p == 0 && gl < ng) {
+      double tt = 0.0;
+#pragma unroll
+      for (int i = 0; i < 16; ++i) tt += s_p[gl][i][cl];
+      s_tot[gl][cl] = tt;
+    }
+    __syncthreads();
+    if (fin) {
+      const int c = ch;
+      for (int g = 0; g < ng; ++g) {
+        float* cg = coef + (size_t)(g0 + g) * 5 * C;
+        const float* pivot = ws + (size_t)(g0 + g) * gstride + SUG_PIVOT_OFFSET(C);
+        const double m1 = s_tot[g][threadIdx.x] / count;
+        double var = s_tot[g][8 + threadIdx.x] / count - m1 * m1;
+        if (var < 0) var = 0;
+        const double mean = (double)pivot[c] + m1;
+        const float rstd = (float)(1.0 / sqrt(var + (double)eps));
+        const float scale = gamma[c] * rstd;
+        cg[c] = scale;
+        cg[C + c] = beta[c] - (float)mean * scale;
+        cg[2 * C + c] = (float)mean;
+        cg[3 * C + c] = rstd;
+        const double unb = count > 1.0 ? var * count / (count - 1.0) : var;
+        cg[4 * C + c] = (float)unb;
+        rm = (1.f - momentum) * rm + momentum * (float)mean;
+        rv = (1.f - momentum) * rv + momentum * (float)unb;
+      }
+    }
+  }
+  if (fin) {
+    if (rmean) rmean[ch] = rm;
+    if (rvar) rvar[ch] = rv;
+  }
+}
+
 __global__ __launch_bounds__(256) void bn_replay_kernel(const float* __restrict__ coef, int G, int C,
                                                         float momentum, float* __restrict__ rmean,
                                                         float* __restrict__ rvar) {
@@ -547,9 +617,10 @@
                                                               int64_t rows, int C, float slope,
                                                               float* __restrict__ a,
                                                               float* __restrict__ ws, int LX,
-                                                              int rows_per_block, int pivoted) {
+                                                              int rows_per_block, int pivoted, int own_ws) {
   extern __shared__ __attribute__((aligned(16))) float s_red[];
-  float* const ws_pivot = ws + SUG_PIVOT_OFFSET(C) + (size_t)blockIdx.y * C;
+  if (own_ws) ws += (size_t)blockIdx.y * SUG_STATS_BLOCKS * 2 * C;
+  float* const ws_pivot = ws + SUG_PIVOT_OFFSET(C) + (own_ws ? (size_t)0 : (size_t)blockIdx.y * C);
   const int64_t g0 = (int64_t)blockIdx.y * rows;
   y += g0 * ldy;
   if (MODE >= 1) {
@@ -557,7 +628,7 @@
     if (MODE == 1) a += g0 * C;
     coef += (int64_t)blockIdx.y * 5 * C;
   }
-  ws += (size_t)blockIdx.y * gridDim.x * 2 * C;
+  if (!own_ws) ws += (size_t)blockIdx.y * gridDim.x * 2 * C;
   const int LY = 256 / LX;
   const int lx = threadIdx.x % LX, ly = threadIdx.x / LX;
   const int C4 = C >> 2;
@@ -996,7 +1067,8 @@
 
 template <int MODE>
 static int launch_col_reduce(const float* y, int64_t ldy, const float* z, const float* coef, int64_t rows,
-                             int C, float slope, float* a, float* ws, hipStream_t st, int groups = 1, int pivoted = 0);
+                             int C, float slope, float* a, float* ws, hipStream_t st, int groups = 1, int pivoted = 0,
+                             int own_ws = 0);
 
 static int col_rows_per_block(int64_t rows, int cw) {
   int64_t rpb = 64 * (256 / cw) > 256 ? 64 * (256 / cw) : 256;
@@ -1006,20 +1078,20 @@
 
 template <int MODE>
 static int launch_col_reduce(const float* y, int64_t ldy, const float* z, const float* coef, int64_t rows,
-                             int C, float slope, float* a, float* ws, hipStream_t st, int groups, int pivoted) {
+                             int C, float slope, float* a, float* ws, hipStream_t st, int groups, int pivoted, int own_ws) {
   const bool vec = (C % 4 == 0) && (ldy % 4 == 0) && ((uintptr_t)y % 16 == 0) &&
                    (MODE == 0 || (((uintptr_t)z % 16 == 0) && (MODE == 2 || (uintptr_t)a % 16 == 0) && ((uintptr_t)coef % 16 == 0)));
   if (vec) {
     int lx = 1;
     while (lx < (C >> 2) && lx < 256) lx <<= 1;
     const int ly = 256 / lx;
-    int64_t rpb = (rows * groups + SUG_STATS_ROWS - 1) / SUG_STATS_ROWS;
+    int64_t rpb = (rows * (own_ws ? 1 : groups) + SUG_STATS_ROWS - 1) / SUG_STATS_ROWS;
     if (rpb < 4 * ly) rpb = 4 * ly;
     rpb = (rpb + ly - 1) / ly * ly;
     const int grid = sug_divup(rows, rpb);
-    if ((int64_t)grid * groups > SUG_STATS_ROWS || groups > 16) return -1;
+    if ((int64_t)grid * (own_ws ? 1 : groups) > SUG_STATS_ROWS || groups > 16) return -1;
     hipLaunchKernelGGL((col_reduce_vec4_kernel<MODE>), dim3(grid, groups), dim3(256), (size_t)ly * 2 * C * sizeof(float),
-                       st, y, ldy, z, coef, rows, C, slope, a, ws, lx, (int)rpb, pivoted);
+                       st, y, ldy, z, coef, rows, C, slope, a, ws, lx, (int)rpb, pivoted, own_ws);
     return grid;
   }
   if (groups > 1 || MODE == 2) return -1;
@@ -1066,6 +1138,19 @@
   hipLaunchKernelGGL(stats_finalize_groups_kernel, dim3(sug_divup(C, 8)), dim3(1024), 0, st, ws, grid, C, groups, gamma, beta,
                      (double)rows, eps, momentum, running_mean, running_var, coef, ws + SUG_PIVOT_OFFSET(C));
   SUG_LAUNCH_CHECK("sug_bn_act_rows_fwd(finalize)");
+  return SUG_OK;
+}
+int sug_col_stats_bn_own_ws(const float* y, int64_t ldy, int64_t rows, int C, int groups, const float* gamma,
+                            const float* beta, float eps, float momentum, float* running_mean, float* running_var,
+                            float* coef, float* ws, hipStream_t st) {
+  if (groups < 2) return 1;
+  const int grid = launch_col_reduce<0>(y, ldy, nullptr, nullptr, rows, C, 0.f, nullptr, ws, st, groups, 1, 1);
+  if (grid < 0) return 1;
+  SUG_LAUNCH_CHECK("sug_col_stats_bn_groups_exact(stats)");
+  hipLaunchKernelGGL(stats_finalize_own_ws_kernel, dim3(sug_divup(C, 8)), dim3(256 * (groups < SUG_FIN_GT ? groups : SUG_FIN_GT)), 0,
+                     st, ws, grid, C, groups, gamma, beta,
+                     (double)rows, eps, momentum, running_mean, running_var, coef);
+  SUG_LAUNCH_CHECK("sug_col_stats_bn_groups_exact(finalize)");
   return SUG_OK;
 }
 int sug_affine_act_groups(const float* z, int64_t ldz, const float* coef, int64_t rows, int groups, int C, float slope,
diff --git a/sug_amd/csrc/layers.cpp b/sug_amd/csrc/layers.cpp
--- a/sug_amd/csrc/layers.cpp
+++ b/sug_amd/csrc/layers.cpp
@@ -13,6 +13,14 @@
 int sug_bn_bwd_apply_groups(const float* a, int64_t lda, int from_g, float slope, const float* y, int64_t ldy,
                             const float* coef, const double* red, int64_t rows_g, int groups, int C, float* dy,
                             int64_t lddy, ihipStream_t* st);
+int sug_col_stats_bn_own_ws(const float* y, int64_t ldy, int64_t rows, int C, int groups, const float* gamma,
+                            const float* beta, float eps, float momentum, float* running_mean, float* running_var,
+                            float* coef, float* ws, ihipStream_t* st);
+int sug_bn_act_pool_fwd_groups(const float* y, int64_t ldy, const float* coef, int B, int groups, int N, int C, float slope,
+                               float* out_max, float* out_mean, int64_t ld_pool, int32_t* arg, float* ws, ihipStream_t* st);
+int sug_bn_act_pool_bwd_groups(const float* y, int64_t ldy, const float* coef, const float* gmax, const float* gmean,
+                               int64_t ld_pool, const int32_t* arg, int B, int groups, int N, int C, float slope, double* red,
+                               float* ws, float* dy, int64_t lddy, float* dgb, ihipStream_t* st);
 int sug_edgeconv_fwd_bn_act_groups(const float* pq, int64_t ldpq, const int32_t* idx, const float* gamma,
                                    const float* beta, int B, int N, int k, int Co, int groups, float eps, float momentum,
                                    float slope, float* running_mean, float* running_var, float* z, uint8_t* arg,
@@ -201,3 +209,67 @@
   if (dgb) LAYER_TRY(sug_fold_groups(red, groups, 2 * C, dgb, stream));
   return SUG_OK;
 }
+
+extern "C" int sug_col_stats_bn_groups_exact(const float* y, int64_t ldy, int64_t rows, int C, int groups, const float* gamma,
+                                             const float* beta, float eps, float momentum, float* running_mean,
+                                             float* running_var, float* coef, float* ws, void* stream) {
+  LAYER_REQUIRE(groups >= 1 && rows > 0 && rows % groups == 0, "sug_col_stats_bn_groups_exact: %lld rows do not split into %d groups",
+                (long long)rows, groups);
+  LAYER_REQUIRE(y && gamma && beta && coef && ws, "sug_col_stats_bn_groups_exact: null pointer");
+  LAYER_REQUIRE(C > 0 && C <= 4096 && ldy >= C, "sug_col_stats_bn_groups_exact: bad shape");
+  const int64_t rg = rows / groups;
+  if (groups > 1 && groups <= 16) {
+    const int rc = sug_col_stats_bn_own_ws(y, ldy, rg, C, groups, gamma, beta, eps, momentum, running_mean, running_var, coef, ws,
+                                           (ihipStream_t*)stream);
+    if (rc <= 0) return rc;
+  }
+  for (int g = 0; g < groups; ++g)
+    LAYER_TRY(sug_col_stats_bn(y + g * rg * ldy, ldy, rg, C, gamma, beta, eps, momentum, running_mean, running_var,
+                               coef + (int64_t)g * 5 * C, ws, stream));
+  return SUG_OK;
+}
+
+extern "C" int sug_bn_act_pool_groups_fwd(const float* y, int64_t ldy, int B, int N, int C, int groups, const float* gamma,
+                                          const float* beta, int training, float eps, float momentum, float slope,
+                                          float* running_mean, float* running_var, float* coef, float* out_max, float* out_mean,
+                                          int64_t ld_pool, int32_t* arg, double* stats, float* ws_stats, float* ws_pool,
+                                          void* stream) {
+  LAYER_REQUIRE(groups >= 1 && B > 0 && B % groups == 0, "sug_bn_act_pool_groups_fwd: B=%d does not split into %d groups", B, groups);
+  if (training && groups > 1 && groups <= 16) {
+    LAYER_REQUIRE(y && gamma && beta && coef && out_max && out_mean && arg && ws_stats && ws_pool,
+                  "sug_bn_act_pool_groups_fwd: null pointer");
+    LAYER_REQUIRE(N > 0 && C > 0 && C <= 4096 && ldy >= C && ld_pool >= C, "sug_bn_act_pool_groups_fwd: bad shape");
+    ihipStream_t* st = (ihipStream_t*)stream;
+    const int Bg = B / groups;
+    const int64_t rg = (int64_t)Bg * N;
+    int rc = sug_col_stats_bn_own_ws(y, ldy, rg, C, groups, gamma, beta, eps, momentum, running_mean, running_var, coef, ws_stats, st);
+    if (rc < 0) return rc;
+    if (rc == 0) {
+      rc = sug_bn_act_pool_fwd_groups(y, ldy, coef, B, groups, N, C, slope, out_max, out_mean, ld_pool, arg, ws_pool, st);
+      if (rc <= 0) return rc;
+      for (int g = 0; g < groups; ++g)
+        LAYER_TRY(sug_bn_act_pool_fwd(y + g * rg * ldy, ldy, coef + (int64_t)g * 5 * C, Bg, N, C, slope,
+                                      out_max + (int64_t)g * Bg * ld_pool, out_mean + (int64_t)g * Bg * ld_pool, ld_pool,
+                                      arg + (int64_t)g * Bg * C, ws_pool, stream));
+      return SUG_OK;
+    }
+  }
+  return sug_bn_act_pool_layer_fwd(y, ldy, B, N, C, groups, gamma, beta, training, eps, momentum, slope, running_mean, running_var,
+                                   coef, out_max, out_mean, ld_pool, arg, stats, ws_stats, ws_pool, stream);
+}
+
+extern "C" int sug_bn_act_pool_groups_bwd(const float* y, int64_t ldy, const float* coef, const float* gmax, const float* gmean,
+                                          int64_t ld_pool, const int32_t* arg, int B, int N, int C, int groups, float slope,
+                                          int training, double* red, float* ws, float* dy, int64_t lddy, float* dgb,
+                                          void* stream) {
+  LAYER_REQUIRE(groups >= 1 && B > 0 && B % groups == 0, "sug_bn_act_pool_groups_bwd: B=%d does not split into %d groups", B, groups);
+  if (training && groups > 1 && groups <= 16) {
+    LAYER_REQUIRE(y && coef && gmax && gmean && arg && red && ws && dy, "sug_bn_act_pool_groups_bwd: null pointer");
+    LAYER_REQUIRE(N > 0 && C > 0 && ldy >= C && lddy >= C && ld_pool >= C, "sug_bn_act_pool_groups_bwd: bad shape");
+    const int rc = sug_bn_act_pool_bwd_groups(y, ldy, coef, gmax, gmean, ld_pool, arg, B, groups, N, C, slope, red, ws, dy, lddy,
+                                              dgb, (ihipStream_t*)stream);
+    if (rc <= 0) return rc;
+  }
+  return sug_bn_act_pool_layer_bwd(y, ldy, coef, gmax, gmean, ld_pool, arg, B, N, C, groups, slope, training, red, ws, dy, lddy,
+                                   dgb, stream);
+}
diff --git a/sug_amd/csrc/mmd.hip b/sug_amd/csrc/mmd.hip
--- a/sug_amd/csrc/mmd.hip
+++ b/sug_amd/csrc/mmd.hip
@@ -201,9 +201,8 @@
   if (i < n) out[i] = (float)((sums[3 * i] + sums[3 * i + 1] - 2.0 * sums[3 * i + 2]) / mm);
 }
 
-__global__ __launch_bounds__(256) void chamfer_dir_kernel(const float* __restrict__ a,
-                                                          const float* __restrict__ bpts, int N, int M,
-                                                          float* __restrict__ part) {
+__device__ __forceinline__ void chamfer_dir_body(const float* __restrict__ a, const float* __restrict__ bpts, int N, int M,
+                                                 float* __restrict__ part, int nb) {
   extern __shared__ __attribute__((aligned(16))) float s_p[];
   const int b = blockIdx.y;
   const float* bb = bpts + (int64_t)b * M * 3;
@@ -241,7 +240,25 @@
   const float s = wave_sum_f(best);
   if ((threadIdx.x & (WAVE - 1)) == 0) s_w[threadIdx.x / WAVE] = s;
   __syncthreads();
-  if (threadIdx.x == 0) part[(int64_t)b * gridDim.x + blockIdx.x] = ((s_w[0] + s_w[1]) + s_w[2]) + s_w[3];
+  if (threadIdx.x == 0) part[(int64_t)b * nb + blockIdx.x] = ((s_w[0] + s_w[1]) + s_w[2]) + s_w[3];
+}
+
+__global__ __launch_bounds__(256) void chamfer_dir_kernel(const float* __restrict__ a,
+                                                          const float* __restrict__ bpts, int N, int M,
+                                                          float* __restrict__ part) {
+  chamfer_dir_body(a, bpts, N, M, part, gridDim.x);
+}
+
+__global__ __launch_bounds__(256) void chamfer_both_kernel(const float* __restrict__ a, const float* __restrict__ bpts, int N,
+                                                           int M, int nbn, int nbm, float* __restrict__ pn,
+                                                           float* __restrict__ pm) {
+  if (blockIdx.z == 0) {
+    if ((int)blockIdx.x >= nbn) return;
+    chamfer_dir_body(a, bpts, N, M, pn, nbn);
+  } else {
+    if ((int)blockIdx.x >= nbm) return;
+    chamfer_dir_body(bpts, a, M, N, pm, nbm);
+  }
 }
 
 __global__ __launch_bounds__(256) void chamfer_fold_kernel(const float* __restrict__ pn, int nbn, const float* __restrict__ pm,
@@ -571,6 +588,21 @@
   return SUG_OK;
 }
 
+extern "C" int sug_chamfer_merged(const float* a, const float* b, int B, int N, int M, float* out, float* ws, void* stream) {
+  SUG_REQUIRE(a && b && out && ws, "sug_chamfer_merged: null pointer");
+  SUG_REQUIRE(B > 0 && N > 0 && M > 0 && N <= 5000 && M <= 5000 && B <= 65535, "sug_chamfer_merged: bad shape");
+  hipStream_t st = (hipStream_t)stream;
+  const int nbn = sug_divup(4 * N, 256), nbm = sug_divup(4 * M, 256);
+  float* pm = ws + (int64_t)B * nbn;
+  hipLaunchKernelGGL(chamfer_both_kernel, dim3(nbn > nbm ? nbn : nbm, B, 2), dim3(256), (size_t)(N > M ? N : M) * 4 * sizeof(float),
+                     st, a, b, N, M, nbn, nbm, ws, pm);
+  SUG_LAUNCH_CHECK("sug_chamfer_merged(directions)");
+  hipLaunchKernelGGL(chamfer_fold_kernel, dim3(sug_divup(B, 256)), dim3(256), 0, st, ws, nbn, pm, nbm, B, 1.0f / (float)N,
+                     1.0f / (float)M, out);
+  SUG_LAUNCH_CHECK("sug_chamfer_merged");
+  return SUG_OK;
+}
+
 extern "C" int sug_mmd_rbf_rows_bwd(const float* z, int64_t ldz, const float* wt, int m, int D, int row0, int mloc,
                                     const float* gscale, float gmul, float* dz, int64_t lddz, void* stream) {
   SUG_REQUIRE(z && wt && gscale && dz, "sug_mmd_rbf_bwd: null pointer");
@@ -819,6 +851,24 @@
   return SUG_OK;
 }
 
+extern "C" int sug_chamfer_weights_merged(const float* a, const float* b, int B, int N, int M, int method, float* out,
+                                          float* ws, void* stream) {
+  SUG_REQUIRE(a && b && out && ws, "sug_chamfer_weights_merged: null pointer");
+  SUG_REQUIRE(B > 0 && N > 0 && M > 0 && N <= 5000 && M <= 5000 && B <= 65535, "sug_chamfer_weights_merged: bad shape");
+  SUG_REQUIRE(method >= 1 && method <= 3, "sug_chamfer_weights_merged: weighting method %d (1 naive_inverse, 2 exp_inverse, 3 mean2one)",
+              method);
+  hipStream_t st = (hipStream_t)stream;
+  const int nbn = sug_divup(4 * N, 256), nbm = sug_divup(4 * M, 256);
+  float* pm = ws + (int64_t)B * nbn;
+  hipLaunchKernelGGL(chamfer_both_kernel, dim3(nbn > nbm ? nbn : nbm, B, 2), dim3(256), (size_t)(N > M ? N : M) * 4 * sizeof(float),
+                     st, a, b, N, M, nbn, nbm, ws, pm);
+  SUG_LAUNCH_CHECK("sug_chamfer_weights_merged(directions)");
+  hipLaunchKernelGGL(chamfer_fold_weights_kernel, dim3(1), dim3(256), 0, st, ws, nbn, pm, nbm, B, 1.0f / (float)N,
+                     1.0f / (float)M, method, out);
+  SUG_LAUNCH_CHECK("sug_chamfer_weights_merged");
+  return SUG_OK;
+}
+
 namespace {
 
 constexpr int SEL_MAX_M = SUG_CLASS_MMD_MAX_ROWS, SEL_MAX_CLASSES = SUG_CLASS_MMD_MAX_CLASSES, SEL_MAX_D = SUG_CLASS_MMD_MAX_D;
diff --git a/sug_amd/ops.py b/sug_amd/ops.py
--- a/sug_amd/ops.py
+++ b/sug_amd/ops.py
@@ -1176,6 +1176,9 @@
     return out
 
 
+BN_POOL_GROUPED = _os.environ.get('SUG_BN_POOL_GROUPED', '1') != '0'
+
+
 class _BNActPool(torch.autograd.Function):
 
     @staticmethod
@@ -1190,20 +1193,25 @@
         omax, omean = pooled[:, :C], pooled[:, C:]
         arg = torch.empty(B, C, dtype=torch.int32, device=dev)
         stats = torch.empty(2 * C, dtype=torch.float64, device=dev)
-        wss = _stats_ws(C, dev)
-        wsp = torch.empty(12 * (B // G) * C, dtype=torch.float32, device=dev)
-        check(lib().sug_bn_act_pool_layer_fwd(_p(y), ld, B, N, C, G, _p(g), _p(b), st.train, st.eps, st.momentum,
-                                              float(slope), _p(st.mean), _p(st.var), _p(coef), _p(omax),
-                                              _p(omean), 2 * C, _p(arg), _p(stats), _p(wss), _p(wsp), _st()),
-              'sug_bn_act_pool_layer_fwd')
+        grouped = BN_POOL_GROUPED and G > 1
+        if grouped:
+            wss = torch.empty(G * STATS_BLOCKS * 2 * C, dtype=torch.float32, device=dev)
+            wsp = torch.empty(12 * B * C, dtype=torch.float32, device=dev)
+            fwd, name = lib().sug_bn_act_pool_groups_fwd, 'sug_bn_act_pool_groups_fwd'
+        else:
+            wss = _stats_ws(C, dev)
+            wsp = torch.empty(12 * (B // G) * C, dtype=torch.float32, device=dev)
+            fwd, name = lib().sug_bn_act_pool_layer_fwd, 'sug_bn_act_pool_layer_fwd'
+        check(fwd(_p(y), ld, B, N, C, G, _p(g), _p(b), st.train, st.eps, st.momentum, float(slope), _p(st.mean), _p(st.var),
+                  _p(coef), _p(omax), _p(omean), 2 * C, _p(arg), _p(stats), _p(wss), _p(wsp), _st()), name)
         ctx.save_for_backward(y, coef, arg)
-        ctx.meta = (B, N, C, ld, float(slope), st.train, G)
+        ctx.meta = (B, N, C, ld, float(slope), st.train, G, grouped)
         return pooled
 
     @staticmethod
     def backward(ctx, g):
         y, coef, arg = ctx.saved_tensors
-        B, N, C, ld, slope, train, G = ctx.meta
+        B, N, C, ld, slope, train, G, grouped = ctx.meta
         dev = y.device
         if g.stride(1) != 1 or g.stride(0) < 2 * C:
             g = g.contiguous()
@@ -1212,9 +1220,10 @@
         ws = _stats_ws(C, dev)
         dy = torch.empty(B, N, C, dtype=torch.float32, device=dev)
         rf = torch.empty(2 * C, dtype=torch.float32, device=dev)
-        check(lib().sug_bn_act_pool_layer_bwd(_p(y), ld, _p(coef), _p(gmax), _p(gmean), ldp, _p(arg), B, N, C, G, slope,
-                                              train, _p(red), _p(ws), _p(dy), C, _p(rf), _st()),
-              'sug_bn_act_pool_layer_bwd')
+        bwd, name = (lib().sug_bn_act_pool_groups_bwd, 'sug_bn_act_pool_groups_bwd') if grouped else \
+            (lib().sug_bn_act_pool_layer_bwd, 'sug_bn_act_pool_layer_bwd')
+        check(bwd(_p(y), ld, _p(coef), _p(gmax), _p(gmean), ldp, _p(arg), B, N, C, G, slope, train, _p(red), _p(ws), _p(dy), C,
+                  _p(rf), _st()), name)
         return (dy,) + _dgamma_dbeta(rf) + (None, None)
 
 
@@ -1230,6 +1239,14 @@
     _check_groups('bn_update_stats', rows, 'rows', G)
     rg = rows // G
     g, b = bn.weight.detach().contiguous(), bn.bias.detach().contiguous()
+    if BN_POOL_GROUPED and G > 1:
+        coef = torch.empty(G, 5, C, dtype=torch.float32, device=y.device)
+        ws = torch.empty(G * STATS_BLOCKS * 2 * C, dtype=torch.float32, device=y.device)
+        check(lib().sug_col_stats_bn_groups_exact(_p(y2), y2.stride(0), rows, C, G, _p(g), _p(b), bn.eps, bn.momentum,
+                                                  _p(bn.running_mean), _p(bn.running_var), _p(coef), _p(ws), _st()),
+              'sug_col_stats_bn_groups_exact')
+        _count_bn_call(bn)
+        return
     coef = torch.empty(5, C, dtype=torch.float32, device=y.device)
     ws = _stats_ws(C, y.device)
     for i in range(G):
@@ -1850,6 +1867,7 @@
 
 
 CALAYER_FUSED = _os.environ.get('SUG_CALAYER_FUSED', '1') != '0'
+GATE_BN_MULTI = _os.environ.get('SUG_GATE_BN_MULTI', '1') != '0'
 
 
 def calayer_supported(layers, x):
@@ -1891,17 +1909,22 @@
         out = torch.empty(nl * M, C, dtype=torch.float32, device=dev)
         stat = torch.empty(nl, 2, C, dtype=torch.float32, device=dev)
         xc = x if x.stride(0) == C else x.contiguous()
-        for a in range(nl):
+        multi = GATE_BN_MULTI and 1 < nl <= 4
+        if multi:
+            check(L.sug_gate_bn_fwd_multi(nl, _p(xc), _p(z), M, C, _ptrs(gam), _ptrs(bet), _ptrs([p[6] for p in P]),
+                                          _ptrs([p[7] for p in P]), 1 if training else 0, float(eps), float(momentum), _p(out),
+                                          _p(stat), _st()), 'sug_gate_bn_fwd_multi')
+        for a in range(0 if multi else nl):
             check(L.sug_gate_bn_fwd(_p(xc[a * M:]), _p(z[a * M:]), M, C, _p(gam[a]), _p(bet[a]), _p(P[a][6]), _p(P[a][7]),
                                     1 if training else 0, float(eps), float(momentum), _p(out[a * M:]), _p(stat[a]), _st()),
                   'sug_gate_bn_fwd')
         ctx.save_for_backward(xc, h, z, stat, *W0, *W2, *gam)
-        ctx.meta = (nl, M, C, Hd, bool(training))
+        ctx.meta = (nl, M, C, Hd, bool(training), multi)
         return out
 
     @staticmethod
     def backward(ctx, g):
-        nl, M, C, Hd, training = ctx.meta
+        nl, M, C, Hd, training, multi = ctx.meta
         sv = ctx.saved_tensors
         x, h, z, stat = sv[:4]
         W0, W2, gam = sv[4:4 + nl], sv[4 + nl:4 + 2 * nl], sv[4 + 2 * nl:4 + 3 * nl]
@@ -1910,7 +1933,10 @@
         g = g.contiguous()
         dxg, dz = torch.empty_like(x), torch.empty_like(x)
         dgb = torch.empty(nl, 2, C, dtype=torch.float32, device=dev)
-        for a in range(nl):
+        if multi:
+            check(L.sug_gate_bn_bwd_multi(nl, _p(g), _p(x), _p(z), M, C, _ptrs(gam), _p(stat), 1 if training else 0, _p(dxg), _p(dz),
+                                          _p(dgb), _st()), 'sug_gate_bn_bwd_multi')
+        for a in range(0 if multi else nl):
             check(L.sug_gate_bn_bwd(_p(g[a * M:]), _p(x[a * M:]), _p(z[a * M:]), M, C, _p(gam[a]), _p(stat[a]), 1 if training else 0,
                                     _p(dxg[a * M:]), _p(dz[a * M:]), _p(dgb[a, 0]), _p(dgb[a, 1]), _st()), 'sug_gate_bn_bwd')
         f32 = torch.float32
@@ -3139,6 +3165,9 @@
     return outs
 
 
+CHAMFER_MERGED = _os.environ.get('SUG_CHAMFER_MERGED', '1') != '0'
+
+
 def chamfer(a, b):
     _need_gpu(a, b)
     a, b = a.detach().contiguous(), b.detach().contiguous()
@@ -3146,7 +3175,8 @@
     M = b.shape[1]
     out = torch.empty(B, dtype=torch.float32, device=a.device)
     ws = torch.empty(lib().sug_chamfer_workspace(B, N, M), dtype=torch.float32, device=a.device)
-    check(lib().sug_chamfer(_p(a), _p(b), B, N, M, _p(out), _p(ws), _st()), 'sug_chamfer')
+    fn, name = (lib().sug_chamfer_merged, 'sug_chamfer_merged') if CHAMFER_MERGED else (lib().sug_chamfer, 'sug_chamfer')
+    check(fn(_p(a), _p(b), B, N, M, _p(out), _p(ws), _st()), name)
     return out
 
 
@@ -3159,7 +3189,9 @@
     M = b.shape[1]
     out = torch.empty(B, dtype=torch.float32, device=a.device)
     ws = torch.empty(lib().sug_chamfer_workspace(B, N, M), dtype=torch.float32, device=a.device)
-    check(lib().sug_chamfer_weights(_p(a), _p(b), B, N, M, _SDA_METHODS[method], _p(out), _p(ws), _st()), 'sug_chamfer_weights')
+    fn, name = (lib().sug_chamfer_weights_merged, 'sug_chamfer_weights_merged') if CHAMFER_MERGED else \
+        (lib().sug_chamfer_weights, 'sug_chamfer_weights')
+    check(fn(_p(a), _p(b), B, N, M, _SDA_METHODS[method], _p(out), _p(ws), _st()), name)
     return out
 
 
```

After: 14030, median of 6. +1.2%, better.
